# zhouzypaul/fql

Measured on AMD Instinct MI355X. Metric: FQL gradient-steps/s (batch=256), higher is better.
Workload: dtype f32

## Files before the change

### fql_amd/csrc/fql_chain.h

```cpp
#pragma once
#include "fql_kernels.h"

#define FQL_CHAIN_THREADS 512
#ifndef FQL_CHAIN_WAVES
#define FQL_CHAIN_WAVES 4
#endif

struct ChainArgs {
    const float* A;
    const float* Wf;
    const float* bias;
    float* C;
    union {
        struct {
            const float* ea_in;
            float* ea_out;
            const float* W0f;
            const float* evp_in;
            const float* eb;
            const float* W4f;
            float* evp_out;
        };
        struct {
            const float* Gv;
            const float* stats;
            const float* gamma;
            const float* dq;
            const float* wq;
            int ldq, ldw;
            int width;
            int ncol, ldc;
        };
    };
    int M, ad, ap, ea_ld;
    float inv_steps, t_s;
    int variant;
    const float* Zprev;
    int xg;
    int hw;
    int tl;
    unsigned long long* stamps;
};

struct WfragTask {
    const float* src;
    float* dst;
    int K, N, ld;
    int kvalid;
    int tile0;
    int mode;
};
__global__ __launch_bounds__(FQL_THREADS) void fql_wfrag_kernel(const WfragTask* __restrict__ tasks, int ntasks, int tl) {
    tl_enter(tl);
    const WfragTask& T = tasks[find_task(tasks, ntasks, blockIdx.x)];
    const int e = (blockIdx.x - T.tile0) * FQL_THREADS + threadIdx.x;
    if (T.mode == 1) {
        const int n = e % T.N, r = e / T.N;
        const int q = r & 3, j = r >> 2;
        if (j >= (T.K >> 5)) return;
        float v[8];
#pragma unroll
        for (int i = 0; i < 8; ++i) { const int k = 32 * j + 8 * q + i; v[i] = (k < T.kvalid) ? ldg(T.src + (size_t)k * T.ld + n) : 0.f; }
        u32x4 hi, lo;
#pragma unroll
        for (int i = 0; i < 4; ++i) { unsigned h, l; bsplit2(v[2 * i], v[2 * i + 1], h, l); hi[i] = h; lo[i] = l; }
        unsigned* d = reinterpret_cast<unsigned*>(T.dst) + (((size_t)(2 * j) * T.N + n) * 4 + q) * 4;
        *(FQL_GAS u32x4*)d = hi;
        *(FQL_GAS u32x4*)(d + (size_t)T.N * 16) = lo;
        return;
    }
    if (T.mode == 2) {
        const int n = e % T.N, k4 = e / T.N;
        if (k4 >= (T.K >> 2)) return;
        float v[4];
#pragma unroll
        for (int i = 0; i < 4; ++i) v[i] = (4 * k4 + i < T.kvalid) ? ldg(T.src + (size_t)(4 * k4 + i) * T.ld + n) : 0.f;
        unsigned h0, l0, h1, l1;
        bsplit2(v[0], v[1], h0, l0);
        bsplit2(v[2], v[3], h1, l1);
        *(FQL_GAS u32x4*)(reinterpret_cast<unsigned*>(T.dst) + ((size_t)k4 * T.N + n) * 4) = u32x4{h0, h1, l0, l1};
        return;
    }
    const int n = e % T.N, k4 = e / T.N;
    if (k4 >= (T.K >> 2)) return;
    f32x4 v;
#pragma unroll
    for (int s = 0; s < 4; ++s) v[s] = (4 * k4 + s < T.kvalid) ? ldg(T.src + (size_t)(4 * k4 + s) * T.ld + n) : 0.f;
    stg4(T.dst + ((size_t)k4 * T.N + n) * 4, v);
}

template <int H, int V>
__device__ __forceinline__ void chain_body(const ChainArgs& P) {
    static_assert(H % 128 == 0 && H <= 1024, "hidden width must be a multiple of 128");
    constexpr int S = H + 4;
    constexpr int GQ = H / 64;
    constexpr int NA = H / 128;
    constexpr int CT = H / 128;
    constexpr int NT = H / 32;
    extern __shared__ __attribute__((aligned(16))) float lds[];
    float* red = lds + 16 * S;
    float* ea = red + 4 * 2 * 64 * 4;
    float* hs = ea + 512;
    const int tid = threadIdx.x, wave = tid >> 6, lane = tid & 63;
    const int c = lane & 15, q = lane >> 4;
    const int nt = wave & 1, kp = wave >> 1;
    constexpr int variant = V;
    const int ntc = variant == 4 ? P.ncol / 32 : NT;
    int tm = blockIdx.x / ntc, tn = blockIdx.x - tm * ntc;
    if (P.xg) xcd_tile((int)blockIdx.x, P.M >> 4, ntc, P.xg, tm, tn);
    const int row0 = tm * 16, n0 = tn * 32 + nt * 16;
    tl_enter(P.tl);
#ifdef FQL_STAMPS
    unsigned long long stamp[8];
    int nst = 0;
#define CSTAMP() do { __builtin_amdgcn_s_waitcnt(0); stamp[nst++] = __builtin_amdgcn_s_memrealtime(); } while (0)
#else
#define CSTAMP() do {} while (0)
#endif
    CSTAMP();
    f32x4 bf[GQ];
    {
        if (variant == 3 || variant == 4) {
            const float* wb = P.Wf + (size_t)(n0 + c) * H + 16 * kp * GQ + 4 * q;
#pragma unroll
            for (int g = 0; g < GQ; ++g) bf[g] = ldg4(wb + 16 * g);
        } else {
            const float* wb = P.Wf + ((size_t)(4 * kp * GQ + q) * H + n0 + c) * 4;
#pragma unroll
            for (int g = 0; g < GQ; ++g) bf[g] = ldg4(wb + (size_t)g * 16 * H);
        }
    }
    const float bias = variant == 4 ? 0.f : variant == 3 ? ldg(P.Zprev + (size_t)(row0 + 4 * q + kp) * H + n0 + c) : ldg(P.bias + n0 + c);
    f32x4 bw4[2];
    if (variant == 2 && wave == 0) {
#pragma unroll
        for (int g = 0; g < 2; ++g) bw4[g] = ldg4(P.W4f + ((size_t)(tn * 8 + 4 * g + q) * P.ap + c) * 4);
    }
    if (variant == 0) {
        f32x4 cacc[CT], wf[CT];
#pragma unroll
        for (int t = 0; t < CT; ++t) {
            const int ct = wave + 8 * t;
            cacc[t] = ldg4(P.A + ((size_t)((row0 >> 2) + q) * H + 16 * ct + c) * 4);
            wf[t] = ldg4(P.W0f + ((size_t)q * H + 16 * ct + c) * 4);
        }
        {
            const int e = tid >> 1, half = tid & 1;
            const int r = e >> 4, j = e & 15;
            float a = 0.f;
            if (j < P.ad) {
                a = ldg(P.ea_in + (size_t)(row0 + r) * P.ea_ld + j);
                if (P.evp_in) {
                    float pv[NT / 2];
                    const float* pp = P.evp_in + ((size_t)(half * (NT / 2)) * P.M + row0 + r) * P.ap + j;
#pragma unroll
                    for (int tp = 0; tp < NT / 2; ++tp) pv[tp] = ldg(pp + (size_t)tp * P.M * P.ap);
                    float sum = 0.f;
#pragma unroll
                    for (int tp = 0; tp < NT / 2; ++tp) sum += pv[tp];
                    const float other = __shfl_xor(sum, 1);
                    const float tot = half ? other + sum : sum + other;
                    a += (tot + ldg(P.eb + j)) * P.inv_steps;
                }
                if (tn == 0 && half == 0 && P.ea_out) stg(P.ea_out + (size_t)(row0 + r) * P.ap + j, a);
            } else if (j == P.ad) {
                a = P.t_s;
            }
            if (half == 0) ea[r * 32 + j] = a;
        }
        CSTAMP();
        __syncthreads();
        {
            const f32x4 af = *reinterpret_cast<const f32x4*>(&ea[c * 32 + 4 * q]);
#pragma unroll
            for (int t = 0; t < CT; ++t) {
#pragma unroll
                for (int s4 = 0; s4 < 4; ++s4) cacc[t] = __builtin_amdgcn_mfma_f32_16x16x4f32(af[s4], wf[t][s4], cacc[t], 0, 0, 0);
                const int ct = wave + 8 * t;
#pragma unroll
                for (int i = 0; i < 4; ++i) lds[(4 * q + i) * S + 16 * ct + c] = gelu_f(cacc[t][i]);
            }
        }
    } else if (variant == 4) {
        constexpr int NV = H / 256;
        f32x4 dy[2][NV], zz[2][NV], gq[2][NV], gm[NV];
        float mean[2], rstd[2];
#pragma unroll
        for (int i = 0; i < NV; ++i) gm[i] = ldg4(P.gamma + 4 * (lane + 64 * i));
        float wqv[NV][4];
        if (!P.A) {
#pragma unroll
            for (int i = 0; i < NV; ++i)
#pragma unroll
                for (int e = 0; e < 4; ++e) wqv[i][e] = ldg(P.wq + (size_t)(4 * (lane + 64 * i) + e) * P.ldw);
        }
#pragma unroll
        for (int r = 0; r < 2; ++r) {
            const size_t row = (size_t)(row0 + 2 * wave + r);
            mean[r] = ldg(P.stats + 2 * row); rstd[r] = ldg(P.stats + 2 * row + 1);
            const float dqr = P.A ? 0.f : ldg(P.dq + row * P.ldq);
#pragma unroll
            for (int i = 0; i < NV; ++i) {
                const int k4 = 4 * (lane + 64 * i);
                zz[r][i] = ldg4(P.Zprev + row * H + k4);
                gq[r][i] = ldg4(P.Gv + row * H + k4);
                if (P.A) dy[r][i] = ldg4(P.A + row * H + k4);
                else dy[r][i] = f32x4{dqr * wqv[i][0], dqr * wqv[i][1], dqr * wqv[i][2], dqr * wqv[i][3]};
            }
        }
        const float inv = 1.0f / (float)P.width;
#pragma unroll
        for (int r = 0; r < 2; ++r) {
            float s1 = 0.f, s2 = 0.f;
#pragma unroll
            for (int i = 0; i < NV; ++i)
#pragma unroll
                for (int e = 0; e < 4; ++e) {
                    const float d = dy[r][i][e] * gm[i][e], xh = (gq[r][i][e] - mean[r]) * rstd[r];
                    dy[r][i][e] = d; gq[r][i][e] = xh;
                    if (4 * (lane + 64 * i) + e < P.width) { s1 += d; s2 += d * xh; }
                }
#pragma unroll
            for (int o = 1; o < 64; o <<= 1) { s1 += __shfl_xor(s1, o); s2 += __shfl_xor(s2, o); }
            const float m1 = s1 * inv, m2 = s2 * inv;
#pragma unroll
            for (int i = 0; i < NV; ++i) {
                f32x4 o;
#pragma unroll
                for (int e = 0; e < 4; ++e)
                    o[e] = (4 * (lane + 64 * i) + e < P.width) ? rstd[r] * (dy[r][i][e] - m1 - gq[r][i][e] * m2) * zz[r][i][e] : 0.f;
                *reinterpret_cast<f32x4*>(&lds[(2 * wave + r) * S + 4 * (lane + 64 * i)]) = o;
            }
        }
    } else {
        f32x4 av[NA];
        const float* Ag = P.A + (size_t)row0 * H;
#pragma unroll
        for (int i = 0; i < NA; ++i) av[i] = ldg4(Ag + (size_t)(tid + i * FQL_CHAIN_THREADS) * 4);
#pragma unroll
        for (int i = 0; i < NA; ++i) {
            const int f = tid + i * FQL_CHAIN_THREADS;
            const int r = f / (H / 4), kk = f - r * (H / 4);
            *reinterpret_cast<f32x4*>(&lds[r * S + 4 * kk]) = av[i];
        }
        CSTAMP();
    }
    __syncthreads();
    CSTAMP();
    f32x4 acc = {0.f, 0.f, 0.f, 0.f}, acc2 = {0.f, 0.f, 0.f, 0.f};
    {
        const float* arow = lds + c * S + 4 * q + 16 * kp * GQ;
#pragma unroll
        for (int g = 0; g < GQ; g += 2) {
            const f32x4 a = *reinterpret_cast<const f32x4*>(arow + 16 * g);
            const f32x4 a2 = *reinterpret_cast<const f32x4*>(arow + 16 * g + 16);
#pragma unroll
            for (int s4 = 0; s4 < 4; ++s4) {
                acc = __builtin_amdgcn_mfma_f32_16x16x4f32(a[s4], bf[g][s4], acc, 0, 0, 0);
                acc2 = __builtin_amdgcn_mfma_f32_16x16x4f32(a2[s4], bf[g + 1][s4], acc2, 0, 0, 0);
            }
        }
        acc += acc2;
    }
    *reinterpret_cast<f32x4*>(&red[((kp * 2 + nt) * 64 + lane) * 4]) = acc;
    CSTAMP();
    __syncthreads();
    float v = (variant == 3 || variant == 4) ? 0.f : bias;
#pragma unroll
    for (int p = 0; p < 4; ++p) v += red[((p * 2 + nt) * 64 + lane) * 4 + kp];
    v = variant == 4 ? v : variant == 3 ? v * bias : gelu_f(v);
    const int row = row0 + 4 * q + kp;
    if (variant == 4) {
        stg(P.C + (size_t)row * P.ldc + n0 + c, v);
    } else if (variant != 2) {
        stg(P.C + (size_t)row * H + n0 + c, v);
    } else {
        hs[(4 * q + kp) * 36 + 16 * nt + c] = v;
        __syncthreads();
        if (wave == 0) {
            f32x4 pa = {0.f, 0.f, 0.f, 0.f};
#pragma unroll
            for (int g = 0; g < 2; ++g) {
                const f32x4 a4 = *reinterpret_cast<const f32x4*>(&hs[c * 36 + 16 * g + 4 * q]);
#pragma unroll
                for (int s4 = 0; s4 < 4; ++s4) pa = __builtin_amdgcn_mfma_f32_16x16x4f32(a4[s4], bw4[g][s4], pa, 0, 0, 0);
            }
            if (c < P.ap) {
#pragma unroll
                for (int i = 0; i < 4; ++i) stg(P.evp_out + ((size_t)tn * P.M + row0 + 4 * q + i) * P.ap + c, pa[i]);
            }
        }
    }
    tl_exit(P.tl);
#ifdef FQL_STAMPS
    CSTAMP();
    if (lane == 0 && wave == 0 && P.stamps) {
        unsigned long long* d = P.stamps + (size_t)blockIdx.x * 8;
        for (int i = 0; i < nst; ++i) d[i] = stamp[i];
    }
#endif
}
struct Dgrad0Args {
    GemmTask t[4];
    int ntasks, col0;
};
__device__ __forceinline__ void fql_dgrad0_body(const Dgrad0Args& P) {
    __shared__ __attribute__((aligned(16))) float red[4 * 64 * 4];
    const int tid = threadIdx.x, kp = tid >> 6, lane = tid & 63, c = lane & 15, q = lane >> 4;
    const int ntm = P.t[0].M >> 4;
    const int ti = (int)blockIdx.x / ntm, tm = (int)blockIdx.x - ti * ntm;
    const GemmTask& T = P.t[ti];
    const int row0 = tm * 16, kq = T.K >> 2;
    const float* ap = T.A + (size_t)(row0 + c) * T.lda + kp * kq + 4 * q;
    const float* bp = T.B + (size_t)(P.col0 + c) * T.ldb + kp * kq + 4 * q;
    f32x4 acc = {0.f, 0.f, 0.f, 0.f}, acc2 = {0.f, 0.f, 0.f, 0.f};
    for (int g0 = 0; g0 < kq; g0 += 128) {
        f32x4 a[8], b[8];
#pragma unroll
        for (int g = 0; g < 8; ++g) { a[g] = ldg4(ap + g0 + 16 * g); b[g] = ldg4(bp + g0 + 16 * g); }
#pragma unroll
        for (int g = 0; g < 8; g += 2)
#pragma unroll
            for (int s4 = 0; s4 < 4; ++s4) {
                acc = __builtin_amdgcn_mfma_f32_16x16x4f32(a[g][s4], b[g][s4], acc, 0, 0, 0);
                acc2 = __builtin_amdgcn_mfma_f32_16x16x4f32(a[g + 1][s4], b[g + 1][s4], acc2, 0, 0, 0);
            }
    }
    acc += acc2;
    *reinterpret_cast<f32x4*>(&red[(kp * 64 + lane) * 4]) = acc;
    __syncthreads();
    float v = 0.f;
#pragma unroll
    for (int p = 0; p < 4; ++p) v += red[(p * 64 + lane) * 4 + kp];
    stg(T.C + (size_t)(row0 + 4 * q + kp) * T.ldc + P.col0 + c, v);
}
__global__ __launch_bounds__(FQL_THREADS) void fql_dgrad0_kernel(const Dgrad0Args P) { fql_dgrad0_body(P); }
__global__ __launch_bounds__(FQL_THREADS) void fql_dgrad0_multi_kernel(const Dgrad0Args* __restrict__ args) { fql_dgrad0_body(args[blockIdx.y]); }

__device__ __forceinline__ void fql_head_dgrad_body(const GemmTask& T) {
    __shared__ __attribute__((aligned(16))) float da[16 * 20];
    const int tid = threadIdx.x, wave = tid >> 6, lane = tid & 63, c = lane & 15, q = lane >> 4;
    const int ntn = T.N >> 6;
    const int tm = (int)blockIdx.x / ntn, tn = (int)blockIdx.x - tm * ntn;
    const int row0 = tm * 16, n0 = tn * 64 + 16 * wave;
    const f32x4 b4 = ldg4(T.B + (size_t)(n0 + c) * T.ldb + 4 * q);
    float zp[4];
#pragma unroll
    for (int i = 0; i < 4; ++i) zp[i] = ldg(T.Zprev + (size_t)(row0 + 4 * q + i) * T.ldc + n0 + c);
    {
        const int r = tid >> 4, j = tid & 15;
        float g = 0.f;
        if (j < T.i2) {
            const float ar = ldg(T.ea_in + (size_t)(row0 + r) * T.i0 + j);
            float tg;
            if (T.flags & GF_A_EULFIN) {
                float pv[32];
#pragma unroll
                for (int tp = 0; tp < 32; ++tp) pv[tp] = ldg(T.aux2 + ((size_t)min(tp, T.ln_width - 1) * T.M + row0 + r) * T.i0 + j);
                float sum = 0.f;
#pragma unroll
                for (int tp = 0; tp < 32; ++tp) sum += (tp < T.ln_width) ? pv[tp] : 0.f;
                tg = clip1(ldg(T.aux + (size_t)(row0 + r) * T.i0 + j) + (sum + ldg(T.eb + j)) * T.f1);
                if (tn == 0) stg(const_cast<float*>(T.evp) + (size_t)(row0 + r) * T.i0 + j, tg);
            } else tg = ldg(T.evp + (size_t)(row0 + r) * T.i0 + j);
            g = T.f0 * (ar - tg);
            if (ar > -1.0f && ar < 1.0f) {
                const size_t o = (size_t)(row0 + r) * T.e_ntp + T.i1 + j;
                g += ldg(T.ew + o) + ldg(T.ew4 + o);
            }
            if (tn == 0 && T.ea_out) stg(T.ea_out + (size_t)(row0 + r) * T.i0 + j, g);
        }
        da[r * 20 + j] = g;
    }
    __syncthreads();
    const f32x4 a4 = *reinterpret_cast<const f32x4*>(&da[c * 20 + 4 * q]);
    f32x4 acc = {0.f, 0.f, 0.f, 0.f};
#pragma unroll
    for (int s4 = 0; s4 < 4; ++s4) acc = __builtin_amdgcn_mfma_f32_16x16x4f32(a4[s4], b4[s4], acc, 0, 0, 0);
#pragma unroll
    for (int i = 0; i < 4; ++i) stg(T.C + (size_t)(row0 + 4 * q + i) * T.ldc + n0 + c, acc[i] * zp[i]);
}
__global__ __launch_bounds__(FQL_THREADS) void fql_head_dgrad_kernel(const GemmTask T) { fql_head_dgrad_body(T); }
__global__ __launch_bounds__(FQL_THREADS) void fql_head_dgrad_multi_kernel(const GemmTask* __restrict__ args) { const GemmTask T = ((const FQL_CONST_AS GemmTask*)args)[blockIdx.y]; fql_head_dgrad_body(T); }

template <int H, int V>
__global__ __launch_bounds__(FQL_CHAIN_THREADS, FQL_CHAIN_WAVES) void fql_chain_kernel(const ChainArgs P) { chain_body<H, V>(P); }
struct ChainPair { ChainArgs t[2]; };
template <int H, int V>
__global__ __launch_bounds__(FQL_CHAIN_THREADS, FQL_CHAIN_WAVES) void fql_chain_pair_kernel(const ChainPair P) { chain_body<H, V>(P.t[blockIdx.y]); }
template <int H, int V>
__global__ __launch_bounds__(FQL_CHAIN_THREADS, FQL_CHAIN_WAVES) void fql_chain_multi_kernel(const ChainArgs* __restrict__ args) { const ChainArgs P = args[blockIdx.y]; chain_body<H, V>(P); }
__device__ __forceinline__ float lane_xor1(float v) {
    return __int_as_float(__builtin_amdgcn_mov_dpp(__float_as_int(v), 0xB1, 0xF, 0xF, true));
}
#ifndef FQL_CHAIN_SPLIT_WAVES_A
#define FQL_CHAIN_SPLIT_WAVES_A 4
#endif
template <int H, int V>
__global__ __launch_bounds__(FQL_CHAIN_THREADS, (V == 0 ? FQL_CHAIN_SPLIT_WAVES_A : 4)) void fql_chain_split_kernel(const ChainArgs P) {
    static_assert(H % 128 == 0 && H <= 1024, "hidden width must be a multiple of 128");
    constexpr int RS = H / 2;
    constexpr int NS = H / 128;
    constexpr int NA = H / 128;
    constexpr int CT = H / 128;
    constexpr int NT = H / 32;
    extern __shared__ __attribute__((aligned(16))) float lds[];
    unsigned* ahi = reinterpret_cast<unsigned*>(lds);
    unsigned* alo = ahi + 16 * RS;
    float* red = reinterpret_cast<float*>(alo + 16 * RS);
    float* ea = red + 4 * 2 * 64 * 4;
    float* hs = ea + 512;
    const int tid = threadIdx.x, wave = tid >> 6, lane = tid & 63;
    const int c = lane & 15, q = lane >> 4;
    const int nt = wave & 1, kp = wave >> 1;
    int tm = blockIdx.x / NT, tn = blockIdx.x - tm * NT;
    if (P.xg) xcd_tile((int)blockIdx.x, P.M >> 4, NT, P.xg, tm, tn);
    const int row0 = tm * 16, n0 = tn * 32 + nt * 16;
    constexpr int variant = V;
    tl_enter(P.tl);
    u32x4 bh[NS], bl[NS];
    {
        const unsigned* wb = reinterpret_cast<const unsigned*>(P.Wf) + (((size_t)(2 * kp * NS) * H + n0 + c) * 4 + q) * 4;
#pragma unroll
        for (int s = 0; s < NS; ++s) { bh[s] = ldg4u(wb + (size_t)s * H * 32); bl[s] = ldg4u(wb + (size_t)s * H * 32 + H * 16); }
    }
    const float bias = ldg(P.bias + n0 + c);
    u32x4 w4h, w4l;
    if (variant == 2 && wave == 0) {
        const unsigned* w4 = reinterpret_cast<const unsigned*>(P.W4f) + (((size_t)(2 * tn) * P.ap + c) * 4 + q) * 4;
        w4h = ldg4u(w4); w4l = ldg4u(w4 + P.ap * 16);
    }
    if (variant == 0) {
        f32x4 cacc[CT];
        u32x4 wf[CT];
#pragma unroll
        for (int t = 0; t < CT; ++t) {
            const int ct = wave + 8 * t;
            cacc[t] = ldg4(P.A + (((size_t)(row0 >> 4) * (H / 16) + ct) * 64 + 16 * q + c) * 4);
            wf[t] = ldg4u(reinterpret_cast<const unsigned*>(P.W0f) + ((size_t)q * H + 16 * ct + c) * 4);
        }
        {
            const int e = tid >> 1, half = tid & 1;
            const int r = e >> 4, j = e & 15;
            float a = 0.f;
            if (j < P.ad) {
                a = ldg(P.ea_in + (size_t)(row0 + r) * P.ea_ld + j);
                if (P.evp_in) {
                    float pv[NT / 2];
                    const float* pp = P.evp_in + ((size_t)(half * (NT / 2)) * P.M + row0 + r) * P.ap + j;
#pragma unroll
                    for (int tp = 0; tp < NT / 2; ++tp) pv[tp] = ldg(pp + (size_t)tp * P.M * P.ap);
                    float sum = 0.f;
#pragma unroll
                    for (int tp = 0; tp < NT / 2; ++tp) sum += pv[tp];
                    const float other = __shfl_xor(sum, 1);
                    const float tot = half ? other + sum : sum + other;
                    a += (tot + ldg(P.eb + j)) * P.inv_steps;
                }
                if (tn == 0 && half == 0 && P.ea_out) stg(P.ea_out + (size_t)(row0 + r) * P.ap + j, a);
            } else if (j == P.ad) {
                a = P.t_s;
            }
            if (half == 0) ea[r * 32 + j] = a;
        }
        __syncthreads();
        {
            const f32x4 af = *reinterpret_cast<const f32x4*>(&ea[c * 32 + 4 * q]);
            u32x2 afh, afl;
            bsplit4(af, afh, afl);
#pragma unroll
            for (int t = 0; t < CT; ++t) {
                const u32x2 wh = u32x2{wf[t][0], wf[t][1]}, wl = u32x2{wf[t][2], wf[t][3]};
                cacc[t] = mfma_bf16_k16(wl, afh, cacc[t]);
                cacc[t] = mfma_bf16_k16(wh, afl, cacc[t]);
                cacc[t] = mfma_bf16_k16(wh, afh, cacc[t]);
            }
#pragma unroll
            for (int t = 0; t < CT; ++t) {
                const int ct = wave + 8 * t;
                f32x4 g;
#pragma unroll
                for (int i = 0; i < 4; ++i) g[i] = gelu_f(cacc[t][i]);
                u32x2 hi, lo;
                bsplit4(g, hi, lo);
                const int w = c * RS + 4 * ((2 * ct + (q >> 1)) ^ c) + 2 * (q & 1);
                *reinterpret_cast<u32x2*>(ahi + w) = hi;
                *reinterpret_cast<u32x2*>(alo + w) = lo;
            }
        }
    } else {
        u32x4 av[NA];
        const unsigned* Ah = reinterpret_cast<const unsigned*>(P.A) + (size_t)row0 * RS;
        const unsigned* Al = Ah + (size_t)P.M * RS;
#pragma unroll
        for (int i = 0; i < NA; ++i) {
            const int pc = (tid + i * FQL_CHAIN_THREADS) & (4 * RS - 1);
            av[i] = ldg4u((i < NA / 2 ? Ah : Al) + (size_t)pc * 4);
        }
#pragma unroll
        for (int i = 0; i < NA; ++i) {
            const int pc = (tid + i * FQL_CHAIN_THREADS) & (4 * RS - 1);
            const int r = pc / (RS / 4), sl = pc - r * (RS / 4);
            *reinterpret_cast<u32x4*>((i < NA / 2 ? ahi : alo) + r * RS + 4 * (sl ^ r)) = av[i];
        }
    }
    __syncthreads();
    f32x4 acc = {0.f, 0.f, 0.f, 0.f}, acc2 = {0.f, 0.f, 0.f, 0.f}, acc3 = {0.f, 0.f, 0.f, 0.f};
#pragma unroll
    for (int s = 0; s < NS; ++s) {
        const int w = c * RS + 4 * ((4 * (kp * NS + s) + q) ^ c);
        const u32x4 fah = *reinterpret_cast<const u32x4*>(ahi + w);
        const u32x4 fal = *reinterpret_cast<const u32x4*>(alo + w);
        acc = mfma_bf16(fah, bh[s], acc);
        acc2 = mfma_bf16(fah, bl[s], acc2);
        acc3 = mfma_bf16(fal, bh[s], acc3);
    }
    acc += acc2 + acc3;
    *reinterpret_cast<f32x4*>(&red[((kp * 2 + nt) * 64 + lane) * 4]) = acc;
    __syncthreads();
    float v = bias;
#pragma unroll
    for (int p = 0; p < 4; ++p) v += red[((p * 2 + nt) * 64 + lane) * 4 + kp];
    v = gelu_f(v);
    const int row = row0 + 4 * q + kp;
    if (variant != 2) {
        const float o = lane_xor1(v);
        unsigned h, l;
        bsplit2((c & 1) ? o : v, (c & 1) ? v : o, h, l);
        unsigned* Cw = reinterpret_cast<unsigned*>(P.C) + ((c & 1) ? (size_t)P.M * RS : 0) + (size_t)row * RS + ((n0 + c) >> 1);
        *(FQL_GAS unsigned*)Cw = (c & 1) ? l : h;
    } else {
        hs[(4 * q + kp) * 36 + 16 * nt + c] = v;
        __syncthreads();
        if (wave == 0) {
            const f32x4 a0 = *reinterpret_cast<const f32x4*>(&hs[c * 36 + 8 * q]);
            const f32x4 a1 = *reinterpret_cast<const f32x4*>(&hs[c * 36 + 8 * q + 4]);
            u32x2 h0, l0, h1, l1;
            bsplit4(a0, h0, l0);
            bsplit4(a1, h1, l1);
            const u32x4 fah = u32x4{h0[0], h0[1], h1[0], h1[1]}, fal = u32x4{l0[0], l0[1], l1[0], l1[1]};
            f32x4 pa = {0.f, 0.f, 0.f, 0.f};
            pa = mfma_bf16(fal, w4h, pa);
            pa = mfma_bf16(fah, w4l, pa);
            pa = mfma_bf16(fah, w4h, pa);
            if (c < P.ap) {
#pragma unroll
                for (int i = 0; i < 4; ++i) stg(P.evp_out + ((size_t)tn * P.M + row0 + 4 * q + i) * P.ap + c, pa[i]);
            }
        }
    }
    tl_exit(P.tl);
}
#define FQL_CHAIN_LDS_BYTES(H) ((size_t)(16 * ((H) + 4) + 4 * 2 * 64 * 4 + 512 + 16 * 36) * sizeof(float))
```

### fql_amd/csrc/fql_engine.hip

```cpp
#include "../../include/fql_amd.h"
#include "fql_kernels.h"
#include "fql_conv.h"
#include "fql_chain.h"
#include "fql_aux.h"
#include "fql_ifql.h"
#include "fql_rebrac.h"
#include "fql_sac.h"
#include "fql_bc.h"
#include "fql_iql.h"
#include "fql_iqld.h"
#include "fql_cfgrl.h"
#include <hip/hip_ext.h>
#include "fql_aql.h"

#include <algorithm>
#include <cmath>
#include <cstdarg>
#include <cstdio>
#include <cstdlib>
#include <cstring>
#include <map>
#include <memory>
#include <random>
#include <string>
// ... 131 lines not shown
template <typename... Pm, typename... A>
Bound bind(void (*k)(Pm...), Geo g, A&&... a) {
    static_assert(sizeof...(Pm) == sizeof...(A) && sizeof...(Pm) <= FQL_BOUND_ARGS, "a bound launch takes exactly the kernel's arguments");
    static_assert(packed_bytes<Pm...>() <= FQL_BOUND_BYTES, "arguments larger than a kernarg segment");
    Bound b;
    b.fn = (const void*)k;
    b.grid[0] = g.grid.x; b.grid[1] = g.grid.y; b.grid[2] = g.grid.z;
    b.block[0] = g.block.x; b.block[1] = g.block.y; b.block[2] = g.block.z;
    b.lds = (unsigned)g.lds;
    b.args.resize(packed_bytes<Pm...>());
    size_t off = 0;
    auto put = [&](auto v) {
        using T = decltype(v);
        off = (off + alignof(T) - 1) & ~(alignof(T) - 1);
        b.at[b.nargs++] = (int)off;
        std::memcpy(b.args.data() + off, &v, sizeof(T));
        off += sizeof(T);
    };
    (put(static_cast<Pm>(a)), ...);
    return b;
}
inline Bound tl_in(Bound k, size_t off) { k.tl_at = k.at[0] + (int)off; return k; }
inline Bound tl_last(Bound k) { k.tl_at = k.at[k.nargs - 1]; return k; }
inline void launch_bound(const Bound& k, const void* args, hipStream_t s, hipEvent_t pa = nullptr, hipEvent_t pb = nullptr) {
    void* argv[FQL_BOUND_ARGS];
    for (int i = 0; i < k.nargs; ++i) argv[i] = (unsigned char*)args + k.at[i];
    const dim3 g(k.grid[0], k.grid[1], k.grid[2]), b(k.block[0], k.block[1], k.block[2]);
    if (pa) (void)hipExtLaunchKernel(k.fn, g, b, argv, k.lds, s, pa, pb, 0);
    else (void)hipLaunchKernel(k.fn, g, b, argv, k.lds, s);
}

struct Op {
    OpType type;
    std::vector<const void*> reads, writes;
    GemmTask gemm;
    WgradTask wgrad;
    LnBwdTask ln;
    PostOsArgs postos;
    LossCriticArgs lc;
    LossQArgs lq;
    LossBcArgs lb;
    ConvArgs conv;
    ConvWgradArgs cw;
    ConvWredArgs cwr;
    const ConvWprepTask* wprep_tasks = nullptr;
    int wprep_n = 0;
    int cw_grid = 0;
    Bound k;
    double macs = 0.0;
    int level = 0;
    int lane = 0;
    int launch = -1;
    std::vector<int> deps;
};

struct Launch {
    Launch() = default;
    Launch(OpType t, int ln) : type(t), lane(ln) {}
    OpType type;
    int lane = 0;
    int grid = 0, ntasks = 0;
    Bound k;
    double macs = 0.0;
    void* table = nullptr;
    void *table_w = nullptr, *table_l = nullptr, *table_m = nullptr;
    int n_w = 0, n_l = 0, tile_w = 0, tile_l = 0, tile_m = 0;
    std::vector<GemmTask> h_gemm;
    std::vector<WgradTask> h_wgrad;
    std::vector<LnBwdTask> h_ln;
    std::vector<MiscTask> h_misc;
    bool ka = false;
    std::vector<int> waits;
    bool record_after = false;
    hipEvent_t ev = nullptr;
};

inline bool ka_tasks_env() {
    const char* e = getenv("FQL_KERNARG_TASKS");
    return !e || atoi(e) != 0;
}
inline bool fused_tail_env() {
    const char* e = getenv("FQL_FUSED_TAIL");
    return !e || atoi(e) != 0;
}
inline std::unique_ptr<SideArgs> ka_side_args(const Launch& L) {
    const size_t ng = L.h_gemm.size(), nw = L.h_wgrad.size(), nl = L.h_ln.size(), nm = L.h_misc.size();
    if (ng > FQL_KA_GEMM || nw > FQL_KA_WGRAD || nl > FQL_KA_LN || nm > FQL_KA_MISC) return nullptr;
    auto a = std::make_unique<SideArgs>();
    std::memset(a.get(), 0, sizeof(SideArgs));
    SideFront& f = a->f;
    f.tile_w = L.tile_w; f.tile_l = L.tile_l; f.tile_m = L.tile_m; f.tl = -1;
    for (int& v : f.g0) v = FQL_KA_FRONT_PAD;
    for (int& v : f.w0) v = FQL_KA_FRONT_PAD;
    for (int& v : f.l0) v = FQL_KA_FRONT_PAD;
    for (size_t i = 0; i < ng; ++i) { a->g[i] = L.h_gemm[i]; if (i) f.g0[i - 1] = L.h_gemm[i].tile0; }
    for (size_t i = 0; i < nw; ++i) { a->w[i] = L.h_wgrad[i]; if (i) f.w0[i - 1] = L.h_wgrad[i].tile0; }
    for (size_t i = 0; i < nl; ++i) { a->l[i] = L.h_ln[i]; if (i) f.l0[i - 1] = L.h_ln[i].tile0; }
    for (size_t i = 0; i < nm; ++i) a->m[i] = L.h_misc[i];
    return a;
}
struct AdamOpt {
    float lr = 0.f;
    DevState* st = nullptr;
    int polyak = -1;
    bool fin = false;
};
struct Program {
    std::vector<Op> ops;
    std::vector<Launch> launches;
    bool lane_used[FQL_LANES] = {};
    hipEvent_t ev_fork = nullptr, ev_join[FQL_LANES] = {};
    hipGraph_t graph = nullptr;
    hipGraphExec_t exec = nullptr;
    int64_t macs = 0;
    AqlProgram aql;
    bool aql_tried = false;
};

template <typename P, typename IssueFn>
void issue_lanes(P& pr, hipStream_t s0, const hipStream_t* ls, bool fork, IssueFn&& issue) {
    auto lazy = [](hipEvent_t& e) { if (!e) HIP_CHECK(hipEventCreateWithFlags(&e, hipEventDisableTiming)); };
    bool side = false;
    if (ls) for (int l = 1; l < FQL_LANES; ++l) side |= pr.lane_used[l];
    if (side && fork) {
        lazy(pr.ev_fork);
        HIP_CHECK(hipEventRecord(pr.ev_fork, s0));
        for (int l = 1; l < FQL_LANES; ++l) if (pr.lane_used[l]) HIP_CHECK(hipStreamWaitEvent(ls[l], pr.ev_fork, 0));
    }
    for (auto& L : pr.launches) {
        const hipStream_t s = side && L.lane != 0 ? ls[L.lane] : s0;
        if (side)
            for (int w : L.waits) if (pr.launches[w].ev) HIP_CHECK(hipStreamWaitEvent(s, pr.launches[w].ev, 0));
        issue(L, s);
        if (side && L.record_after) {
            lazy(L.ev);
            HIP_CHECK(hipEventRecord(L.ev, s));
        }
    }
    if (side)
        for (int l = 1; l < FQL_LANES; ++l) {
            if (!pr.lane_used[l]) continue;
            lazy(pr.ev_join[l]);
            HIP_CHECK(hipEventRecord(pr.ev_join[l], ls[l]));
            HIP_CHECK(hipStreamWaitEvent(s0, pr.ev_join[l], 0));
        }
    HIP_CHECK(hipGetLastError());
}
template <typename P>
void destroy_lane_events(P& pr) {
    for (auto& L : pr.launches) if (L.ev) { hipEventDestroy(L.ev); L.ev = nullptr; }
    if (pr.ev_fork) { hipEventDestroy(pr.ev_fork); pr.ev_fork = nullptr; }
    for (hipEvent_t& e : pr.ev_join) if (e) { hipEventDestroy(e); e = nullptr; }
}

template <typename Body>
void capture_graph(hipStream_t s, Body&& body, hipGraph_t& graph, hipGraphExec_t& exec) {
    static const bool trace = getenv("FQL_TRACE") != nullptr;
    HIP_CHECK(hipStreamBeginCapture(s, hipStreamCaptureModeThreadLocal));
    try {
        body();
    } catch (...) {
        hipGraph_t g = nullptr;
        hipStreamEndCapture(s, &g);
        if (g) hipGraphDestroy(g);
        throw;
    }
// ... 1692 lines not shown
            HIP_CHECK(hipMemcpy(all + at, o->wprep_tasks, (size_t)o->wprep_n * sizeof(ConvWprepTask), hipMemcpyDeviceToDevice));
            at += o->wprep_n;
        }
        Launch L(OP_CONV_WPREP, sel[0]->lane);
        L.k = bind_wprep(all, tot);
        return L;
    }
    Launch form_gemm16(const Cell& sel, std::vector<void*>& owner) {
        Launch L(OP_GEMM, sel[0]->lane);
        L.ntasks = (int)sel.size();
        int tile = 0;
        for (const Op* o : sel) {
            GemmTask t = o->gemm;
            t.wk = (t.N <= 16) ? 4 : 2;
            t.tmt = 1;
            t.ntn = (t.N / 16 + (4 / t.wk) - 1) / (4 / t.wk);
            t.tile0 = tile;
            tile += (t.M / 16) * t.ntn;
            L.h_gemm.push_back(t);
        }
        L.table = upload(owner, L.h_gemm.data(), L.h_gemm.size() * sizeof(GemmTask));
        L.grid = tile;
        bind_gemm16(L);
        return L;
    }

    static double op_macs(const Op& o) {
        if (o.type == OP_GEMM || o.type == OP_GEMM64 || o.type == OP_HEAD_DGRAD) return (double)o.gemm.M * o.gemm.N * o.gemm.K;
        if (o.type == OP_DGRAD0) return (double)o.gemm.M * 16.0 * o.gemm.K;
        if (o.type == OP_WGRAD) return (double)o.wgrad.M * o.wgrad.Kin * o.wgrad.N;
        if (o.type == OP_CHAIN) return o.macs;
        if (o.type == OP_CONV || o.type == OP_CONV_U8) return (double)o.conv.N * o.conv.H * o.conv.W * 9.0 * (o.conv.transposed ? o.conv.Ci : o.conv.Ci_real) * o.conv.Co;
        if (o.type == OP_CONV_WGRAD) return (double)o.cw.N * o.cw.H * o.cw.W * 9.0 * o.cw.Ci_real * o.cw.Co;
        return 0.0;
    }
    static void cross_lane_waits(Program& pr) {
        std::vector<int> need(pr.launches.size() * FQL_LANES, -1);
        for (const Op& o : pr.ops) {
            if (o.launch < 0) continue;
            for (int d : o.deps) {
                const int dl = pr.ops[d].launch;
                const int ol = pr.launches[dl].lane;
                int& nd = need[o.launch * FQL_LANES + ol];
                if (ol != o.lane) nd = std::max(nd, dl);
            }
        }
        int waited_upto[FQL_LANES][FQL_LANES];
        for (auto& r : waited_upto) for (int& v : r) v = -1;
        for (int li = 0; li < (int)pr.launches.size(); ++li) {
            Launch& L = pr.launches[li];
            for (int ol = 0; ol < FQL_LANES; ++ol) {
                const int nd = need[li * FQL_LANES + ol];
                if (nd <= waited_upto[L.lane][ol]) continue;
                L.waits.push_back(nd);
                pr.launches[nd].record_after = true;
                waited_upto[L.lane][ol] = nd;
            }
        }
    }
    void dump_program(const Program& pr) const {
        std::vector<int> level(pr.launches.size(), -1);
        std::vector<std::string> what(pr.launches.size());
        char b[96];
        for (const Op& o : pr.ops) {
            if (o.launch < 0) continue;
            level[o.launch] = o.level;
            if (o.type == OP_GEMM || o.type == OP_GEMM64) snprintf(b, sizeof b, " g%s(%dx%dx%d%s)", o.type == OP_GEMM64 ? "64" : "16", o.gemm.M, o.gemm.N, o.gemm.K, (o.gemm.flags & GF_TRANS_B) ? "T" : "");
            else if (o.type == OP_WGRAD) snprintf(b, sizeof b, " w(%dx%dx%d)", o.wgrad.M, o.wgrad.Kin, o.wgrad.N);
            else if (o.type == OP_LNBWD) snprintf(b, sizeof b, " ln(%d)", o.ln.M);
            else snprintf(b, sizeof b, " t%d", (int)o.type);
            what[o.launch] += b;
        }
        int cnt[FQL_LANES] = {};
        for (int li = 0; li < (int)pr.launches.size(); ++li) {
            const Launch& L = pr.launches[li];
            cnt[L.lane]++;
            fprintf(stderr, "[fql] #%2d level %3d lane %d type %2d ntasks %2d grid %5d waits[", li, level[li], L.lane, (int)L.type, L.ntasks, L.grid);
            for (int w : L.waits) fprintf(stderr, "%d ", w);
            fprintf(stderr, "] :%s\n", what[li].c_str());
        }
        fprintf(stderr, "[fql] launches per lane:");
        for (int l = 0; l < FQL_LANES; ++l) fprintf(stderr, " %d", cnt[l]);
        fprintf(stderr, "\n");
    }
    static void check_lane_edges(const Program& pr) {
        bool edge[FQL_LANES][FQL_LANES] = {};
        for (const Launch& L : pr.launches)
            for (int w : L.waits) edge[pr.launches[w].lane][L.lane] = true;
        for (int a = 1; a < FQL_LANES; ++a)
            for (int b = a + 1; b < FQL_LANES; ++b)
                if (edge[a][b] && edge[b][a])
                    invalid("lane placement makes lanes %d and %d wait on each other in both directions: not capturable on this HIP runtime "
                            "(hipStreamEndCapture recursion); move one of the passes", a, b);
    }

    hipEvent_t prof_a = nullptr, prof_b = nullptr;
    void issue_args(const Launch& L, int tl, unsigned char* a) const {
        const Bound& k = L.k;
        if (!k.fn) throw HipError{"internal: op type " + std::to_string((int)L.type) + " carries no bound launch"};
        std::memcpy(a, k.args.data(), k.args.size());
        if (k.tl_at >= 0) std::memcpy(a + k.tl_at, &tl, sizeof tl);
        if (L.type == OP_IQLD_CFG) std::memcpy(a + offsetof(IqldCfgStepArgs, cfg), &sample_cfg, sizeof sample_cfg);
    }
    void issue(const Launch& L, hipStream_t s, int tl) {
        alignas(16) unsigned char a[FQL_BOUND_BYTES];
        issue_args(L, tl, a);
        launch_bound(L.k, a, s, prof_a, prof_b);
    }
    int tl_of(const Program& pr, const Launch& L) const { return &pr == &prog_full ? (int)(&L - pr.launches.data()) : -1; }
    void run_launches(Program& pr, hipStream_t s0, const hipStream_t* ls = nullptr, bool fork = true) {
        static const bool trace_l = getenv("FQL_TRACE") != nullptr;
        issue_lanes(pr, s0, ls, fork, [&](const Launch& L, hipStream_t s) {
            if (trace_l) {
                fprintf(stderr, "[fql] launch %d type %d lane %d grid %d waits %zu:", (int)(&L - pr.launches.data()), (int)L.type, L.lane, L.grid, L.waits.size());
                for (int w : L.waits) fprintf(stderr, " %d(lane %d)", w, pr.launches[w].lane);
                fprintf(stderr, "\n");
            }
            issue(L, s, tl_of(pr, L));
        });
    }
    std::vector<AqlDispatch> dispatches(const Program& pr) const {
        std::vector<AqlDispatch> out;
        alignas(16) unsigned char a[FQL_BOUND_BYTES];
        for (const Launch& L : pr.launches) {
            issue_args(L, tl_of(pr, L), a);
            const Bound& k = L.k;
            out.push_back(AqlDispatch{k.fn, {k.grid[0], k.grid[1], k.grid[2]}, {k.block[0], k.block[1], k.block[2]}, k.lds, std::vector<uint8_t>(a, a + k.args.size())});
        }
        return out;
    }

    void build_aql(Program& pr) {
        static const bool off = getenv("FQL_AQL") && atoi(getenv("FQL_AQL")) == 0;
        static const bool trace_a = getenv("FQL_TRACE") != nullptr;
        AqlProgram& ap = pr.aql;
        ap = AqlProgram{};
        if (off || visual) return;
        void* kargs = nullptr;
        try {
            if (!aql.up && aql.why.empty()) aql.init(device, (const void*)&fql_create);
            if (!aql.up) throw AqlError{aql.why};
            const std::vector<AqlDispatch> rec = dispatches(pr);
            const size_t n = pr.launches.size();

            std::vector<const AqlKernelInfo*> ki(n);
            std::vector<size_t> koff(n);
            size_t tot = 0;
            for (size_t i = 0; i < n; ++i) {
                ki[i] = &aql.kernel(rec[i].fn);
                if (ki[i]->kernarg_size < rec[i].args.size()) throw AqlError{"recorded arguments exceed the kernel's kernarg segment"};
                koff[i] = tot;
                tot += ((size_t)ki[i]->kernarg_size + 63) & ~(size_t)63;
            }
            std::vector<uint8_t> host(tot);
            for (size_t i = 0; i < n; ++i) AqlRuntime::fill_kernarg(host.data() + koff[i], rec[i], *ki[i]);
            HIP_CHECK(hipMalloc(&kargs, tot));
            HIP_CHECK(hipMemcpy(kargs, host.data(), tot, hipMemcpyHostToDevice));
            std::vector<int> sig(n, AQL_SIG_NONE);
            int nsig = 0;
            bool used[FQL_AQL_LANES] = {};
            for (const Launch& L : pr.launches) {
                if (L.lane < 0 || L.lane >= FQL_AQL_LANES) throw AqlError{"lane out of range"};
                used[L.lane] = true;
                for (int w : L.waits) if (sig[w] == AQL_SIG_NONE) sig[w] = nsig++;
            }
            if (!used[0]) throw AqlError{"program without a lane 0"};
            int endsig[FQL_AQL_LANES];
            for (int l = 1; l < FQL_AQL_LANES; ++l) endsig[l] = used[l] ? nsig++ : AQL_SIG_NONE;
            constexpr int AG = HSA_FENCE_SCOPE_AGENT, SY = HSA_FENCE_SCOPE_SYSTEM, NO = HSA_FENCE_SCOPE_NONE;
            for (int l = 1; l < FQL_AQL_LANES; ++l)
                if (used[l]) {
                    AqlPacket b = AqlRuntime::barrier_packet(false, NO, NO);
                    b.deps[0] = AQL_SIG_PREV_DONE;
                    ap.lane[l].push_back(b);
                }
            bool first[FQL_AQL_LANES] = {true, true, true, true};
            for (size_t i = 0; i < n; ++i) {
                const Launch& L = pr.launches[i];
                for (size_t w0 = 0; w0 < L.waits.size(); w0 += 5) {
                    AqlPacket b = AqlRuntime::barrier_packet(false, NO, NO);
                    for (size_t j = 0; j < 5 && w0 + j < L.waits.size(); ++j) b.deps[j] = sig[L.waits[w0 + j]];
                    ap.lane[L.lane].push_back(b);
                }
                AqlPacket k = AqlRuntime::kernel_packet(rec[i], *ki[i], (uint64_t)(uintptr_t)kargs + koff[i], true, first[L.lane] ? SY : AG, AG);
                first[L.lane] = false;
                k.complete = sig[i];
                ap.lane[L.lane].push_back(k);
            }
            for (int l = 1; l < FQL_AQL_LANES; ++l)
                if (used[l]) {
                    AqlPacket b = AqlRuntime::barrier_packet(true, NO, AG);
                    b.complete = endsig[l];
                    ap.lane[l].push_back(b);
                }
            {
                AqlPacket b = AqlRuntime::barrier_packet(true, NO, SY);
                int j = 0;
                for (int l = 1; l < FQL_AQL_LANES; ++l) if (used[l]) b.deps[j++] = endsig[l];
                b.complete = AQL_SIG_DONE;
                ap.lane[0].push_back(b);
            }
            aql.ensure_signals(nsig);
            for (int l = 0; l < FQL_AQL_LANES; ++l) if (used[l]) aql.ensure_queue(l);
            ap.nsig = nsig;
            ap.kernargs = kargs;
            ap.ok = true;
            if (trace_a) fprintf(stderr, "[fql] AQL program: %zu launches, packets per lane %zu %zu %zu %zu, %d signals, %zu bytes of kernargs\n", n,
                                 ap.lane[0].size(), ap.lane[1].size(), ap.lane[2].size(), ap.lane[3].size(), nsig, tot);
        } catch (const AqlError& e) {
            if (kargs) hipFree(kargs);
            ap = AqlProgram{};
            if (aql.why.empty()) aql.why = e.msg;
            if (trace_a || getenv("FQL_AQL")) fprintf(stderr, "[fql] AQL path off: %s\n", e.msg.c_str());
        }
    }

    void capture(Program& pr) {
        if (pr.exec) { hipGraphExecDestroy(pr.exec); pr.exec = nullptr; }
        if (pr.graph) { hipGraphDestroy(pr.graph); pr.graph = nullptr; }
        HIP_CHECK(hipStreamSynchronize(stream));
        capture_graph(stream, [&] { run_launches(pr, stream, lane_streams); }, pr.graph, pr.exec);
    }

    bool capture_split(Program& pr) {
        int last_needed_by_lane1 = -1, first_lane0_wait = -1;
        for (int li = 0; li < (int)pr.launches.size(); ++li) {
            const Launch& L = pr.launches[li];
            if (L.lane > 1) return false;
            for (int w : L.waits) {
                if (L.lane == 1) last_needed_by_lane1 = std::max(last_needed_by_lane1, w);
                if (L.lane == 0 && first_lane0_wait < 0) first_lane0_wait = li;
            }
        }
        if (last_needed_by_lane1 < 0 || first_lane0_wait < 0 || first_lane0_wait <= last_needed_by_lane1) return false;
        auto seg_of = [&](int li) {
            const Launch& L = pr.launches[li];
            if (L.lane == 1) return 1;
            if (li <= last_needed_by_lane1) return 0;
            return li < first_lane0_wait ? 2 : 3;
        };
        for (int seg = 0; seg < 4; ++seg) {
            Program sub;
            for (int li = 0; li < (int)pr.launches.size(); ++li)
                if (seg_of(li) == seg) { Launch L = pr.launches[li]; L.waits.clear(); L.record_after = false; L.ev = nullptr; L.lane = 0; sub.launches.push_back(L); }
            if (sub.launches.empty()) return false;
            HIP_CHECK(hipStreamSynchronize(stream));
            capture_graph(stream, [&] { run_launches(sub, stream); }, split_graph[seg], split_exec[seg]);
        }
        if (!ev_a) HIP_CHECK(hipEventCreateWithFlags(&ev_a, hipEventDisableTiming));
        if (!ev_b) HIP_CHECK(hipEventCreateWithFlags(&ev_b, hipEventDisableTiming));
        return true;
    }
    void free_split() {
        for (int i = 0; i < 4; ++i) {
            if (split_exec[i]) { hipGraphExecDestroy(split_exec[i]); split_exec[i] = nullptr; }
            if (split_graph[i]) { hipGraphDestroy(split_graph[i]); split_graph[i] = nullptr; }
        }
        split_ok = false;
    }
    void launch_split(hipStream_t s0, hipStream_t s1) {
        HIP_CHECK(hipGraphLaunch(split_exec[0], s0));
        HIP_CHECK(hipEventRecord(ev_a, s0));
        HIP_CHECK(hipStreamWaitEvent(s1, ev_a, 0));
        HIP_CHECK(hipGraphLaunch(split_exec[1], s1));
        HIP_CHECK(hipEventRecord(ev_b, s1));
        HIP_CHECK(hipGraphLaunch(split_exec[2], s0));
        if (!ev_c) HIP_CHECK(hipEventCreateWithFlags(&ev_c, hipEventDisableTiming));
// ... 3723 lines not shown
        for (int j = 0; j < i; ++j) if (members[j] == h) invalid("fql_group_create: member %d appears twice", i);
        if (h->group) invalid("fql_group_create: member %d already belongs to a group", i);
        if (h->visual) invalid("fql_group_create: member %d has an encoder (groups take state agents only)", i);
        if (h->cfg.precision != 0) invalid("fql_group_create: member %d has precision %d (groups take fp32 members only)", i, h->cfg.precision);
        if (h->began) invalid("fql_group_create: member %d is between fql_update_begin and fql_update_end", i);
        require_graph(h->prog_full);
        fql_config a = h->cfg, b = members[0]->cfg;
        a.alpha = b.alpha = 0.f;
        a.batch_size = b.batch_size = 0;
        if (std::memcmp(&a, &b, sizeof a) != 0)
            invalid("fql_group_create: member %d's config differs from member 0's in more than seed and alpha", i);
        if (h->B != members[0]->B) invalid("fql_group_create: member %d has batch size %d, member 0 has %d", i, h->B, members[0]->B);
        const Program& p = h->prog_full, &p0 = members[0]->prog_full;
        if (p.launches.size() != p0.launches.size()) invalid("fql_group_create: member %d's update has %zu launches, member 0's %zu", i, p.launches.size(), p0.launches.size());
        for (size_t li = 0; li < p.launches.size(); ++li) {
            const Launch &L = p.launches[li], &L0 = p0.launches[li];
            if (L.type != L0.type || L.lane != L0.lane || L.grid != L0.grid || L.waits != L0.waits || L.record_after != L0.record_after)
                invalid("fql_group_create: launch %zu of member %d differs from member 0's (type %d/%d, lane %d/%d, grid %d/%d)", li, i, (int)L.type,
                        (int)L0.type, L.lane, L0.lane, L.grid, L0.grid);
            if (L.type == OP_WFRAG && h->wfrag_grid != members[0]->wfrag_grid) invalid("fql_group_create: member %d's weight-copy launch differs", i);
        }
    }
}
}

extern "C" {

int fql_group_create(const fql_handle* members, int k, fql_group* out) {
    if (!out) { g_create_error = "fql_group_create: out must not be NULL"; return FQL_E_INVALID; }
    *out = nullptr;
    for (int i = 0; members && i < k; ++i)
        if (members[i] && members[i]->kind != AgentKind::FQL) {
            g_create_error = "fql_group_create: member " + std::to_string(i) + " is " + members[i]->desc().label + " (groups take FQL agents only)";
            return FQL_E_STATE;
        }
    auto* g = new fql_group_s();
    try {
        group_check(members, k);
        g->m.assign(members, members + k);
        g->K = k;
        g->B = members[0]->B;
        for (fql_handle h : g->m) { h->aql_drain(); HIP_CHECK(hipStreamSynchronize(h->stream)); }
        const size_t n = g->m[0]->prog_full.launches.size();
        for (size_t li = 0; li < n; ++li)
            for (int i = 1; i < k; ++i) {
                const Bound &a = g->m[i]->prog_full.launches[li].k, &b = g->m[0]->prog_full.launches[li].k;
                if (a.fn != b.fn || std::memcmp(a.grid, b.grid, sizeof a.grid) || std::memcmp(a.block, b.block, sizeof a.block) || a.lds != b.lds)
                    invalid("fql_group_create: launch %zu of member %d runs another kernel or shape than member 0's", li, i);
            }
        for (size_t li = 0; li < n; ++li) {
            const Bound& k0 = g->m[0]->prog_full.launches[li].k;
            if (k0.grid[1] != 1 || k0.grid[2] != 1) invalid("fql_group_create: launch %zu has a 2-D grid: not groupable", li);
            g->launches.push_back(g->zip((int)li, [](fql_engine& e) -> Program& { return e.prog_full; }));
            g->lane_used[g->launches.back().lane] = true;
        }
        for (int l = 0; l < FQL_LANES; ++l) HIP_CHECK(hipStreamCreateWithFlags(&g->lanes[l], hipStreamNonBlocking));
        for (hipEvent_t* e : {&g->ev_in, &g->ev_done}) HIP_CHECK(hipEventCreateWithFlags(e, hipEventDisableTiming));
        HIP_CHECK(hipMalloc((void**)&g->d_idx, (size_t)k * g->B * sizeof(int64_t)));
        g->capture();
    } catch (const Invalid& e) {
        g_create_error = e.msg; g->release(); delete g; return FQL_E_INVALID;
    } catch (const HipError& e) {
        g_create_error = e.msg; g->release(); delete g; return FQL_E_HIP;
    }
    for (fql_handle h : g->m) { h->group = g; h->grp_done = g->ev_done; h->grp_pending = false; h->grp_touched = true; }
    *out = g;
    return FQL_OK;
}

int fql_debug_task_forms(fql_handle h, fql_group g, void* out, size_t bytes) {
    if ((!h && !g) || (bytes && !out) || bytes % sizeof(int32_t)) return FQL_E_INVALID;
    if (!g && (h->visual || !h->prog_full.exec || h->prog_full.launches.empty())) return FQL_E_STATE;
    auto form = [](const Launch& L) { return !is_table_launch(L.type) ? 0 : L.ka ? 2 : 1; };
    std::vector<int32_t> w{0, FQL_KA_GEMM, FQL_KA_WGRAD, FQL_KA_LN, FQL_KA_MISC, 0};
    if (g) for (const GLaunch& G : g->launches) w.push_back(G.form);
    else for (const Launch& L : h->prog_full.launches) w.push_back(form(L));
    w[5] = (int32_t)w.size() - 6;
    w[0] = (int32_t)w.size();
    if (bytes > w.size() * sizeof(int32_t)) return FQL_E_INVALID;
    if (bytes) std::memcpy(out, w.data(), bytes);
    return FQL_OK;
}

int fql_group_destroy(fql_group g) {
    if (!g) return FQL_OK;
    g->release();
    delete g;
    return FQL_OK;
}

int fql_group_update_from_dataset(fql_group g, const int64_t* idx, int batch_size, float* info13xk, void* stream) {
    if (!g) { g_create_error = "fql_group_update_from_dataset: NULL group"; return FQL_E_INVALID; }
    try {
        if (batch_size != g->B) invalid("fql_group_update_from_dataset: batch_size %d does not match the members' %d", batch_size, g->B);
        if (g->member_began()) { g_create_error = "fql_group_update_from_dataset: a member is between fql_update_begin and fql_update_end"; return FQL_E_STATE; }
        const hipStream_t s = g->enter(stream);
        const int64_t* rows = idx;
        if (idx && !fql_engine::is_device_ptr(idx)) {
            HIP_CHECK(hipMemcpyAsync(g->d_idx, idx, (size_t)g->K * g->B * sizeof(int64_t), hipMemcpyHostToDevice, s));
            HIP_CHECK(hipStreamSynchronize(s));
            rows = g->d_idx;
        }
        for (int i = 0; i < g->K; ++i) g->m[i]->source_from_dataset(rows ? rows + (size_t)i * g->B : nullptr, g->B, 0, 0, nullptr, s);
        HIP_CHECK(hipGraphLaunch(g->exec, s));
        if (info13xk) {
            for (int i = 0; i < g->K; ++i)
                HIP_CHECK(hipMemcpyAsync(info13xk + (size_t)i * FQL_NUM_INFO, &g->m[i]->d_state->info[0], FQL_NUM_INFO * sizeof(float), hipMemcpyDefault, s));
        }
        g->leave(s, info13xk && !fql_engine::is_device_ptr(info13xk));
    } catch (const Invalid& e) {
        g_create_error = e.msg; return FQL_E_INVALID;
    } catch (const HipError& e) {
        g_create_error = e.msg; return FQL_E_HIP;
    }
    return FQL_OK;
}

static int group_sample(fql_group g, const char* fn, bool flow, const float* obs, const float* noise, const uint64_t* seeds, int n, float* out, void* stream) {
    if (!g) { g_create_error = std::string(fn) + ": NULL group"; return FQL_E_INVALID; }
    try {
        if (n <= 0) invalid("%s: n must be positive (got %d)", fn, n);
        if (!obs || !out) invalid("%s: observations/out must not be NULL", fn);
        if (flow && !noise) invalid("%s: noises must not be NULL", fn);
        if (!noise && !seeds) invalid("%s: seeds must not be NULL when noises is NULL (one seed per member)", fn);
        if (g->member_began()) { g_create_error = std::string(fn) + ": a member is between fql_update_begin and fql_update_end"; return FQL_E_STATE; }
        const hipStream_t s = g->enter(stream);
        g->sample(flow, obs, noise, seeds, n, out, s);
        g->leave(s, !stream && fql_engine::is_device_ptr(out));
    } catch (const Invalid& e) {
        g_create_error = e.msg; return FQL_E_INVALID;
    } catch (const HipError& e) {
        g_create_error = e.msg; return FQL_E_HIP;
    } catch (const std::exception& e) {
        g_create_error = e.what(); return FQL_E_HIP;
    }
    return FQL_OK;
}
int fql_group_sample_actions(fql_group g, const float* observations, int n, const float* noises, const uint64_t* seeds, float* out, void* stream) {
    return group_sample(g, "fql_group_sample_actions", false, observations, noises, seeds, n, out, stream);
}
int fql_group_flow_actions(fql_group g, const float* observations, const float* noises, int n, float* out, void* stream) {
    return group_sample(g, "fql_group_flow_actions", true, observations, noises, nullptr, n, out, stream);
}
int fql_group_sample_stats(fql_group g, int flow, int64_t* launches_per_call) {
    if (!g) { g_create_error = "fql_group_sample_stats: NULL group"; return FQL_E_INVALID; }
    if (!launches_per_call) { g_create_error = "fql_group_sample_stats: launches_per_call must not be NULL"; return FQL_E_INVALID; }
    try {
        *launches_per_call = g->sample_launches(flow != 0);
    } catch (const Invalid& e) {
        g_create_error = e.msg; return FQL_E_INVALID;
    } catch (const HipError& e) {
        g_create_error = e.msg; return FQL_E_HIP;
    }
    return FQL_OK;
}

int fql_group_synchronize(fql_group g) {
    if (!g) { g_create_error = "fql_group_synchronize: NULL group"; return FQL_E_INVALID; }
    if ((g->last == hipStreamLegacy ? hipDeviceSynchronize() : hipEventSynchronize(g->ev_done)) != hipSuccess || hipStreamSynchronize(g->lanes[0]) != hipSuccess) {
        g_create_error = std::string("fql_group_synchronize: ") + hipGetErrorString(hipGetLastError());
        return FQL_E_HIP;
    }
    for (fql_handle h : g->m) h->grp_pending = false;
    return FQL_OK;
}

// ... 2 lines not shown
```

### fql_amd/csrc/fql_kernels.h

```cpp
#pragma once
#include <hip/hip_runtime.h>
#include <stdint.h>

typedef float f32x4 __attribute__((ext_vector_type(4)));

#define FQL_GAS __attribute__((address_space(1)))
__device__ __forceinline__ float ldg(const float* p) { return *(const FQL_GAS float*)p; }
__device__ __forceinline__ f32x4 ldg4(const float* p) { return *(const FQL_GAS f32x4*)p; }
__device__ __forceinline__ void stg(float* p, float v) { *(FQL_GAS float*)p = v; }
__device__ __forceinline__ void stg4(float* p, f32x4 v) { *(FQL_GAS f32x4*)p = v; }

#define FQL_THREADS 256

struct FastDiv {
    unsigned m;
    int d;
    __device__ __forceinline__ explicit FastDiv(int dd) : m(dd > 1 ? 0xFFFFFFFFu / (unsigned)dd + 1u : 0u), d(dd) {}
    __device__ __forceinline__ FastDiv(int dd, unsigned long long max_x) : m(dd > 1 && max_x * (unsigned long long)dd < (1ull << 32) ? 0xFFFFFFFFu / (unsigned)dd + 1u : 0u), d(dd) {}
    __device__ __forceinline__ int div(int x) const { return m ? (int)__umulhi((unsigned)x, m) : (d == 1 ? x : (int)((unsigned)x / (unsigned)d)); }
    __device__ __forceinline__ void divmod(int x, int& q, int& r) const { q = div(x); r = x - q * d; }
};

__device__ __forceinline__ float frcp(int d) { return __builtin_amdgcn_rcpf((float)d); }
__device__ __forceinline__ int sdiv(int x, float rd) { return (int)(((float)x + 0.5f) * rd); }

__device__ __forceinline__ void xcd_tile(int local, int ntm, int ntn, int gm, int& tm, int& tn) {
    const int gs = 31 - __clz(gm);
    const int x = local & 7, j = local >> 3;
    const int bn = ntn >> (3 - gs), bm = ntm >> gs;
    const int xm = x >> (3 - gs);
    const int jm = sdiv(j, frcp(bn));
    tm = xm * bm + jm;
    tn = (x - (xm << (3 - gs))) * bn + (j - jm * bn);
}

typedef unsigned u32x4 __attribute__((ext_vector_type(4)));
typedef unsigned u32x2 __attribute__((ext_vector_type(2)));
typedef __bf16 bf16x8 __attribute__((ext_vector_type(8)));
typedef __bf16 bf16x4 __attribute__((ext_vector_type(4)));
typedef __bf16 bf16x2 __attribute__((ext_vector_type(2)));
typedef float f32x2 __attribute__((ext_vector_type(2)));
__device__ __forceinline__ unsigned cvt_pk_bf16(float x0, float x1) {
    return __builtin_bit_cast(unsigned, __builtin_convertvector(f32x2{x0, x1}, bf16x2));
}
__device__ __forceinline__ void bsplit2(float x0, float x1, unsigned& hi, unsigned& lo) {
    hi = cvt_pk_bf16(x0, x1);
    const float h0 = __uint_as_float(hi << 16), h1 = __uint_as_float(hi & 0xffff0000u);
    lo = cvt_pk_bf16(x0 - h0, x1 - h1);
}
__device__ __forceinline__ void bsplit4(const f32x4& v, u32x2& hi, u32x2& lo) {
    unsigned h0, l0, h1, l1;
    bsplit2(v[0], v[1], h0, l0);
    bsplit2(v[2], v[3], h1, l1);
    hi = u32x2{h0, h1};
    lo = u32x2{l0, l1};
}
__device__ __forceinline__ f32x4 mfma_bf16(const u32x4& a, const u32x4& b, const f32x4& acc) {
    return __builtin_amdgcn_mfma_f32_16x16x32_bf16(__builtin_bit_cast(bf16x8, a), __builtin_bit_cast(bf16x8, b), acc, 0, 0, 0);
}
typedef short s16x4 __attribute__((ext_vector_type(4)));
__device__ __forceinline__ f32x4 mfma_bf16_k16(const u32x2& a, const u32x2& b, const f32x4& acc) {
    return __builtin_amdgcn_mfma_f32_16x16x16bf16_1k(__builtin_bit_cast(s16x4, a), __builtin_bit_cast(s16x4, b), acc, 0, 0, 0);
}
__device__ __forceinline__ u32x4 ldg4u(const unsigned* p) { return *(const FQL_GAS u32x4*)p; }
__device__ __forceinline__ u32x2 lds_read_tr16(const unsigned* p) {
    typedef __attribute__((address_space(3))) bf16x4* lds_bf16x4_ptr;
    return __builtin_bit_cast(u32x2, __builtin_amdgcn_ds_read_tr16_b64_v4bf16((lds_bf16x4_ptr)p));
}

#ifdef FQL_TIMELINE
#define FQL_TL_MAX 128
#define FQL_TL_WGS 2048
__device__ unsigned long long g_fql_tl[FQL_TL_MAX][FQL_TL_WGS][2];
__device__ __forceinline__ void tl_enter(int id) {
    if (id >= 0 && id < FQL_TL_MAX && threadIdx.x == 0 && blockIdx.x < FQL_TL_WGS) g_fql_tl[id][blockIdx.x][0] = __builtin_amdgcn_s_memrealtime();
}
__device__ __forceinline__ void tl_exit(int id) {
    if (id >= 0 && id < FQL_TL_MAX && threadIdx.x == 0 && blockIdx.x < FQL_TL_WGS) g_fql_tl[id][blockIdx.x][1] = __builtin_amdgcn_s_memrealtime();
}
#else
#define tl_enter(id) ((void)0)
#define tl_exit(id) ((void)0)
#endif

enum : int {
    GF_TRANS_B = 1 << 0,
    GF_BIAS = 1 << 1,
    GF_GELU = 1 << 2,
    GF_SAVE_Z = 1 << 3,
    GF_A_LN = 1 << 4,
    GF_LN_WRITE = 1 << 5,
// ... 341 lines not shown
                    acc[r] = __builtin_amdgcn_mfma_f32_16x16x4f32(a.w, bt[4 * t + 3], acc[r], 0, 0, 0);
                }
            }
        }
    }
}

template <int NA, int TMT, bool EUL>
__device__ __forceinline__ void gemm16_body(const GemmTask& T, float* lds) {
    const int local = blockIdx.x - T.tile0;
    const int tm = sdiv(local, frcp(T.ntn)), tn = local - tm * T.ntn;
    const int row0 = tm * 16 * TMT;
    const int K = T.K, N = T.N;
    const int S = K + 4;
    const int tid = threadIdx.x;
    const int wave = tid >> 6, lane = tid & 63;
    const int flags = T.flags;
    const int WK = T.wk, wks = WK >> 1, NW = 4 >> wks;
    float* red = lds + 16 * TMT * S;
#ifdef FQL_STAMPS
    unsigned long long stamp[8];
    int nst = 0;
#define STAMP() do { __builtin_amdgcn_s_waitcnt(0); stamp[nst++] = __builtin_amdgcn_s_memrealtime(); } while (0)
    STAMP();
#else
#define STAMP() do {} while (0)
#endif

    const int nt = wave & (NW - 1), kp = wave >> (2 - wks);
    const int n0 = (tn * NW + nt) * 16;
    const int c = lane & 15, q = lane >> 4;
    const bool active = n0 < N;
    const int G = K >> 4;
    const int gbeg = (kp * G) >> wks, gend = ((kp + 1) * G) >> wks;
    const bool transb = (flags & GF_TRANS_B) != 0;
    const int k4 = K >> 2;
    const float rk4 = frcp(k4);
    const int nA = 16 * k4;
    float b0[32], b1[32];
    BAddr ba = transb ? gemm_baddr<true>(T, n0, c, q) : gemm_baddr<false>(T, n0, c, q);
    float bias = 0.f;
    float* ea = red + 1024 * TMT;
    float* hs = ea + 512;
    const bool euler0 = EUL && TMT == 1 && (flags & GF_A_EULER0);
    const bool head = EUL && TMT == 1 && (flags & GF_HEAD_PART);
    auto issue_b = [&]() {
#pragma unroll
        for (int i = 0; i < 32; ++i) { b0[i] = 0.f; b1[i] = 0.f; }
        if (active) {
            const int nfull = (gend - gbeg) >> 3;
            if (transb) {
                if (nfull > 0) gemm_load_chunk<true>(b0, ba.base + (size_t)(16 * gbeg) * ba.kstep, ba.ldb);
                if (nfull > 1) gemm_load_chunk<true>(b1, ba.base + (size_t)(16 * (gbeg + 8)) * ba.kstep, ba.ldb);
            } else {
                if (nfull > 0) gemm_load_chunk<false>(b0, ba.base + (size_t)(16 * gbeg) * ba.kstep, ba.ldb);
                if (nfull > 1) gemm_load_chunk<false>(b1, ba.base + (size_t)(16 * (gbeg + 8)) * ba.kstep, ba.ldb);
            }
            if ((flags & GF_BIAS) && kp == 0) bias = ldg(T.bias + n0 + c);
        }
    };
    float bw4[8];
#pragma unroll
    for (int i = 0; i < 8; ++i) bw4[i] = 0.f;
    if (head && wave == 0) {
#pragma unroll
        for (int g = 0; g < 2; ++g)
#pragma unroll
            for (int s4 = 0; s4 < 4; ++s4) {
                const int k = tn * 32 + 16 * g + 4 * q + s4;
                const float v = ldg(T.ew4 + (size_t)min(k, N - 1) * T.i1 + c);
                bw4[4 * g + s4] = (k < N) ? v : 0.f;
            }
    }
    if (euler0) {
        issue_b();
        const int ad = T.i2, apw = T.i1, M = T.M;
        constexpr int CT = NA;
        f32x4 cacc[CT];
        float wf[CT][4];
#pragma unroll
        for (int t = 0; t < CT; ++t) {
            const int ct = min(wave + 4 * t, (K >> 4) - 1);
#pragma unroll
            for (int i = 0; i < 4; ++i) cacc[t][i] = ldg(T.A + (size_t)(row0 + 4 * q + i) * T.lda + 16 * ct + c);
#pragma unroll
            for (int s4 = 0; s4 < 4; ++s4) wf[t][s4] = ldg(T.ew + (size_t)(4 * q + s4) * K + 16 * ct + c);
        }
        for (int e = tid; e < 16 * 16; e += FQL_THREADS) {
            const int r = e >> 4, j = e & 15;
            float a = 0.f;
            if (j < ad) {
                a = ldg(T.ea_in + (size_t)(row0 + r) * T.i0 + j);
                if (T.evp) {
                    float pv[32];
#pragma unroll
                    for (int tp = 0; tp < 32; ++tp) pv[tp] = ldg(T.evp + ((size_t)min(tp, T.e_ntp - 1) * M + row0 + r) * apw + j);
                    float sum = 0.f;
#pragma unroll
                    for (int tp = 0; tp < 32; ++tp) sum += (tp < T.e_ntp) ? pv[tp] : 0.f;
                    a += (sum + ldg(T.eb + j)) * T.f0;
                }
                if (tn == 0 && T.ea_out) stg(T.ea_out + (size_t)(row0 + r) * apw + j, a);
            } else if (j == ad) {
                a = T.f1;
            }
            ea[r * 32 + j] = a;
        }
        __syncthreads();
        {
            const f32x4 af = *reinterpret_cast<const f32x4*>(&ea[c * 32 + 4 * q]);
#pragma unroll
            for (int t = 0; t < CT; ++t) {
                if (wave + 4 * t < (K >> 4)) {
#pragma unroll
                    for (int s4 = 0; s4 < 4; ++s4) cacc[t] = __builtin_amdgcn_mfma_f32_16x16x4f32(af[s4], wf[t][s4], cacc[t], 0, 0, 0);
                    const int ct = wave + 4 * t;
#pragma unroll
                    for (int i = 0; i < 4; ++i) lds[(4 * q + i) * S + 16 * ct + c] = gelu_f(cacc[t][i]);
                }
            }
        }
    } else if (EUL && TMT == 1 && (flags & GF_A_LOSSACT)) {
        issue_b();
        for (int e = tid; e < 16 * K; e += FQL_THREADS) {
            const int r = sdiv(e, frcp(K)), j = e - r * K;
            float g = 0.f;
            if (j < T.i2) {
                const float ar = ldg(T.ea_in + (size_t)(row0 + r) * T.i0 + j);
                float tg;
                if (flags & GF_A_EULFIN) {
                    float pv[32];
#pragma unroll
                    for (int tp = 0; tp < 32; ++tp) pv[tp] = ldg(T.aux2 + ((size_t)min(tp, T.ln_width - 1) * T.M + row0 + r) * T.i0 + j);
                    float sum = 0.f;
#pragma unroll
                    for (int tp = 0; tp < 32; ++tp) sum += (tp < T.ln_width) ? pv[tp] : 0.f;
                    tg = clip1(ldg(T.aux + (size_t)(row0 + r) * T.i0 + j) + (sum + ldg(T.eb + j)) * T.f1);
                    if (tn == 0) stg(const_cast<float*>(T.evp) + (size_t)(row0 + r) * T.i0 + j, tg);
                } else tg = ldg(T.evp + (size_t)(row0 + r) * T.i0 + j);
                g = T.f0 * (ar - tg);
                if (ar > -1.0f && ar < 1.0f) {
                    const size_t o = (size_t)(row0 + r) * T.e_ntp + T.i1 + j;
                    g += ldg(T.ew + o) + ldg(T.ew4 + o);
                }
                if (tn == 0 && T.ea_out) stg(T.ea_out + (size_t)(row0 + r) * T.i0 + j, g);
            }
            lds[r * S + j] = g;
        }
    } else {
#pragma unroll
    for (int pass = 0; pass < TMT; ++pass) {
        f32x4 av[NA];
        const float* __restrict__ Ag = T.A + (size_t)(row0 + 16 * pass) * T.lda;
#pragma unroll
        for (int i = 0; i < NA; ++i) {
            const int f = min(tid + i * FQL_THREADS, nA - 1);
            const int r = sdiv(f, rk4), kk = f - r * k4;
            av[i] = ldg4(Ag + (size_t)r * T.lda + 4 * kk);
        }
        if (pass == 0) issue_b();
#pragma unroll
        for (int i = 0; i < NA; ++i) {
            const int f = tid + i * FQL_THREADS;
            if (f < nA) {
                const int r = sdiv(f, rk4), kk = f - r * k4;
                *reinterpret_cast<f32x4*>(&lds[(16 * pass + r) * S + 4 * kk]) = av[i];
            }
        }
    }
    }
    STAMP();
    __syncthreads();
    STAMP();
    if (flags & GF_A_LN) {
        const int j = tid & 15;
        const int width = T.ln_width;
        const bool wr = (flags & GF_LN_WRITE) && tn == 0;
#pragma unroll
        for (int pass = 0; pass < TMT; ++pass) {
            const int r = 16 * pass + (tid >> 4);
            float s = 0.f, s2 = 0.f;
            for (int kb = j; kb < width; kb += 128) {
                float xv[8];
#pragma unroll
                for (int i = 0; i < 8; ++i) xv[i] = lds[r * S + min(kb + 16 * i, width - 1)];
#pragma unroll
                for (int i = 0; i < 8; ++i)
                    if (kb + 16 * i < width) { s += xv[i]; s2 += xv[i] * xv[i]; }
            }
#pragma unroll
            for (int o = 1; o < 16; o <<= 1) {
                s += __shfl_xor(s, o);
                s2 += __shfl_xor(s2, o);
            }
            const float inv = 1.0f / (float)width;
            const float mean = s * inv;
            const float var = fmaxf(0.0f, s2 * inv - mean * mean);
            const float rstd = 1.0f / sqrtf(var + 1e-6f);
            for (int kb = j; kb < K; kb += 128) {
                float xv[8], gv[8], bv[8];
#pragma unroll
                for (int i = 0; i < 8; ++i) {
                    const int kc = min(kb + 16 * i, width - 1);
                    gv[i] = ldg(T.ln_g + kc); bv[i] = ldg(T.ln_b + kc);
                    xv[i] = lds[r * S + kc];
                }
#pragma unroll
                for (int i = 0; i < 8; ++i) {
                    const int k = kb + 16 * i;
                    if (k >= K) continue;
                    const float v = (k < width) ? (xv[i] - mean) * rstd * gv[i] + bv[i] : 0.f;
                    lds[r * S + k] = v;
                    if (wr) stg(T.ln_xout + (size_t)(row0 + r) * T.lda + k, v);
                }
            }
            if (wr && j == 0) {
                stg(T.ln_stats + 2 * (row0 + r), mean);
                stg(T.ln_stats + 2 * (row0 + r) + 1, rstd);
            }
        }
        __syncthreads();
    }

    float zpre[TMT][4];
#pragma unroll
    for (int rt = 0; rt < TMT; ++rt)
#pragma unroll
        for (int i = 0; i < 4; ++i) zpre[rt][i] = 0.f;
    if (active && kp == 0 && (flags & (GF_GELUGRAD | GF_RELUGRAD))) {
#pragma unroll
        for (int rt = 0; rt < TMT; ++rt)
#pragma unroll
            for (int i = 0; i < 4; ++i) zpre[rt][i] = ldg(T.Zprev + (size_t)(row0 + 16 * rt + 4 * q + i) * T.ldc + n0 + c);
    }
    f32x4 acc[TMT];
#pragma unroll
    for (int r = 0; r < TMT; ++r) acc[r] = f32x4{0.f, 0.f, 0.f, 0.f};
    if (active) {
        if (transb) gemm_wave<true, TMT>(acc, ba, lds, S, gbeg, gend, c, q, b0, b1);
        else gemm_wave<false, TMT>(acc, ba, lds, S, gbeg, gend, c, q, b0, b1);
    }
    STAMP();
    if (WK > 1) {
        if (kp > 0) {
#pragma unroll
            for (int r = 0; r < TMT; ++r) *reinterpret_cast<f32x4*>(&red[((((kp - 1) * NW + nt) * TMT + r) * 64 + lane) * 4]) = acc[r];
        }
        __syncthreads();
        if (kp > 0 && !head) return;
        if (kp == 0)
        for (int p = 1; p < WK; ++p) {
#pragma unroll
            for (int r = 0; r < TMT; ++r) acc[r] += *reinterpret_cast<const f32x4*>(&red[((((p - 1) * NW + nt) * TMT + r) * 64 + lane) * 4]);
        }
    }
    if (head) {
        if (kp == 0) {
#pragma unroll
            for (int i = 0; i < 4; ++i) hs[(4 * q + i) * 36 + 16 * nt + c] = active ? gelu_f(acc[0][i] + bias) : 0.f;
        }
        __syncthreads();
        if (wave == 0) {
            f32x4 pa = {0.f, 0.f, 0.f, 0.f};
#pragma unroll
            for (int g = 0; g < 2; ++g) {
                const f32x4 a4 = *reinterpret_cast<const f32x4*>(&hs[c * 36 + 16 * g + 4 * q]);
#pragma unroll
                for (int s4 = 0; s4 < 4; ++s4) pa = __builtin_amdgcn_mfma_f32_16x16x4f32(a4[s4], bw4[4 * g + s4], pa, 0, 0, 0);
            }
            if (c < T.i1) {
#pragma unroll
                for (int i = 0; i < 4; ++i) stg(T.evp + ((size_t)tn * T.M + row0 + 4 * q + i) * T.i1 + c, pa[i]);
            }
        }
        return;
    }
    if (!active) return;
    STAMP();

    const int n = n0 + c;
    if (flags & GF_C_FRAGT) {
#pragma unroll
        for (int rt = 0; rt < TMT; ++rt) {
            const int m0 = row0 + 16 * rt;
            float* tb = T.C + ((size_t)(m0 >> 4) * (T.ldc >> 4) + (n >> 4)) * 256 + ((n & 15) >> 2) * 64 + (n & 3);
#pragma unroll
            for (int i = 0; i < 4; ++i) stg(tb + (4 * q + i) * 4, acc[rt][i] + bias);
        }
        return;
    }
    if (flags & GF_C_FRAG) {
#pragma unroll
        for (int rt = 0; rt < TMT; ++rt) {
            f32x4 o;
#pragma unroll
            for (int i = 0; i < 4; ++i) o[i] = acc[rt][i] + bias;
            stg4(T.C + ((size_t)(((row0 + 16 * rt) >> 2) + q) * T.ldc + n) * 4, o);
        }
        return;
    }
#pragma unroll
    for (int rt = 0; rt < TMT; ++rt) {
#pragma unroll
    for (int i = 0; i < 4; ++i) {
        const int row = row0 + 16 * rt + 4 * q + i;
        float v = acc[rt][i] + bias;
        const size_t o = (size_t)row * T.ldc + n;
        if (flags & GF_EULER) {
            float* xr = T.aux + (size_t)row * T.i0 + T.i1;
            if (n < T.i2) {
                const float a = ldg(xr + n) + v * T.f0;
                stg(xr + n, a);
                if (flags & GF_EULER_LAST) stg(T.aux2 + (size_t)row * T.ldc + n, clip1(a));
            }
            if (n == 0 && !(flags & GF_EULER_BARE)) stg(xr + T.i2, T.f1);
            continue;
        }
        if (flags & GF_SAVE_Z) { float gg, dg; gelu_both(v, gg, dg); stg(T.Zout + o, dg); v = (flags & GF_GELU) ? gg : v; }
        else if (flags & GF_GELU) v = gelu_f(v);
        if (flags & GF_GELUGRAD) v *= zpre[rt][i];
        if (flags & GF_RELUGRAD) v = (zpre[rt][i] > 0.f) ? v : 0.f;
        if (flags & GF_CLIP_OUT) v = clip1(v);
        stg(T.C + o, v);
        if ((flags & GF_OS_SCATTER) && n < T.i2) {
            const int B3 = T.M / 3;
            if (row < B3) stg(T.aux + (size_t)row * T.i0 + T.i1 + n, clip1(v));
            else if (row < 2 * B3) stg(T.aux2 + (size_t)(row - B3) * T.i0 + T.i1 + n, clip1(v));
        }
    }
    }
#ifdef FQL_STAMPS
    STAMP();
    if (lane == 0 && wave == 0 && T.aux) {
        unsigned long long* d = reinterpret_cast<unsigned long long*>(T.aux) + (size_t)blockIdx.x * 8;
        for (int i = 0; i < nst; ++i) d[i] = stamp[i];
    }
#endif
}

#ifndef FQL_GEMM_WAVES
#define FQL_GEMM_WAVES 1
#endif
template <bool KBIG>
__global__ __launch_bounds__(FQL_THREADS, FQL_GEMM_WAVES) void fql_gemm16_kernel(const GemmTask* __restrict__ tasks, int ntasks, int tl) {
    extern __shared__ __attribute__((aligned(16))) float lds[];
    tl_enter(tl);
    const GemmTask& T = tasks[find_task(tasks, ntasks, blockIdx.x)];
    if (T.K <= 128) gemm16_body<2, 1, false>(T, lds);
    else if (!KBIG || T.K <= 512) gemm16_body<8, 1, false>(T, lds);
    else gemm16_body<16, 1, false>(T, lds);
    tl_exit(tl);
}
template <bool KBIG>
__global__ __launch_bounds__(FQL_THREADS) void fql_gemm16_euler_kernel(const GemmTask* __restrict__ tasks, int ntasks, int tl) {
    extern __shared__ __attribute__((aligned(16))) float lds[];
    tl_enter(tl);
    const GemmTask& T = tasks[find_task(tasks, ntasks, blockIdx.x)];
    if (T.K <= 128) gemm16_body<2, 1, true>(T, lds);
    else if (!KBIG || T.K <= 512) gemm16_body<8, 1, true>(T, lds);
    else gemm16_body<16, 1, true>(T, lds);
    tl_exit(tl);
}

#define G64_S 68
template <int NR>
__device__ __forceinline__ void ln_fold_partials(const float* __restrict__ partials, int row_first, int ntin, float (&sum)[NR], float (&sumsq)[NR]) {
    const int rs = (2 * ntin + 3) & ~3;
    const int nf4 = (ntin + 1) >> 1;
#pragma unroll
    for (int i = 0; i < NR; ++i) { sum[i] = 0.f; sumsq[i] = 0.f; }
    for (int base = 0; base < nf4; base += 4) {
        f32x4 pv[NR][4];
#pragma unroll
        for (int i = 0; i < NR; ++i) {
            const float* pp = partials + (size_t)(row_first + 16 * i) * rs;
#pragma unroll
            for (int t = 0; t < 4; ++t) pv[i][t] = ldg4(pp + 4 * min(base + t, nf4 - 1));
        }
#pragma unroll
        for (int i = 0; i < NR; ++i)
#pragma unroll
            for (int t = 0; t < 4; ++t) {
                if (2 * (base + t) < ntin) { sum[i] += pv[i][t][0]; sumsq[i] += pv[i][t][1]; }
                if (2 * (base + t) + 1 < ntin) { sum[i] += pv[i][t][2]; sumsq[i] += pv[i][t][3]; }
            }
    }
}

template <bool transb, int RI>
__device__ __forceinline__ void gemm64_body(const GemmTask& T, float* lds) {
    constexpr int TM = 32 * RI;
    float* As = lds;
    float* Bs = lds + 2 * TM * G64_S;
    float* part = Bs + 2 * 64 * G64_S;
    const int local = (int)blockIdx.x - T.tile0;
    const int tm = sdiv(local, frcp(T.ntn)), tn = local - tm * T.ntn;
    const int row0 = tm * TM, n0 = tn * 64;
    const int K = T.K;
    const int tid = threadIdx.x, wave = tid >> 6, lane = tid & 63;
    const int wr = wave >> 1, wc = wave & 1;
    const int c = lane & 15, q = lane >> 4;
    const int flags = T.flags;
    const bool a_ln = (flags & GF_A_LN) != 0;
    const bool ln_wr = (flags & GF_LN_WRITE) && tn == 0;
#ifdef FQL_STAMPS
    unsigned long long stamp[8];
    int nst = 0;
#define GSTAMP() do { __builtin_amdgcn_s_waitcnt(0); stamp[nst++] = __builtin_amdgcn_s_memrealtime(); } while (0)
#else
#define GSTAMP() do {} while (0)
#endif
    GSTAMP();
    const int sr = tid >> 4, sc4 = tid & 15;
    constexpr int NRA = 2 * RI;
    f32x4 ra0[NRA], rb0[4], ra1[NRA], rb1[4], lg0, lb0, lg1, lb1;
    lg0 = lb0 = lg1 = lb1 = f32x4{0.f, 0.f, 0.f, 0.f};
    const float* __restrict__ Ag = T.A + (size_t)(row0 + sr) * T.lda + 4 * sc4;
    const float* __restrict__ Bg = transb ? T.B + (size_t)(n0 + sr) * T.ldb + 4 * sc4 : T.B + (size_t)sr * T.ldb + n0 + 4 * sc4;
    auto load_chunk = [&](f32x4 (&ra)[NRA], f32x4 (&rb)[4], f32x4& lg, f32x4& lb, int k0) {
#pragma unroll
        for (int i = 0; i < NRA; ++i) ra[i] = ldg4(Ag + (size_t)(16 * i) * T.lda + k0);
#pragma unroll
        for (int i = 0; i < 4; ++i) rb[i] = transb ? ldg4(Bg + (size_t)(16 * i) * T.ldb + k0) : ldg4(Bg + (size_t)(k0 + 16 * i) * T.ldb);
        if (a_ln) { lg = ldg4(T.ln_g + k0 + 4 * sc4); lb = ldg4(T.ln_b + k0 + 4 * sc4); }
    };
    const int nchunks = K >> 6;
    load_chunk(ra0, rb0, lg0, lb0, 0);
    if (nchunks > 1) load_chunk(ra1, rb1, lg1, lb1, 64);
    float mean[NRA], rstd[NRA];
#pragma unroll
    for (int i = 0; i < NRA; ++i) { mean[i] = 0.f; rstd[i] = 1.f; }
    if (a_ln) {
        const float inv = 1.0f / (float)T.ln_width;
        float sm[NRA], sq[NRA];
        ln_fold_partials<NRA>(T.aux2, row0 + sr, T.i0, sm, sq);
#pragma unroll
        for (int i = 0; i < NRA; ++i) {
            const int row = row0 + sr + 16 * i;
            mean[i] = sm[i] * inv;
            const float var = fmaxf(0.0f, sq[i] * inv - mean[i] * mean[i]);
            rstd[i] = 1.0f / sqrtf(var + 1e-6f);
            if (ln_wr && sc4 == 0) { stg(T.ln_stats + 2 * row, mean[i]); stg(T.ln_stats + 2 * row + 1, rstd[i]); }
        }
    }
    GSTAMP();
    auto store_chunk = [&](f32x4 (&ra)[NRA], const f32x4 (&rb)[4], const f32x4& lg, const f32x4& lb, int k0, int buf) {
        float* a = As + buf * TM * G64_S;
        float* b = Bs + buf * 64 * G64_S;
        if (a_ln) {
            const int k = k0 + 4 * sc4;
#pragma unroll
            for (int i = 0; i < NRA; ++i) {
#pragma unroll
                for (int e = 0; e < 4; ++e) {
                    const float v = (ra[i][e] - mean[i]) * rstd[i] * lg[e] + lb[e];
                    ra[i][e] = (k + e < T.ln_width) ? v : 0.f;
                }
                if (ln_wr) stg4(T.ln_xout + (size_t)(row0 + sr + 16 * i) * T.lda + k, ra[i]);
            }
        }
#pragma unroll
        for (int i = 0; i < NRA; ++i) *reinterpret_cast<f32x4*>(a + (sr + 16 * i) * G64_S + 4 * sc4) = ra[i];
#pragma unroll
        for (int i = 0; i < 4; ++i) *reinterpret_cast<f32x4*>(b + (sr + 16 * i) * G64_S + 4 * sc4) = rb[i];
    };
    f32x4 acc[RI][2];
#pragma unroll
    for (int i = 0; i < RI; ++i)
#pragma unroll
        for (int j = 0; j < 2; ++j) acc[i][j] = f32x4{0.f, 0.f, 0.f, 0.f};
    const float bias0 = (flags & GF_BIAS) ? ldg(T.bias + n0 + 32 * wc + c) : 0.f;
    const float bias1 = (flags & GF_BIAS) ? ldg(T.bias + n0 + 32 * wc + 16 + c) : 0.f;

    auto compute = [&](int buf) {
        const float* a = As + buf * TM * G64_S + (16 * RI * wr + c) * G64_S + 4 * q;
        const float* b = Bs + buf * 64 * G64_S;
        f32x4 fa[2][RI], fb[2][2];
        auto read_frags = [&](int slot, int g) {
#pragma unroll
            for (int i = 0; i < RI; ++i) fa[slot][i] = *reinterpret_cast<const f32x4*>(a + 16 * i * G64_S + 16 * g);
            if (transb) {
#pragma unroll
                for (int j = 0; j < 2; ++j) fb[slot][j] = *reinterpret_cast<const f32x4*>(b + (32 * wc + 16 * j + c) * G64_S + 16 * g + 4 * q);
            } else {
#pragma unroll
                for (int j = 0; j < 2; ++j)
#pragma unroll
                    for (int s = 0; s < 4; ++s) fb[slot][j][s] = b[(16 * g + 4 * q + s) * G64_S + 32 * wc + 16 * j + c];
            }
        };
        read_frags(0, 0);
#pragma unroll
        for (int g = 0; g < 4; ++g) {
            if (g < 3) read_frags((g + 1) & 1, g + 1);
#pragma unroll
            for (int s = 0; s < 4; ++s)
#pragma unroll
                for (int i = 0; i < RI; ++i)
#pragma unroll
                    for (int j = 0; j < 2; ++j) acc[i][j] = __builtin_amdgcn_mfma_f32_16x16x4f32(fa[g & 1][i][s], fb[g & 1][j][s], acc[i][j], 0, 0, 0);
        }
    };
    store_chunk(ra0, rb0, lg0, lb0, 0, 0);
    if (nchunks > 2) load_chunk(ra0, rb0, lg0, lb0, 128);
    __syncthreads();
    GSTAMP();
#ifdef FQL_STAMPS
    const bool dbg_noload = (flags >> 15) & 1, dbg_nocompute = (flags >> 16) & 1;
#else
    const bool dbg_noload = false, dbg_nocompute = false;
#endif
    for (int ch = 0; ch < nchunks; ch += 2) {
        if (!dbg_nocompute) compute(0);
        if (ch + 1 < nchunks) store_chunk(ra1, rb1, lg1, lb1, 64 * (ch + 1), 1);
        __syncthreads();
        if (ch + 3 < nchunks && !dbg_noload) load_chunk(ra1, rb1, lg1, lb1, 64 * (ch + 3));
        if (ch + 1 < nchunks) {
            if (!dbg_nocompute) compute(1);
            if (ch + 2 < nchunks) store_chunk(ra0, rb0, lg0, lb0, 64 * (ch + 2), 0);
            __syncthreads();
            if (ch + 4 < nchunks && !dbg_noload) load_chunk(ra0, rb0, lg0, lb0, 64 * (ch + 4));
        }
    }

    GSTAMP();
    float s1[RI][4], s2[RI][4];
#pragma unroll
    for (int i = 0; i < RI; ++i) {
#pragma unroll
        for (int r = 0; r < 4; ++r) {
            const int row = row0 + 16 * RI * wr + 16 * i + 4 * q + r;
            s1[i][r] = 0.f; s2[i][r] = 0.f;
#pragma unroll
            for (int j = 0; j < 2; ++j) {
                const int n = n0 + 32 * wc + 16 * j + c;
                const size_t o = (size_t)row * T.ldc + n;
                float v = acc[i][j][r] + (j ? bias1 : bias0);
                if (flags & GF_SAVE_Z) { float gg, dg; gelu_both(v, gg, dg); stg(T.Zout + o, dg); v = (flags & GF_GELU) ? gg : v; }
                else if (flags & GF_GELU) v = gelu_f(v);
                if (flags & GF_GELUGRAD) v *= ldg(T.Zprev + o);
                if (flags & GF_RELUGRAD) v = (ldg(T.Zprev + o) > 0.f) ? v : 0.f;
                stg(T.C + o, v);
                s1[i][r] += v; s2[i][r] += v * v;
            }
        }
    }
    if (flags & GF_LN_PART) {
#pragma unroll
        for (int i = 0; i < RI; ++i)
#pragma unroll
            for (int r = 0; r < 4; ++r) {
                float a = s1[i][r], b = s2[i][r];
#pragma unroll
                for (int o = 1; o < 16; o <<= 1) { a += __shfl_xor(a, o); b += __shfl_xor(b, o); }
                if (c == 0) {
                    const int rl = 16 * RI * wr + 16 * i + 4 * q + r;
                    part[(wc * TM + rl) * 2] = a;
                    part[(wc * TM + rl) * 2 + 1] = b;
                }
            }
        __syncthreads();
        if (tid < 2 * TM) {
            const int half = tid / TM, rl = tid - half * TM;
            float* pp = T.aux + (size_t)(row0 + rl) * ((2 * T.i1 + 3) & ~3) + 2 * (2 * tn + half);
            stg(pp, part[(half * TM + rl) * 2]);
            stg(pp + 1, part[(half * TM + rl) * 2 + 1]);
        }
    }
#ifdef FQL_STAMPS
    GSTAMP();
    if (tid == 0 && T.stamps64) {
        unsigned long long* d = T.stamps64 + (size_t)blockIdx.x * 8;
        for (int i = 0; i < nst; ++i) d[i] = stamp[i];
    }
#endif
}

template <bool transb, int NJ>
__device__ __forceinline__ void gemm32_body(const GemmTask& T, float* lds) {
    constexpr int TN = 32 * NJ;
    constexpr int BS = transb ? G64_S : TN + 4;
    constexpr int BROWS = transb ? TN : 64;
    constexpr int NB = 2 * NJ;
    float* As = lds;
    float* Bs = lds + 2 * 32 * G64_S;
    float* part = Bs + 2 * BROWS * BS;
    const int local = (int)blockIdx.x - T.tile0;
    int tm = sdiv(local, frcp(T.ntn)), tn = local - tm * T.ntn;
    if (T.xg) xcd_tile(local, T.M >> 5, T.ntn, T.xg, tm, tn);
    const int row0 = tm * 32, n0 = tn * TN;
    const int K = T.K;
    const int tid = threadIdx.x, wave = tid >> 6, lane = tid & 63;
    const int wr = wave >> 1, wc = wave & 1;
    const int c = lane & 15, q = lane >> 4;
    const int flags = T.flags;
    const bool a_ln = (flags & GF_A_LN) != 0;
    const bool ln_wr = (flags & GF_LN_WRITE) && tn == 0;
#ifdef FQL_STAMPS
    unsigned long long stamp[8];
    int nst = 0;
#define TSTAMP() do { __builtin_amdgcn_s_waitcnt(0); stamp[nst++] = __builtin_amdgcn_s_memrealtime(); } while (0)
#else
#define TSTAMP() do {} while (0)
#endif
    TSTAMP();
    const int sr = tid >> 4, sc4 = tid & 15;
    const int br0 = (transb || NJ == 2) ? sr : (tid >> 3), brs = (transb || NJ == 2) ? 16 : 32;
    const int bc4 = (transb || NJ == 2) ? sc4 : (tid & 7);
    const float* __restrict__ Ag = T.A + (size_t)(row0 + sr) * T.lda + 4 * sc4;
    const float* __restrict__ Bg = transb ? T.B + (size_t)(n0 + br0) * T.ldb + 4 * bc4 : T.B + (size_t)br0 * T.ldb + n0 + 4 * bc4;
    f32x4 ra0[2], rb0[NB], ra1[2], rb1[NB], lg0, lb0, lg1, lb1;
    lg0 = lb0 = lg1 = lb1 = f32x4{0.f, 0.f, 0.f, 0.f};
    auto load_chunk = [&](f32x4 (&ra)[2], f32x4 (&rb)[NB], f32x4& lg, f32x4& lb, int k0) {
#pragma unroll
        for (int i = 0; i < 2; ++i) ra[i] = ldg4(Ag + (size_t)(16 * i) * T.lda + k0);
#pragma unroll
        for (int i = 0; i < NB; ++i) rb[i] = transb ? ldg4(Bg + (size_t)(brs * i) * T.ldb + k0) : ldg4(Bg + (size_t)(k0 + brs * i) * T.ldb);
        if (a_ln) { lg = ldg4(T.ln_g + k0 + 4 * sc4); lb = ldg4(T.ln_b + k0 + 4 * sc4); }
    };
    const int nchunks = K >> 6;
    load_chunk(ra0, rb0, lg0, lb0, 0);
    if (nchunks > 1) load_chunk(ra1, rb1, lg1, lb1, 64);
    float mean[2] = {0.f, 0.f}, rstd[2] = {1.f, 1.f};
    if (a_ln) {
        const float inv = 1.0f / (float)T.ln_width;
        float sm[2], sq[2];
        ln_fold_partials<2>(T.aux2, row0 + sr, T.i0, sm, sq);
#pragma unroll
        for (int i = 0; i < 2; ++i) {
            mean[i] = sm[i] * inv;
            const float var = fmaxf(0.0f, sq[i] * inv - mean[i] * mean[i]);
            rstd[i] = 1.0f / sqrtf(var + 1e-6f);
            if (ln_wr && sc4 == 0) { const int row = row0 + sr + 16 * i; stg(T.ln_stats + 2 * row, mean[i]); stg(T.ln_stats + 2 * row + 1, rstd[i]); }
        }
    }
    TSTAMP();
    auto store_chunk = [&](f32x4 (&ra)[2], const f32x4 (&rb)[NB], const f32x4& lg, const f32x4& lb, int k0, int buf) {
        float* a = As + buf * 32 * G64_S;
        float* b = Bs + buf * BROWS * BS;
        if (a_ln) {
            const int k = k0 + 4 * sc4;
#pragma unroll
            for (int i = 0; i < 2; ++i) {
#pragma unroll
                for (int e = 0; e < 4; ++e) {
                    const float v = (ra[i][e] - mean[i]) * rstd[i] * lg[e] + lb[e];
                    ra[i][e] = (k + e < T.ln_width) ? v : 0.f;
                }
                if (ln_wr) stg4(T.ln_xout + (size_t)(row0 + sr + 16 * i) * T.lda + k, ra[i]);
            }
        }
#pragma unroll
        for (int i = 0; i < 2; ++i) *reinterpret_cast<f32x4*>(a + (sr + 16 * i) * G64_S + 4 * sc4) = ra[i];
#pragma unroll
        for (int i = 0; i < NB; ++i) *reinterpret_cast<f32x4*>(b + (br0 + brs * i) * BS + 4 * bc4) = rb[i];
    };
    f32x4 acc[NJ][2];
#pragma unroll
    for (int j = 0; j < NJ; ++j) acc[j][0] = acc[j][1] = f32x4{0.f, 0.f, 0.f, 0.f};
    f32x4 bias[NJ];
#pragma unroll
    for (int j = 0; j < NJ; ++j) bias[j] = (flags & GF_BIAS) ? ldg4(T.bias + n0 + (wc * NJ + j) * 16 + 4 * q) : f32x4{0.f, 0.f, 0.f, 0.f};

    auto compute = [&](int buf) {
        const float* a = As + buf * 32 * G64_S + (16 * wr + c) * G64_S + 4 * q;
        const float* b = Bs + buf * BROWS * BS;
        f32x4 fa[2], fb[2][NJ];
        auto read_frags = [&](int slot, int g) {
            fa[slot] = *reinterpret_cast<const f32x4*>(a + 16 * g);
#pragma unroll
            for (int j = 0; j < NJ; ++j) {
                const int col = (wc * NJ + j) * 16 + c;
                if (transb) fb[slot][j] = *reinterpret_cast<const f32x4*>(b + col * BS + 16 * g + 4 * q);
                else {
#pragma unroll
                    for (int s4 = 0; s4 < 4; ++s4) fb[slot][j][s4] = b[(16 * g + 4 * q + s4) * BS + col];
                }
            }
        };
        read_frags(0, 0);
#pragma unroll
        for (int g = 0; g < 4; ++g) {
            if (g < 3) read_frags((g + 1) & 1, g + 1);
#pragma unroll
            for (int s4 = 0; s4 < 4; ++s4)
#pragma unroll
                for (int j = 0; j < NJ; ++j)
                    acc[j][g & 1] = __builtin_amdgcn_mfma_f32_16x16x4f32(fb[g & 1][j][s4], fa[g & 1][s4], acc[j][g & 1], 0, 0, 0);
        }
    };
    store_chunk(ra0, rb0, lg0, lb0, 0, 0);
    if (nchunks > 2) load_chunk(ra0, rb0, lg0, lb0, 128);
    __syncthreads();
    TSTAMP();
    for (int ch = 0; ch < nchunks; ch += 2) {
        compute(0);
        if (ch + 1 < nchunks) store_chunk(ra1, rb1, lg1, lb1, 64 * (ch + 1), 1);
        __syncthreads();
        if (ch + 3 < nchunks) load_chunk(ra1, rb1, lg1, lb1, 64 * (ch + 3));
        if (ch + 1 < nchunks) {
            compute(1);
            if (ch + 2 < nchunks) store_chunk(ra0, rb0, lg0, lb0, 64 * (ch + 2), 0);
            __syncthreads();
            if (ch + 4 < nchunks) load_chunk(ra0, rb0, lg0, lb0, 64 * (ch + 4));
        }
    }
    TSTAMP();

    float s1 = 0.f, s2 = 0.f;
    {
        const int row = row0 + 16 * wr + c;
#pragma unroll
        for (int j = 0; j < NJ; ++j) {
            const int n = n0 + (wc * NJ + j) * 16 + 4 * q;
            const size_t o = (size_t)row * T.ldc + n;
            f32x4 v = acc[j][0] + acc[j][1] + bias[j];
            if (flags & GF_SAVE_Z) {
                f32x4 dgv;
#pragma unroll
                for (int r = 0; r < 4; ++r) { float gg, dg; gelu_both(v[r], gg, dg); dgv[r] = dg; v[r] = (flags & GF_GELU) ? gg : v[r]; }
                stg4(T.Zout + o, dgv);
            } else if (flags & GF_GELU) {
#pragma unroll
                for (int r = 0; r < 4; ++r) v[r] = gelu_f(v[r]);
            }
            if (flags & GF_GELUGRAD) v *= ldg4(T.Zprev + o);
            if (flags & GF_RELUGRAD) {
                const f32x4 zp = ldg4(T.Zprev + o);
#pragma unroll
                for (int r = 0; r < 4; ++r) v[r] = (zp[r] > 0.f) ? v[r] : 0.f;
            }
            stg4(T.C + o, v);
#pragma unroll
            for (int r = 0; r < 4; ++r) { s1 += v[r]; s2 += v[r] * v[r]; }
        }
    }
    if (flags & GF_LN_PART) {
        s1 += __shfl_xor(s1, 16); s2 += __shfl_xor(s2, 16);
        s1 += __shfl_xor(s1, 32); s2 += __shfl_xor(s2, 32);
        if (q == 0) {
            const int rl = 16 * wr + c;
            part[(wc * 32 + rl) * 2] = s1;
            part[(wc * 32 + rl) * 2 + 1] = s2;
        }
        __syncthreads();
        const int rs = (2 * T.i1 + 3) & ~3;
        if (NJ == 2) {
            if (tid < 64) {
                const int half = tid >> 5, rl = tid & 31;
                float* pp = T.aux + (size_t)(row0 + rl) * rs + 2 * (2 * tn + half);
                stg(pp, part[(half * 32 + rl) * 2]);
                stg(pp + 1, part[(half * 32 + rl) * 2 + 1]);
            }
        } else if (tid < 32) {
            float* pp = T.aux + (size_t)(row0 + tid) * rs + 2 * tn;
            stg(pp, part[tid * 2] + part[(32 + tid) * 2]);
            stg(pp + 1, part[tid * 2 + 1] + part[(32 + tid) * 2 + 1]);
        }
    }
#ifdef FQL_STAMPS
    TSTAMP();
    if (tid == 0 && T.stamps64) {
        unsigned long long* d = T.stamps64 + (size_t)blockIdx.x * 8;
        for (int i = 0; i < nst; ++i) d[i] = stamp[i];
    }
#endif
}
#define FQL_TILE_LDS_FLOATS(NJ) (2 * 32 * G64_S + 2 * 64 * G64_S + 128)

template <bool transb, int NJ>
__device__ __forceinline__ void gemm32s_body(const GemmTask& T, float* lds_f) {
    constexpr int TN = 32 * NJ;
    constexpr int RW = TN / 2;
    constexpr int BPL = transb ? TN * 32 : 64 * RW;
    constexpr int APL = 32 * 32;
    constexpr int NB = 2 * NJ;
    unsigned* As = reinterpret_cast<unsigned*>(lds_f);
    unsigned* Bs = As + 4 * APL;
    float* part = reinterpret_cast<float*>(Bs + 4 * BPL);
    const int local = (int)blockIdx.x - T.tile0;
    int tm = sdiv(local, frcp(T.ntn)), tn = local - tm * T.ntn;
    if (T.xg) xcd_tile(local, T.M >> 5, T.ntn, T.xg, tm, tn);
    const int row0 = tm * 32, n0 = tn * TN;
    const int K = T.K;
    const int tid = threadIdx.x, wave = tid >> 6, lane = tid & 63;
    const int wr = wave >> 1, wc = wave & 1;
    const int c = lane & 15, q = lane >> 4;
    const int flags = T.flags;
    const bool a_ln = (flags & GF_A_LN) != 0;
    const bool ln_wr = (flags & GF_LN_WRITE) && tn == 0;
#ifdef FQL_STAMPS
    unsigned long long stamp[8];
    int nst = 0;
#define SSTAMP() do { __builtin_amdgcn_s_waitcnt(0); stamp[nst++] = __builtin_amdgcn_s_memrealtime(); } while (0)
#else
#define SSTAMP() do {} while (0)
#endif
    SSTAMP();
    const int sr = tid >> 4, sc4 = tid & 15;
    const int br0 = (transb || NJ == 2) ? sr : (tid >> 3), brs = (transb || NJ == 2) ? 16 : 32;
    const int bc4 = (transb || NJ == 2) ? sc4 : (tid & 7);
    const float* __restrict__ Ag = T.A + (size_t)(row0 + sr) * T.lda + 4 * sc4;
    const float* __restrict__ Bg = transb ? T.B + (size_t)(n0 + br0) * T.ldb + 4 * bc4 : T.B + (size_t)br0 * T.ldb + n0 + 4 * bc4;
    f32x4 ra0[2], rb0[NB], ra1[2], rb1[NB], lg0, lb0, lg1, lb1;
    lg0 = lb0 = lg1 = lb1 = f32x4{0.f, 0.f, 0.f, 0.f};
    auto load_chunk = [&](f32x4 (&ra)[2], f32x4 (&rb)[NB], f32x4& lg, f32x4& lb, int k0) {
#pragma unroll
        for (int i = 0; i < 2; ++i) ra[i] = ldg4(Ag + (size_t)(16 * i) * T.lda + k0);
#pragma unroll
        for (int i = 0; i < NB; ++i) rb[i] = transb ? ldg4(Bg + (size_t)(brs * i) * T.ldb + k0) : ldg4(Bg + (size_t)(k0 + brs * i) * T.ldb);
        if (a_ln) { lg = ldg4(T.ln_g + k0 + 4 * sc4); lb = ldg4(T.ln_b + k0 + 4 * sc4); }
    };
    const int nchunks = K >> 6;
    load_chunk(ra0, rb0, lg0, lb0, 0);
    if (nchunks > 1) load_chunk(ra1, rb1, lg1, lb1, 64);
    float mean[2] = {0.f, 0.f}, rstd[2] = {1.f, 1.f};
    if (a_ln) {
        const float inv = 1.0f / (float)T.ln_width;
        float sm[2], sq[2];
        ln_fold_partials<2>(T.aux2, row0 + sr, T.i0, sm, sq);
#pragma unroll
        for (int i = 0; i < 2; ++i) {
            mean[i] = sm[i] * inv;
            const float var = fmaxf(0.0f, sq[i] * inv - mean[i] * mean[i]);
            rstd[i] = 1.0f / sqrtf(var + 1e-6f);
            if (ln_wr && sc4 == 0) { const int row = row0 + sr + 16 * i; stg(T.ln_stats + 2 * row, mean[i]); stg(T.ln_stats + 2 * row + 1, rstd[i]); }
        }
    }
    SSTAMP();
    const int st_slot = 4 * (sc4 >> 3) + (sc4 & 3), st_h = (sc4 >> 2) & 1;
    auto rowk_word = [&](int row) { return row * 32 + 4 * (st_slot ^ ((row >> 1) & 7)) + 2 * st_h; };
    auto store_chunk = [&](f32x4 (&ra)[2], const f32x4 (&rb)[NB], const f32x4& lg, const f32x4& lb, int k0, int buf) {
        unsigned* ah = As + buf * 2 * APL;
        unsigned* bh = Bs + buf * 2 * BPL;
        if (a_ln) {
            const int k = k0 + 4 * sc4;
#pragma unroll
            for (int i = 0; i < 2; ++i) {
#pragma unroll
                for (int e = 0; e < 4; ++e) {
                    const float v = (ra[i][e] - mean[i]) * rstd[i] * lg[e] + lb[e];
                    ra[i][e] = (k + e < T.ln_width) ? v : 0.f;
                }
                if (ln_wr) stg4(T.ln_xout + (size_t)(row0 + sr + 16 * i) * T.lda + k, ra[i]);
            }
        }
#pragma unroll
        for (int i = 0; i < 2; ++i) {
            u32x2 hi, lo;
            bsplit4(ra[i], hi, lo);
            const int w = rowk_word(sr + 16 * i);
            *reinterpret_cast<u32x2*>(ah + w) = hi;
            *reinterpret_cast<u32x2*>(ah + APL + w) = lo;
        }
#pragma unroll
        for (int i = 0; i < NB; ++i) {
            u32x2 hi, lo;
            bsplit4(rb[i], hi, lo);
            int w;
            if (transb) w = rowk_word(br0 + brs * i);
            else {
                const int k = br0 + brs * i;
                const int key = (NJ == 2) ? ((k >> 1) & 3) : ((k >> 2) & 1);
                w = k * RW + 8 * ((bc4 >> 2) ^ key) + 2 * (bc4 & 3);
            }
            *reinterpret_cast<u32x2*>(bh + w) = hi;
            *reinterpret_cast<u32x2*>(bh + BPL + w) = lo;
        }
    };
    f32x4 acc[NJ][2];
#pragma unroll
    for (int j = 0; j < NJ; ++j) acc[j][0] = acc[j][1] = f32x4{0.f, 0.f, 0.f, 0.f};
    f32x4 bias[NJ];
#pragma unroll
    for (int j = 0; j < NJ; ++j) bias[j] = (flags & GF_BIAS) ? ldg4(T.bias + n0 + (wc * NJ + j) * 16 + 4 * q) : f32x4{0.f, 0.f, 0.f, 0.f};

    const int a_row = (16 * wr + c) * 32, sw = (c >> 1) & 7;
    const int qq = c >> 2, p = c & 3;
    const int tr_row = 4 * q + qq;
    const int tr_key = (NJ == 2) ? ((tr_row >> 1) & 3) : ((tr_row >> 2) & 1);
    auto compute = [&](int buf) {
        const unsigned* ah = As + buf * 2 * APL;
        const unsigned* bh = Bs + buf * 2 * BPL;
#pragma unroll
        for (int kp = 0; kp < 2; ++kp) {
            const int slot = 4 * ((4 * kp + q) ^ sw);
            const u32x4 fah = *reinterpret_cast<const u32x4*>(ah + a_row + slot);
            const u32x4 fal = *reinterpret_cast<const u32x4*>(ah + APL + a_row + slot);
            u32x4 fbh[NJ], fbl[NJ];
#pragma unroll
            for (int j = 0; j < NJ; ++j) {
                if (transb) {
                    const int brow = ((wc * NJ + j) * 16 + c) * 32;
                    fbh[j] = *reinterpret_cast<const u32x4*>(bh + brow + slot);
                    fbl[j] = *reinterpret_cast<const u32x4*>(bh + BPL + brow + slot);
                } else {
                    const int w0 = (32 * kp + tr_row) * RW + 8 * ((wc * NJ + j) ^ tr_key) + 2 * p;
                    const u32x2 h0 = lds_read_tr16(bh + w0), h1 = lds_read_tr16(bh + w0 + 16 * RW);
                    const u32x2 l0 = lds_read_tr16(bh + BPL + w0), l1 = lds_read_tr16(bh + BPL + w0 + 16 * RW);
                    fbh[j] = u32x4{h0[0], h0[1], h1[0], h1[1]};
                    fbl[j] = u32x4{l0[0], l0[1], l1[0], l1[1]};
                }
            }
#pragma unroll
            for (int j = 0; j < NJ; ++j) acc[j][0] = mfma_bf16(fbh[j], fah, acc[j][0]);
#pragma unroll
            for (int j = 0; j < NJ; ++j) acc[j][1] = mfma_bf16(fbl[j], fah, acc[j][1]);
#pragma unroll
            for (int j = 0; j < NJ; ++j) acc[j][1] = mfma_bf16(fbh[j], fal, acc[j][1]);
        }
    };
    store_chunk(ra0, rb0, lg0, lb0, 0, 0);
    if (nchunks > 2) load_chunk(ra0, rb0, lg0, lb0, 128);
    __syncthreads();
    SSTAMP();
    for (int ch = 0; ch < nchunks; ch += 2) {
        compute(0);
        if (ch + 1 < nchunks) store_chunk(ra1, rb1, lg1, lb1, 64 * (ch + 1), 1);
        __syncthreads();
        if (ch + 3 < nchunks) load_chunk(ra1, rb1, lg1, lb1, 64 * (ch + 3));
        if (ch + 1 < nchunks) {
            compute(1);
            if (ch + 2 < nchunks) store_chunk(ra0, rb0, lg0, lb0, 64 * (ch + 2), 0);
            __syncthreads();
            if (ch + 4 < nchunks) load_chunk(ra0, rb0, lg0, lb0, 64 * (ch + 4));
        }
    }

    SSTAMP();
    float s1 = 0.f, s2 = 0.f;
    {
        const int row = row0 + 16 * wr + c;
#pragma unroll
        for (int j = 0; j < NJ; ++j) {
            const int n = n0 + (wc * NJ + j) * 16 + 4 * q;
            const size_t o = (size_t)row * T.ldc + n;
            f32x4 v = acc[j][0] + acc[j][1] + bias[j];
            if (flags & GF_SAVE_Z) {
                f32x4 dgv;
#pragma unroll
                for (int r = 0; r < 4; ++r) { float gg, dg; gelu_both(v[r], gg, dg); dgv[r] = dg; v[r] = (flags & GF_GELU) ? gg : v[r]; }
                stg4(T.Zout + o, dgv);
            } else if (flags & GF_GELU) {
#pragma unroll
                for (int r = 0; r < 4; ++r) v[r] = gelu_f(v[r]);
            }
            if (flags & GF_GELUGRAD) v *= ldg4(T.Zprev + o);
            if (flags & GF_RELUGRAD) {
                const f32x4 zp = ldg4(T.Zprev + o);
#pragma unroll
                for (int r = 0; r < 4; ++r) v[r] = (zp[r] > 0.f) ? v[r] : 0.f;
            }
            stg4(T.C + o, v);
#pragma unroll
            for (int r = 0; r < 4; ++r) { s1 += v[r]; s2 += v[r] * v[r]; }
        }
    }
    if (flags & GF_LN_PART) {
        s1 += __shfl_xor(s1, 16); s2 += __shfl_xor(s2, 16);
        s1 += __shfl_xor(s1, 32); s2 += __shfl_xor(s2, 32);
        if (q == 0) {
            const int rl = 16 * wr + c;
            part[(wc * 32 + rl) * 2] = s1;
            part[(wc * 32 + rl) * 2 + 1] = s2;
        }
        __syncthreads();
        const int rs = (2 * T.i1 + 3) & ~3;
        if (NJ == 2) {
            if (tid < 64) {
                const int half = tid >> 5, rl = tid & 31;
                float* pp = T.aux + (size_t)(row0 + rl) * rs + 2 * (2 * tn + half);
                stg(pp, part[(half * 32 + rl) * 2]);
                stg(pp + 1, part[(half * 32 + rl) * 2 + 1]);
            }
        } else if (tid < 32) {
            float* pp = T.aux + (size_t)(row0 + tid) * rs + 2 * tn;
            stg(pp, part[tid * 2] + part[(32 + tid) * 2]);
            stg(pp + 1, part[tid * 2 + 1] + part[(32 + tid) * 2 + 1]);
        }
    }
#ifdef FQL_STAMPS
    SSTAMP();
    if (tid == 0 && T.stamps64) {
        unsigned long long* d = T.stamps64 + (size_t)blockIdx.x * 8;
        for (int i = 0; i < nst; ++i) d[i] = stamp[i];
    }
#endif
}
#define FQL_TILE_SPLIT_LDS_FLOATS(NJ) (4 * 32 * 32 + 4 * 32 * 32 * (NJ) + 128)

template <bool BIG, bool SPLIT = false>
__device__ __forceinline__ void gemm_tile_dispatch(const GemmTask& T, float* lds) {
    if (SPLIT) {
        if (T.wk == 2) {
            if (T.flags & GF_TRANS_B) gemm32s_body<true, 2>(T, lds);
            else gemm32s_body<false, 2>(T, lds);
        } else {
            if (T.flags & GF_TRANS_B) gemm32s_body<true, 1>(T, lds);
            else gemm32s_body<false, 1>(T, lds);
        }
        return;
    }
    if (BIG && T.tmt == 2) {
        if (T.flags & GF_TRANS_B) gemm64_body<true, 2>(T, lds);
        else gemm64_body<false, 2>(T, lds);
    } else if (T.wk == 2) {
        if (T.flags & GF_TRANS_B) gemm32_body<true, 2>(T, lds);
        else gemm32_body<false, 2>(T, lds);
    } else {
        if (T.flags & GF_TRANS_B) gemm32_body<true, 1>(T, lds);
        else gemm32_body<false, 1>(T, lds);
    }
}

#define FQL_WGRAD_KT 32
#define FQL_WGRAD_LDS_FLOATS (4 * 8 * 64 * 4 + 4 * 64)
__device__ __forceinline__ void wgrad_load_chunk(f32x2 (&a)[8], f32x4 (&b)[8], const float* xp, const float* zp, unsigned xo, unsigned zo, size_t sx, size_t sz, int cnt) {
#pragma unroll
    for (int i = 0; i < 8; ++i) {
        const bool v = i < cnt;
        a[i] = v ? *(const FQL_GAS f32x2*)(xp + i * sx + xo) : f32x2{0.f, 0.f};
        b[i] = v ? ldg4(zp + i * sz + zo) : f32x4{0.f, 0.f, 0.f, 0.f};
    }
}
template <int NU>
__device__ __forceinline__ void wgrad_finish(const WgradTask& T, float* lds, const f32x4 (&acc)[NU][4], const float (&bs)[4], int tk, int k0, int n0,
                                             int ntv, bool xv) {
    float* red = lds;
    float (*redb)[64] = reinterpret_cast<float (*)[64]>(lds + 4 * 4 * NU * 64 * 4);
    const int wave = threadIdx.x >> 6, lane = threadIdx.x & 63;
    const int c = lane & 15, q = lane >> 4;
#pragma unroll
    for (int t = 0; t < 4; ++t) {
#pragma unroll
        for (int u = 0; u < NU; ++u) *reinterpret_cast<f32x4*>(&red[((wave * 4 * NU + 4 * u + t) * 64 + lane) * 4]) = acc[u][t];
        float v = bs[t];
        v += __shfl_xor(v, 16);
        v += __shfl_xor(v, 32);
        if (q == 0) redb[wave][4 * c + t] = v;
    }
    __syncthreads();
    if (xv && 4 * q + wave < 4 * ntv) {
#pragma unroll
        for (int u = 0; u < NU; ++u) {
            f32x4 r;
#pragma unroll
            for (int t = 0; t < 4; ++t) {
                float v = red[((0 * 4 * NU + 4 * u + t) * 64 + lane) * 4 + wave];
#pragma unroll
                for (int w = 1; w < 4; ++w) v += red[((w * 4 * NU + 4 * u + t) * 64 + lane) * 4 + wave];
                r[t] = v;
            }
            stg4(T.dW + (size_t)(k0 + NU * c + u) * T.ldw + n0 + 16 * q + 4 * wave, r);
        }
    }
    if (tk == 0 && T.db && wave == 0 && lane < 16 * ntv) T.db[n0 + lane] = redb[0][lane] + redb[1][lane] + redb[2][lane] + redb[3][lane];
}
__device__ __forceinline__ void wgrad_body(const WgradTask& T, int bid, float* lds) {
    const int local = bid - T.tile0;
    const int tk = sdiv(local, frcp(T.ntn)), tn = local - tk * T.ntn;
    const int wave = __builtin_amdgcn_readfirstlane(threadIdx.x >> 6), lane = threadIdx.x & 63;
    const int c = lane & 15, q = lane >> 4;
    const int k0 = tk * FQL_WGRAD_KT, n0 = tn * 64;
    const int ntv = min(4, (T.N - n0) >> 4);
    const bool xv = k0 + 2 * c < T.Kin;
    const int steps = T.M >> 4;
    const size_t sx = (size_t)4 * T.ldx, sz = (size_t)4 * T.ldz;
    const float* __restrict__ xp = T.X + (size_t)(4 * wave * steps) * T.ldx;
    const float* __restrict__ zp = T.dZ + (size_t)(4 * wave * steps) * T.ldz;
    const unsigned xo = (unsigned)(q * T.ldx + min(k0 + 2 * c, T.Kin - 2)), zo = (unsigned)(q * T.ldz + n0 + min(4 * c, 16 * ntv - 4));
    f32x4 acc[2][4];
#pragma unroll
    for (int t = 0; t < 4; ++t) acc[0][t] = acc[1][t] = f32x4{0.f, 0.f, 0.f, 0.f};
    float bs[4] = {0.f, 0.f, 0.f, 0.f};
    f32x2 a0[8], a1[8];
    f32x4 b0[8], b1[8];
    auto mma = [&](const f32x2(&a)[8], const f32x4(&b)[8]) {
#pragma unroll
        for (int i = 0; i < 8; ++i)
#pragma unroll
            for (int t = 0; t < 4; ++t) {
                bs[t] += b[i][t];
                acc[0][t] = __builtin_amdgcn_mfma_f32_16x16x4f32(b[i][t], a[i][0], acc[0][t], 0, 0, 0);
                acc[1][t] = __builtin_amdgcn_mfma_f32_16x16x4f32(b[i][t], a[i][1], acc[1][t], 0, 0, 0);
            }
    };
    wgrad_load_chunk(a0, b0, xp, zp, xo, zo, sx, sz, steps);
    for (int s = 0; s < steps; s += 16) {
        if (s + 8 < steps) wgrad_load_chunk(a1, b1, xp + (s + 8) * sx, zp + (s + 8) * sz, xo, zo, sx, sz, steps - s - 8);
        mma(a0, b0);
        if (s + 8 < steps) {
            if (s + 16 < steps) wgrad_load_chunk(a0, b0, xp + (s + 16) * sx, zp + (s + 16) * sz, xo, zo, sx, sz, steps - s - 16);
            mma(a1, b1);
        }
    }
    wgrad_finish<2>(T, lds, acc, bs, tk, k0, n0, ntv, xv);
}
#define FQL_WGRAD_KT_SPLIT 16
__device__ __forceinline__ void wgrad_split_body(const WgradTask& T, int bid, float* lds) {
    const int local = bid - T.tile0;
    const int tk = sdiv(local, frcp(T.ntn)), tn = local - tk * T.ntn;
    const int wave = __builtin_amdgcn_readfirstlane(threadIdx.x >> 6), lane = threadIdx.x & 63;
    const int c = lane & 15, q = lane >> 4;
    const int k0 = tk * FQL_WGRAD_KT_SPLIT, n0 = tn * 64;
    const int ntv = min(4, (T.N - n0) >> 4);
    const bool zv = c < 4 * ntv;
    const int steps = T.M >> 4;
    const size_t sx = (size_t)4 * T.ldx, sz = (size_t)4 * T.ldz;
    const float* __restrict__ xp = T.X + (size_t)(4 * wave * steps) * T.ldx;
    const float* __restrict__ zp = T.dZ + (size_t)(4 * wave * steps) * T.ldz;
    const unsigned xo = (unsigned)(q * T.ldx + k0 + c), zo = (unsigned)(q * T.ldz + n0 + min(4 * c, 16 * ntv - 4));
    f32x4 acc[1][4];
#pragma unroll
    for (int t = 0; t < 4; ++t) acc[0][t] = f32x4{0.f, 0.f, 0.f, 0.f};
    float bs[4] = {0.f, 0.f, 0.f, 0.f};
    float a0[8], a1[8];
    f32x4 b0[8], b1[8];
    auto load = [&](float (&a)[8], f32x4 (&b)[8], int s0) {
#pragma unroll
        for (int i = 0; i < 8; ++i) {
            const int st = min(s0 + i, steps - 1);
            a[i] = ldg(xp + st * sx + xo);
            b[i] = ldg4(zp + st * sz + zo);
        }
    };
    auto mma = [&](const float (&a)[8], const f32x4 (&b)[8], int s0) {
        float av[8];
#pragma unroll
        for (int i = 0; i < 8; ++i) av[i] = (s0 + i < steps) ? a[i] : 0.f;
        u32x4 ah, al;
#pragma unroll
        for (int i = 0; i < 4; ++i) { unsigned h, l; bsplit2(av[2 * i], av[2 * i + 1], h, l); ah[i] = h; al[i] = l; }
#pragma unroll
        for (int t = 0; t < 4; ++t) {
            u32x4 bh, bl;
#pragma unroll
            for (int i = 0; i < 4; ++i) {
                unsigned h, l;
                const float b0v = (s0 + 2 * i < steps && zv) ? b[2 * i][t] : 0.f;
                const float b1v = (s0 + 2 * i + 1 < steps && zv) ? b[2 * i + 1][t] : 0.f;
                bs[t] += b0v + b1v;
                bsplit2(b0v, b1v, h, l);
                bh[i] = h; bl[i] = l;
            }
            acc[0][t] = mfma_bf16(bh, al, acc[0][t]);
            acc[0][t] = mfma_bf16(bl, ah, acc[0][t]);
            acc[0][t] = mfma_bf16(bh, ah, acc[0][t]);
            __builtin_amdgcn_sched_barrier(0);
        }
    };
    load(a0, b0, 0);
    for (int s = 0; s < steps; s += 16) {
        if (s + 8 < steps) load(a1, b1, s + 8);
        mma(a0, b0, s);
        if (s + 8 < steps) {
            if (s + 16 < steps) load(a0, b0, s + 16);
            mma(a1, b1, s + 8);
        }
    }
    wgrad_finish<1>(T, lds, acc, bs, tk, k0, n0, ntv, true);
}

template <bool SYN>
__device__ __forceinline__ void lnbwd_body(const LnBwdTask& T, int bid, float (*red)[16][16]) {
    const int local = bid - T.tile0;
    const int wave = threadIdx.x >> 6, lane = threadIdx.x & 63;
    if (local < T.ntiles_rows) {
        const int row = local * 4 + wave;
        if (row >= T.M) return;
        const float mean = ldg(T.stats + 2 * row), rstd = ldg(T.stats + 2 * row + 1);
        const float* dy = T.dY + (size_t)row * T.ld;
        const float* z = T.Z + (size_t)row * T.ld;
        const float* gv = T.Gv + (size_t)row * T.ld;
        const float dqr = SYN ? ldg(T.dq + (size_t)row * T.ldq) : 0.f;
        f32x4 zz[4], dd[4], gm[4], gq[4];
#pragma unroll
        for (int i = 0; i < 4; ++i) {
            const int k4 = 4 * (lane + 64 * i);
            if (k4 < T.H) {
                zz[i] = ldg4(z + k4);
                gq[i] = ldg4(gv + k4);
                gm[i] = ldg4(T.gamma + k4);
                if (SYN) {
#pragma unroll
                    for (int e = 0; e < 4; ++e) dd[i][e] = dqr * ldg(T.wq + (size_t)(k4 + e) * T.ldw);
                } else dd[i] = ldg4(dy + k4);
            } else zz[i] = gq[i] = gm[i] = dd[i] = f32x4{0.f, 0.f, 0.f, 0.f};
        }
        f32x4 d[4], xh[4];
        float s1 = 0.f, s2 = 0.f;
#pragma unroll
        for (int i = 0; i < 4; ++i)
#pragma unroll
            for (int e = 0; e < 4; ++e) {
                const int k = 4 * (lane + 64 * i) + e;
                xh[i][e] = (gq[i][e] - mean) * rstd;
                d[i][e] = dd[i][e] * gm[i][e];
                if (k < T.width) { s1 += d[i][e]; s2 += d[i][e] * xh[i][e]; }
            }
#pragma unroll
        for (int o = 1; o < 64; o <<= 1) {
            s1 += __shfl_xor(s1, o);
            s2 += __shfl_xor(s2, o);
        }
        const float inv = 1.0f / (float)T.width;
        const float m1 = s1 * inv, m2 = s2 * inv;
        float* dz = T.dZ + (size_t)row * T.ld;
#pragma unroll
        for (int i = 0; i < 4; ++i) {
            const int k4 = 4 * (lane + 64 * i);
            if (k4 < T.H) {
                f32x4 o;
#pragma unroll
                for (int e = 0; e < 4; ++e) o[e] = (k4 + e < T.width) ? rstd * (d[i][e] - m1 - xh[i][e] * m2) * zz[i][e] : 0.f;
                stg4(dz + k4, o);
            }
        }
    } else {
        const int cc = threadIdx.x & 15, rg = threadIdx.x >> 4;
        const int col = (local - T.ntiles_rows) * 16 + cc;
        float sg = 0.f, sb = 0.f;
        if (col < T.width) {
            const float wc = SYN ? ldg(T.wq + (size_t)col * T.ldw) : 0.f;
            for (int m0 = rg; m0 < T.M; m0 += 256) {
                f32x2 st[16];
                float dv[16], zv[16];
#pragma unroll
                for (int u = 0; u < 16; ++u) {
                    const int m = min(m0 + 16 * u, T.M - 1);
                    st[u] = *(const FQL_GAS f32x2*)(T.stats + 2 * m);
                    dv[u] = SYN ? ldg(T.dq + (size_t)m * T.ldq) * wc : ldg(T.dY + (size_t)m * T.ld + col);
                    zv[u] = ldg(T.Gv + (size_t)m * T.ld + col);
                }
#pragma unroll
                for (int u = 0; u < 16; ++u) {
                    if (m0 + 16 * u < T.M) {
                        const float xh = (zv[u] - st[u][0]) * st[u][1];
                        sg += dv[u] * xh; sb += dv[u];
                    }
                }
            }
        }
        red[0][rg][cc] = sg; red[1][rg][cc] = sb;
        __syncthreads();
        if (rg == 0 && col < T.H) {
            float g = 0.f, b = 0.f;
#pragma unroll
            for (int r = 0; r < 16; ++r) { g += red[0][r][cc]; b += red[1][r][cc]; }
            stg(T.dgamma + col, (col < T.width) ? g : 0.f);
            stg(T.dbeta + col, (col < T.width) ? b : 0.f);
        }
    }
}

struct DevState {
    uint64_t rng_step;
    uint64_t rng_stream;
    int64_t adam_count;
    int64_t train_step;
    double b1pow, b2pow;
    float grad_scale;
    float lam;
    float info[16];
    float gmax_bits_pad;
    int gmax, gmin;
    float leaf_sumsq[256];
};

struct SrcDesc {
    const float *obs, *act, *rew, *mask, *nobs;
    const int64_t* idx;
    const float *eps1, *x0, *t, *z, *eps2;
    int64_t lo, span;
    int use_rng_idx;
    int advance;
    int split;
    const float *obs2, *act2, *rew2, *mask2, *nobs2;
    int64_t lo2, span2;
    const float* nact;
    int64_t nact_rows;
};

struct PrepArgs {
    const SrcDesc* src;
    DevState* st;
    uint64_t key;
    int B, od, ad;
    int inp_c, inp_b;
    int ap;
    float *X_os, *X_bc, *X_eu, *X_c1, *X_c2, *X_ct, *vel, *w_rew, *w_mask, *w_act;
    float* X_e0;
    const float *E_c, *E_t, *E_bc, *E_os;
    int tl;
    int part;
};

__device__ __forceinline__ void fql_prep_body(const PrepArgs& P) {
    tl_enter(P.tl);
    const SrcDesc& S = *P.src;
    const int wave = threadIdx.x >> 6, lane = threadIdx.x & 63;
    const int b = blockIdx.x * 4 + wave;
    if (b >= P.B) return;
    const uint64_t step = P.st->rng_step;
    const uint64_t key = P.key ^ (P.st->rng_stream * 0x9E3779B97F4A7C15ull);
    int64_t src = b;
    const bool second = S.split > 0 && b >= S.split;
    if (S.idx) src = S.idx[b];
    else if (S.use_rng_idx) {
        const uint64_t u = rng_u32(key, step, 7u, (uint32_t)b);
        src = second ? S.lo2 + (int64_t)((u * (uint64_t)S.span2) >> 32) : S.lo + (int64_t)((u * (uint64_t)S.span) >> 32);
    }
    const int od = P.od, ad = P.ad, B = P.B;
    const bool vis = P.E_c != nullptr;
    const float* obs = vis ? nullptr : (second ? S.obs2 : S.obs) + (size_t)src * od;
    const float* nobs = vis ? nullptr : (second ? S.nobs2 : S.nobs) + (size_t)src * od;
    const float* act = (second ? S.act2 : S.act) + (size_t)src * ad;
    const float tt = S.t ? S.t[b] : rng_uniform(key, step, 3u, (uint32_t)b);
    const int maxw = P.inp_c > P.inp_b ? P.inp_c : P.inp_b;
    for (int j = lane; j < maxw; j += 64) {
        const bool is_obs = j < od, is_act = (j >= od) && (j < od + ad);
        const int a = j - od;
        float o = 0.f, no = 0.f, av = 0.f, e1 = 0.f, e2 = 0.f, zz = 0.f, xx = 0.f;
        float o_c, o_bc, o_os, no_os, no_t;
        if (is_obs && !vis) { o = obs[j]; no = nobs[j]; }
        o_c = o_bc = o_os = o; no_os = no_t = no;
        if (is_obs && vis) {
            const size_t r = (size_t)b * od + j;
            o_c = P.E_c[r]; o_bc = P.E_bc[r]; no_t = P.E_t[r];
            o_os = P.E_os[r]; no_os = P.E_os[(size_t)B * od + r];
        }
        if (is_act) {
            av = act[a];
            e1 = S.eps1 ? S.eps1[(size_t)b * ad + a] : rng_normal(key, step, 1u, (uint32_t)b, (uint32_t)a);
            xx = S.x0 ? S.x0[(size_t)b * ad + a] : rng_normal(key, step, 2u, (uint32_t)b, (uint32_t)a);
            zz = S.z ? S.z[(size_t)b * ad + a] : rng_normal(key, step, 4u, (uint32_t)b, (uint32_t)a);
            e2 = S.eps2 ? S.eps2[(size_t)b * ad + a] : rng_normal(key, step, 5u, (uint32_t)b, (uint32_t)a);
        }
        if (j < P.inp_c && P.part != 1) {
            const size_t w = P.inp_c;
            P.X_os[(size_t)b * w + j] = is_obs ? no_os : e1;
            P.X_os[(size_t)(B + b) * w + j] = is_obs ? o_os : zz;
            P.X_os[(size_t)(2 * B + b) * w + j] = is_obs ? o_os : e2;
            P.X_c1[(size_t)b * w + j] = is_obs ? o_c : av;
            P.X_c2[(size_t)b * w + j] = is_obs ? o_c : 0.f;
            P.X_ct[(size_t)b * w + j] = is_obs ? no_t : 0.f;
        }
        if (j < P.inp_b) {
            const size_t w = P.inp_b;
            const float xt = (1.0f - tt) * xx + tt * av;
            if (P.part != 1) P.X_bc[(size_t)b * w + j] = is_obs ? o_bc : (is_act ? xt : (j == od + ad ? tt : 0.f));
            if (P.part != 2) {
                P.X_eu[(size_t)b * w + j] = is_obs ? o_bc : (is_act ? zz : 0.f);
                if (P.X_e0) P.X_e0[(size_t)b * w + j] = is_obs ? o_bc : 0.f;
            }
        }
        if (is_act && P.part != 1) {
            P.vel[(size_t)b * P.ap + a] = av - xx;
            P.w_act[(size_t)b * P.ap + a] = av;
        }
    }
    if (lane == 0 && P.part != 1) {
        P.w_rew[b] = (second ? S.rew2 : S.rew)[src];
        P.w_mask[b] = (second ? S.mask2 : S.mask)[src];
    }
}
__global__ __launch_bounds__(FQL_THREADS) void fql_prep_kernel(PrepArgs P) { fql_prep_body(P); }
__global__ __launch_bounds__(FQL_THREADS) void fql_prep_multi_kernel(const PrepArgs* __restrict__ args) { const PrepArgs P = ((const FQL_CONST_AS PrepArgs*)args)[blockIdx.y]; fql_prep_body(P); }

__device__ __forceinline__ float block_sum(float v, float* sh) {
#pragma unroll
    for (int o = 1; o < 64; o <<= 1) v += __shfl_xor(v, o);
    __syncthreads();
    if ((threadIdx.x & 63) == 0) sh[threadIdx.x >> 6] = v;
    __syncthreads();
    return sh[0] + sh[1] + sh[2] + sh[3];
}
__device__ __forceinline__ float block_max(float v, float* sh) {
#pragma unroll
    for (int o = 1; o < 64; o <<= 1) v = fmaxf(v, __shfl_xor(v, o));
    __syncthreads();
    if ((threadIdx.x & 63) == 0) sh[threadIdx.x >> 6] = v;
    __syncthreads();
    return fmaxf(fmaxf(sh[0], sh[1]), fmaxf(sh[2], sh[3]));
}

struct PostOsArgs {
    const float* A_os;
    const float* w_act;
    float *X_ct, *X_c2;
    DevState* st;
    int B, od, ad, inp_c, ap;
};
__device__ __forceinline__ void fql_post_onestep_body(const PostOsArgs& P, float* sh) {
    float se = 0.f;
    const int n = P.B * P.ad;
    for (int e = threadIdx.x; e < n; e += FQL_THREADS) {
        const int b = sdiv(e, frcp(P.ad)), a = e - b * P.ad;
        const float d = clip1(P.A_os[(size_t)(2 * P.B + b) * P.ap + a]) - P.w_act[(size_t)b * P.ap + a];
        se += d * d;
    }
    const float tot = block_sum(se, sh);
    if (threadIdx.x == 0) P.st->info[9] = tot / (float)n;
}

struct LossCriticArgs {
    const float *q1a, *q1b, *tqa, *tqb;
    const float *w_rew, *w_mask;
    float *dq1a, *dq1b;
    DevState* st;
    int B, q_agg, want_grad;
    float discount;
};
__device__ __forceinline__ void fql_loss_critic_body(const LossCriticArgs& P, float* sh) {
    float sl = 0.f, sq = 0.f, mx = -INFINITY, mn = INFINITY;
    const float gs = 1.0f / (float)P.B;
    for (int b = threadIdx.x; b < P.B; b += FQL_THREADS) {
        const float ta = P.tqa[(size_t)b * 16], tb = P.tqb[(size_t)b * 16];
        const float nq = P.q_agg ? fminf(ta, tb) : 0.5f * (ta + tb);
        const float y = P.w_rew[b] + P.discount * P.w_mask[b] * nq;
        const float qa = P.q1a[(size_t)b * 16], qb = P.q1b[(size_t)b * 16];
        const float da = qa - y, db = qb - y;
        sl += da * da + db * db;
        sq += qa + qb;
        mx = fmaxf(mx, fmaxf(qa, qb));
        mn = fminf(mn, fminf(qa, qb));
        if (P.want_grad) {
            P.dq1a[(size_t)b * 16] = da * gs;
            P.dq1b[(size_t)b * 16] = db * gs;
        }
    }
    const float tl = block_sum(sl, sh), tq = block_sum(sq, sh);
    const float tmx = block_max(mx, sh), tmn = -block_max(-mn, sh);
    if (threadIdx.x == 0) {
        const float inv = 1.0f / (2.0f * (float)P.B);
        P.st->info[0] = tl * inv;
        P.st->info[1] = tq * inv;
        P.st->info[2] = tmx;
        P.st->info[3] = tmn;
    }
}

struct LossQArgs {
    const float *q2a, *q2b;
    float *dq2a, *dq2b;
    DevState* st;
    int B, normalize, want_grad;
};
__device__ __forceinline__ void fql_loss_q_body(const LossQArgs& P, float* sh) {
    float s = 0.f, sa = 0.f;
    for (int b = threadIdx.x; b < P.B; b += FQL_THREADS) {
        const float q = 0.5f * (P.q2a[(size_t)b * 16] + P.q2b[(size_t)b * 16]);
        s += q; sa += fabsf(q);
    }
    const float ts = block_sum(s, sh), tsa = block_sum(sa, sh);
    const float qmean = ts / (float)P.B;
    const float lam = P.normalize ? 1.0f / (tsa / (float)P.B) : 1.0f;
    if (P.want_grad) {
        const float g = -lam / (2.0f * (float)P.B);
        for (int b = threadIdx.x; b < P.B; b += FQL_THREADS) {
            P.dq2a[(size_t)b * 16] = g;
            P.dq2b[(size_t)b * 16] = g;
        }
    }
    if (threadIdx.x == 0) {
        P.st->info[7] = lam * (-qmean);
        P.st->info[8] = qmean;
        P.st->lam = lam;
    }
}

struct LossBcArgs {
    const float *pred, *vel;
    float* dpred;
    DevState* st;
    int B, ad, ap, want_grad;
};
__device__ __forceinline__ void fql_loss_bc_body(const LossBcArgs& P, float* sh) {
    const int n = P.B * P.ad;
    const float gs = 2.0f / (float)n;
    float s = 0.f;
    for (int e = threadIdx.x; e < n; e += FQL_THREADS) {
        const int b = sdiv(e, frcp(P.ad)), a = e - b * P.ad;
        const float d = P.pred[(size_t)b * P.ap + a] - P.vel[(size_t)b * P.ap + a];
        s += d * d;
        if (P.want_grad) P.dpred[(size_t)b * P.ap + a] = gs * d;
    }
    const float t = block_sum(s, sh);
    if (threadIdx.x == 0) P.st->info[5] = t / (float)n;
}

struct LossActorArgs {
    const float* a_raw;
    const float* tgt;
    const float *dxa, *dxb;
    float* da;
    DevState* st;
    int B, od, ad, inp_c, ap, want_grad;
    float alpha;
};
__device__ __forceinline__ void fql_loss_actor_body(const LossActorArgs& P, float* sh) {
    const int n = P.B * P.ad;
    const float gs = P.alpha * 2.0f / (float)n;
    float s = 0.f;
    for (int e = threadIdx.x; e < n; e += FQL_THREADS) {
        const int b = sdiv(e, frcp(P.ad)), a = e - b * P.ad;
        const float ar = P.a_raw[(size_t)b * P.ap + a];
        const float d = ar - P.tgt[(size_t)b * P.ap + a];
        s += d * d;
        if (P.want_grad) {
            float g = gs * d;
            if (ar > -1.0f && ar < 1.0f) {
                const size_t o = (size_t)b * P.inp_c + P.od + a;
                g += P.dxa[o] + P.dxb[o];
            }
            P.da[(size_t)b * P.ap + a] = g;
        }
    }
    const float t = block_sum(s, sh);
    if (threadIdx.x == 0) {
        const float distill = t / (float)n;
        P.st->info[6] = distill;
        P.st->info[4] = P.st->info[5] + P.alpha * distill + P.st->info[7];
    }
}

__global__ __launch_bounds__(FQL_THREADS) void fql_loss_actor_kernel(LossActorArgs P) { __shared__ float sh[4]; fql_loss_actor_body(P, sh); }
__global__ __launch_bounds__(FQL_THREADS) void fql_loss_actor_multi_kernel(const LossActorArgs* __restrict__ args) { __shared__ float sh[4]; const LossActorArgs P = args[blockIdx.y]; fql_loss_actor_body(P, sh); }

enum : int { MISC_POSTOS = 0, MISC_LOSS_CRITIC, MISC_LOSS_Q, MISC_LOSS_BC };
struct MiscTask {
    int kind;
    union {
        PostOsArgs po;
        LossCriticArgs lc;
        LossQArgs lq;
        LossBcArgs lb;
    };
};

struct AdamChunk { int off, len, leaf; };
struct FinalizeArgs {
    DevState* st;
    const AdamChunk* chunks;
    const float* partials;
    const int* leaf_range;
    int n_chunks, nleaves, do_grad_stats;
    int tl;
};
struct AdamArgs {
    float *P, *G, *Mu, *Nu, *T;
    const AdamChunk* chunks;
    DevState* st;
    float* partials;
    int chunk0;
    int critic_size;
    float lr, tau;
    int tl;
    int n0, chunk1;
    unsigned* ticket;
    int ticket_n;
    FinalizeArgs fin;
};
__device__ __forceinline__ int f2ord(float f) {
    const int i = __float_as_int(f);
    return i >= 0 ? i : i ^ 0x7FFFFFFF;
}
__device__ __forceinline__ float ord2f(int i) { return __int_as_float(i >= 0 ? i : i ^ 0x7FFFFFFF); }

template <bool SC1>
__device__ __forceinline__ float ld_partial(const float* p) {
    if constexpr (SC1) return __hip_atomic_load((FQL_GAS float*)p, __ATOMIC_RELAXED, __HIP_MEMORY_SCOPE_AGENT);
    else return *p;
}
template <bool SC1>
__device__ __forceinline__ void fql_finalize_core(const FinalizeArgs& A, float* sh, float* leafn) {
    DevState* st = A.st;
    if (!A.do_grad_stats) return;
    float mx = -INFINITY, mn = INFINITY;
    for (int c0 = threadIdx.x; c0 < A.n_chunks; c0 += 4 * FQL_THREADS) {
        float vx[4], vn[4];
#pragma unroll
        for (int j = 0; j < 4; ++j) {
            const int cidx = c0 + j * FQL_THREADS;
            vx[j] = cidx < A.n_chunks ? ld_partial<SC1>(A.partials + 4 * cidx + 1) : -INFINITY;
            vn[j] = cidx < A.n_chunks ? ld_partial<SC1>(A.partials + 4 * cidx + 2) : INFINITY;
        }
#pragma unroll
        for (int j = 0; j < 4; ++j) { mx = fmaxf(mx, vx[j]); mn = fminf(mn, vn[j]); }
    }
    for (int base = 0; base < A.nleaves; base += 64) {
        const int l = base + (threadIdx.x >> 2), sub = threadIdx.x & 3;
        float s = 0.f;
        if (l < A.nleaves) {
            const int b = A.leaf_range[l], e = A.leaf_range[l + 1];
            const int per = (e - b + 3) >> 2;
            const int lo = b + sub * per, hi = min(e, lo + per);
            for (int c0 = lo; c0 < hi; c0 += 8) {
                float v[8];
#pragma unroll
                for (int j = 0; j < 8; ++j) v[j] = c0 + j < hi ? ld_partial<SC1>(A.partials + 4 * (c0 + j)) : 0.f;
#pragma unroll
                for (int j = 0; j < 8; ++j) if (c0 + j < hi) s += v[j];
            }
        }
        s += __shfl_xor(s, 1);
        s += __shfl_xor(s, 2);
        if (l < A.nleaves && sub == 0) leafn[l] = sqrtf(s);
    }
    const float tmx = block_max(mx, sh), tmn = -block_max(-mn, sh);
    __syncthreads();
    if (threadIdx.x == 0) {
        float nrm = 0.f;
        for (int i = 0; i < A.nleaves; ++i) nrm += leafn[i];
        st->info[10] = fmaxf(tmx, 0.0f);
        st->info[11] = fminf(tmn, 0.0f);
        st->info[12] = nrm;
        st->rng_step += 1;
        st->adam_count += 1;
        st->train_step += 1;
        st->b1pow *= 0.9;
        st->b2pow *= 0.999;
    }
}

__device__ __forceinline__ void fql_adam_body(const AdamArgs& A) {
    __shared__ float sh[4];
    __shared__ float leafn[256];
    tl_enter(A.tl);
    const int cidx = (A.n0 < 0 || (int)blockIdx.x < A.n0) ? (int)blockIdx.x + A.chunk0 : (int)blockIdx.x - A.n0 + A.chunk1;
    const AdamChunk ch = A.chunks[cidx];
    const float c1 = (float)(1.0 - A.st->b1pow * 0.9), c2 = (float)(1.0 - A.st->b2pow * 0.999);
    const float gsc = A.st->grad_scale;
    float ss = 0.f, mx = -INFINITY, mn = INFINITY;
    const int n4 = ch.len >> 2;
#pragma unroll
    for (int it = 0; it < 4; ++it) {
        const int i = threadIdx.x + it * FQL_THREADS;
        if (i < n4) {
            const int o = ch.off + 4 * i;
            f32x4 g = ldg4(A.G + o);
            const f32x4 p = ldg4(A.P + o);
            f32x4 m = ldg4(A.Mu + o);
            f32x4 v = ldg4(A.Nu + o);
            f32x4 pn;
#pragma unroll
            for (int e = 0; e < 4; ++e) {
                const float ge = g[e] * gsc;
                m[e] = 0.9f * m[e] + 0.1f * ge;
                v[e] = 0.999f * v[e] + 0.001f * ge * ge;
                const float mh = m[e] / c1, vh = v[e] / c2;
                pn[e] = p[e] - A.lr * (mh / (sqrtf(vh) + 1e-8f));
                ss += ge * ge; mx = fmaxf(mx, ge); mn = fminf(mn, ge);
            }
            stg4(A.Mu + o, m);
            stg4(A.Nu + o, v);
            stg4(A.P + o, pn);
            if (o < A.critic_size) {
                f32x4 t = ldg4(A.T + o);
#pragma unroll
                for (int e = 0; e < 4; ++e) t[e] = p[e] * A.tau + t[e] * (1.0f - A.tau);
                stg4(A.T + o, t);
            }
        }
    }
    const float tss = block_sum(ss, sh);
    const float tmx = block_max(mx, sh), tmn = -block_max(-mn, sh);
    float* pp = A.partials + 4 * (size_t)cidx;
    if (!A.ticket) {
        if (threadIdx.x == 0) { pp[0] = tss; pp[1] = tmx; pp[2] = tmn; }
        tl_exit(A.tl);
        return;
    }
    if (threadIdx.x == 0) {
        const u32x4 v = {__float_as_uint(tss), __float_as_uint(tmx), __float_as_uint(tmn), 0u};
        __builtin_amdgcn_raw_buffer_store_b128(v, __builtin_amdgcn_make_buffer_rsrc(pp, 0, 16, 0x00020000), 0, 0, 16);
        asm volatile("s_waitcnt vmcnt(0)" ::: "memory");
        const unsigned t = __hip_atomic_fetch_add((FQL_GAS unsigned*)A.ticket, 1u, __ATOMIC_RELAXED, __HIP_MEMORY_SCOPE_AGENT);
        sh[0] = t == (unsigned)(A.ticket_n - 1) ? 1.0f : 0.0f;
    }
    __syncthreads();
    const bool last = sh[0] != 0.0f;
    if (last) {
        fql_finalize_core<true>(A.fin, sh, leafn);
        if (threadIdx.x == 0) __hip_atomic_store((FQL_GAS unsigned*)A.ticket, 0u, __ATOMIC_RELAXED, __HIP_MEMORY_SCOPE_AGENT);
    }
    tl_exit(A.tl);
}
__global__ __launch_bounds__(FQL_THREADS) void fql_adam_kernel(AdamArgs A) { fql_adam_body(A); }
__global__ __launch_bounds__(FQL_THREADS) void fql_adam_multi_kernel(const AdamArgs* __restrict__ args) { const AdamArgs A = ((const FQL_CONST_AS AdamArgs*)args)[blockIdx.y]; fql_adam_body(A); }

__device__ __forceinline__ void fql_finalize_body(const FinalizeArgs& A) {
    __shared__ float sh[4];
    __shared__ float leafn[256];
    tl_enter(A.tl);
    fql_finalize_core<false>(A, sh, leafn);
}
__global__ __launch_bounds__(FQL_THREADS) void fql_finalize_kernel(FinalizeArgs A) { fql_finalize_body(A); }
__global__ __launch_bounds__(FQL_THREADS) void fql_finalize_multi_kernel(const FinalizeArgs* __restrict__ args) { const FinalizeArgs A = args[blockIdx.y]; fql_finalize_body(A); }

struct EulerFinishArgs {
    const float* a_in;
    const float* evp;
    const float* eb;
    float* tgt;
    int M, ad, ap, ntp, a_ld;
    float scale;
};
__device__ __forceinline__ void fql_euler_finish_body(const EulerFinishArgs& P) {
    const int e = blockIdx.x * FQL_THREADS + threadIdx.x;
    if (e >= P.M * P.ad) return;
    const int r = sdiv(e, frcp(P.ad)), j = e - r * P.ad;
    float pv[32];
#pragma unroll
    for (int tp = 0; tp < 32; ++tp) pv[tp] = ldg(P.evp + ((size_t)min(tp, P.ntp - 1) * P.M + r) * P.ap + j);
    float sum = 0.f;
#pragma unroll
    for (int tp = 0; tp < 32; ++tp) sum += (tp < P.ntp) ? pv[tp] : 0.f;
    stg(P.tgt + (size_t)r * P.ap + j, clip1(ldg(P.a_in + (size_t)r * P.a_ld + j) + (sum + ldg(P.eb + j)) * P.scale));
}
__global__ __launch_bounds__(FQL_THREADS) void fql_euler_finish_kernel(EulerFinishArgs P) { fql_euler_finish_body(P); }
__global__ __launch_bounds__(FQL_THREADS) void fql_euler_finish_multi_kernel(const EulerFinishArgs* __restrict__ args) { const EulerFinishArgs P = args[blockIdx.y]; fql_euler_finish_body(P); }

struct EncDzArgs {
    const float *dxa, *dxb;
    const float* z;
    float* dz;
    int M, n, ld;
};
__global__ __launch_bounds__(FQL_THREADS) void fql_enc_dz_kernel(const EncDzArgs P) {
    const int e = blockIdx.x * FQL_THREADS + threadIdx.x;
    if (e >= P.M * P.n) return;
    const int r = e / P.n, j = e - r * P.n;
    float g = ldg(P.dxa + (size_t)r * P.ld + j);
    if (P.dxb) g += ldg(P.dxb + (size_t)r * P.ld + j);
    stg(P.dz + e, g * ldg(P.z + e));
}

struct AssembleArgs {
    const float *obs, *noise;
    float* X;
    uint64_t key, seed;
    int n, n_pad, od, ad, inp;
};
__device__ __forceinline__ void fql_assemble_body(const AssembleArgs& P) {
    const int wave = threadIdx.x >> 6, lane = threadIdx.x & 63;
    const int b = blockIdx.x * 4 + wave;
    if (b >= P.n_pad) return;
    for (int j = lane; j < P.inp; j += 64) {
        float v = 0.f;
        if (b < P.n) {
            if (j < P.od) v = P.obs[(size_t)b * P.od + j];
            else if (j < P.od + P.ad) {
                const int a = j - P.od;
                v = P.noise ? P.noise[(size_t)b * P.ad + a] : rng_normal(P.key, P.seed, 9u, (uint32_t)b, (uint32_t)a);
            }
        }
        P.X[(size_t)b * P.inp + j] = v;
    }
}
__global__ __launch_bounds__(FQL_THREADS) void fql_assemble_kernel(AssembleArgs P) { fql_assemble_body(P); }
__device__ __forceinline__ void fql_extract_body(const float* src, float* out, int n, int ad, int ap) {
    const int e = blockIdx.x * blockDim.x + threadIdx.x;
    if (e < n * ad) out[e] = src[(size_t)(e / ad) * ap + (e % ad)];
}
__global__ void fql_extract_kernel(const float* src, float* out, int n, int ad, int ap) { fql_extract_body(src, out, n, ad, ap); }
__global__ void fql_dataset_add_kernel(float* obs, float* act, float* rew, float* mask, float* nobs,
                                       const float* row, int64_t pos, int od, int ad) {
    const int j = threadIdx.x;
    if (j < od) { obs[pos * od + j] = row[j]; nobs[pos * od + j] = row[od + ad + 2 + j]; }
    if (j < ad) act[pos * ad + j] = row[od + j];
    if (j == 0) { rew[pos] = row[od + ad]; mask[pos] = row[od + ad + 1]; }
}

#ifndef FQL_SIDE_WAVES
#define FQL_SIDE_WAVES 3
#endif
#ifndef FQL_SIDE_VGPRS
#define FQL_SIDE_VGPRS 168
#endif
template <bool BIG, bool SPLIT = false>
__device__ __forceinline__ void side_body(const GemmTask* __restrict__ gt, int ngt, const WgradTask* __restrict__ wt, int nwt, const LnBwdTask* __restrict__ lt,
                                          int nlt, int tile_w, int tile_l, const MiscTask* __restrict__ mt, int tile_m) {
    extern __shared__ __attribute__((aligned(16))) float lds[];
    const int b = blockIdx.x;
    if (b < tile_w) {
        gemm_tile_dispatch<BIG, SPLIT>(gt[find_task(gt, ngt, b)], lds);
    } else if (b < tile_l) {
        const int bid = b - tile_w;
        if (SPLIT) wgrad_split_body(wt[find_task(wt, nwt, bid)], bid, lds);
        else wgrad_body(wt[find_task(wt, nwt, bid)], bid, lds);
    } else if (b < tile_m) {
        const int bid = b - tile_l;
        const LnBwdTask& T = lt[find_task(lt, nlt, bid)];
        float (*red)[16][16] = reinterpret_cast<float (*)[16][16]>(lds);
        if (T.dq) lnbwd_body<true>(T, bid, red);
        else lnbwd_body<false>(T, bid, red);
    } else {
        const MiscTask& T = mt[b - tile_m];
        switch (T.kind) {
            case MISC_POSTOS: fql_post_onestep_body(T.po, lds); break;
            case MISC_LOSS_CRITIC: fql_loss_critic_body(T.lc, lds); break;
// ... 94 lines not shown
```

Baseline: 2981.

## Drop interior AQL acquire fences by routing in-step reads through L1-bypassing loads

```diff
diff --git a/fql_amd/csrc/fql_chain.h b/fql_amd/csrc/fql_chain.h
--- a/fql_amd/csrc/fql_chain.h
+++ b/fql_amd/csrc/fql_chain.h
@@ -60,7 +60,7 @@
         if (j >= (T.K >> 5)) return;
         float v[8];
 #pragma unroll
-        for (int i = 0; i < 8; ++i) { const int k = 32 * j + 8 * q + i; v[i] = (k < T.kvalid) ? ldg(T.src + (size_t)k * T.ld + n) : 0.f; }
+        for (int i = 0; i < 8; ++i) { const int k = 32 * j + 8 * q + i; v[i] = (k < T.kvalid) ? ldx(T.src + (size_t)k * T.ld + n) : 0.f; }
         u32x4 hi, lo;
 #pragma unroll
         for (int i = 0; i < 4; ++i) { unsigned h, l; bsplit2(v[2 * i], v[2 * i + 1], h, l); hi[i] = h; lo[i] = l; }
@@ -74,7 +74,7 @@
         if (k4 >= (T.K >> 2)) return;
         float v[4];
 #pragma unroll
-        for (int i = 0; i < 4; ++i) v[i] = (4 * k4 + i < T.kvalid) ? ldg(T.src + (size_t)(4 * k4 + i) * T.ld + n) : 0.f;
+        for (int i = 0; i < 4; ++i) v[i] = (4 * k4 + i < T.kvalid) ? ldx(T.src + (size_t)(4 * k4 + i) * T.ld + n) : 0.f;
         unsigned h0, l0, h1, l1;
         bsplit2(v[0], v[1], h0, l0);
         bsplit2(v[2], v[3], h1, l1);
@@ -85,7 +85,7 @@
     if (k4 >= (T.K >> 2)) return;
     f32x4 v;
 #pragma unroll
-    for (int s = 0; s < 4; ++s) v[s] = (4 * k4 + s < T.kvalid) ? ldg(T.src + (size_t)(4 * k4 + s) * T.ld + n) : 0.f;
+    for (int s = 0; s < 4; ++s) v[s] = (4 * k4 + s < T.kvalid) ? ldx(T.src + (size_t)(4 * k4 + s) * T.ld + n) : 0.f;
     stg4(T.dst + ((size_t)k4 * T.N + n) * 4, v);
 }
 
@@ -130,7 +130,7 @@
             for (int g = 0; g < GQ; ++g) bf[g] = ldg4(wb + (size_t)g * 16 * H);
         }
     }
-    const float bias = variant == 4 ? 0.f : variant == 3 ? ldg(P.Zprev + (size_t)(row0 + 4 * q + kp) * H + n0 + c) : ldg(P.bias + n0 + c);
+    const float bias = variant == 4 ? 0.f : variant == 3 ? ldx(P.Zprev + (size_t)(row0 + 4 * q + kp) * H + n0 + c) : ldg(P.bias + n0 + c);
     f32x4 bw4[2];
     if (variant == 2 && wave == 0) {
 #pragma unroll
@@ -141,7 +141,7 @@
 #pragma unroll
         for (int t = 0; t < CT; ++t) {
             const int ct = wave + 8 * t;
-            cacc[t] = ldg4(P.A + ((size_t)((row0 >> 2) + q) * H + 16 * ct + c) * 4);
+            cacc[t] = ldx4(P.A + (size_t)(row0 >> 2) * H * 4, (unsigned)((q * H + 16 * ct + c) * 4));
             wf[t] = ldg4(P.W0f + ((size_t)q * H + 16 * ct + c) * 4);
         }
         {
@@ -149,12 +149,12 @@
             const int r = e >> 4, j = e & 15;
             float a = 0.f;
             if (j < P.ad) {
-                a = ldg(P.ea_in + (size_t)(row0 + r) * P.ea_ld + j);
+                a = ldx(P.ea_in + (size_t)(row0 + r) * P.ea_ld + j);
                 if (P.evp_in) {
                     float pv[NT / 2];
                     const float* pp = P.evp_in + ((size_t)(half * (NT / 2)) * P.M + row0 + r) * P.ap + j;
 #pragma unroll
-                    for (int tp = 0; tp < NT / 2; ++tp) pv[tp] = ldg(pp + (size_t)tp * P.M * P.ap);
+                    for (int tp = 0; tp < NT / 2; ++tp) pv[tp] = ldx(pp + (size_t)tp * P.M * P.ap);
                     float sum = 0.f;
 #pragma unroll
                     for (int tp = 0; tp < NT / 2; ++tp) sum += pv[tp];
@@ -197,14 +197,15 @@
 #pragma unroll
         for (int r = 0; r < 2; ++r) {
             const size_t row = (size_t)(row0 + 2 * wave + r);
-            mean[r] = ldg(P.stats + 2 * row); rstd[r] = ldg(P.stats + 2 * row + 1);
-            const float dqr = P.A ? 0.f : ldg(P.dq + row * P.ldq);
+            mean[r] = ldx(P.stats + 2 * row); rstd[r] = ldx(P.stats + 2 * row + 1);
+            const float dqr = P.A ? 0.f : ldx(P.dq + row * P.ldq);
 #pragma unroll
             for (int i = 0; i < NV; ++i) {
                 const int k4 = 4 * (lane + 64 * i);
-                zz[r][i] = ldg4(P.Zprev + row * H + k4);
-                gq[r][i] = ldg4(P.Gv + row * H + k4);
-                if (P.A) dy[r][i] = ldg4(P.A + row * H + k4);
+                const unsigned ro = (unsigned)((2 * wave + r) * H + k4);
+                zz[r][i] = ldx4(P.Zprev + (size_t)row0 * H, ro);
+                gq[r][i] = ldx4(P.Gv + (size_t)row0 * H, ro);
+                if (P.A) dy[r][i] = ldx4(P.A + (size_t)row0 * H, ro);
                 else dy[r][i] = f32x4{dqr * wqv[i][0], dqr * wqv[i][1], dqr * wqv[i][2], dqr * wqv[i][3]};
             }
         }
@@ -236,7 +237,7 @@
         f32x4 av[NA];
         const float* Ag = P.A + (size_t)row0 * H;
 #pragma unroll
-        for (int i = 0; i < NA; ++i) av[i] = ldg4(Ag + (size_t)(tid + i * FQL_CHAIN_THREADS) * 4);
+        for (int i = 0; i < NA; ++i) av[i] = ldx4(Ag, (unsigned)(tid + i * FQL_CHAIN_THREADS) * 4);
 #pragma unroll
         for (int i = 0; i < NA; ++i) {
             const int f = tid + i * FQL_CHAIN_THREADS;
@@ -311,13 +312,14 @@
     const int ti = (int)blockIdx.x / ntm, tm = (int)blockIdx.x - ti * ntm;
     const GemmTask& T = P.t[ti];
     const int row0 = tm * 16, kq = T.K >> 2;
-    const float* ap = T.A + (size_t)(row0 + c) * T.lda + kp * kq + 4 * q;
+    const float* ap = T.A + (size_t)row0 * T.lda;
+    const unsigned ao = (unsigned)(c * T.lda + kp * kq + 4 * q);
     const float* bp = T.B + (size_t)(P.col0 + c) * T.ldb + kp * kq + 4 * q;
     f32x4 acc = {0.f, 0.f, 0.f, 0.f}, acc2 = {0.f, 0.f, 0.f, 0.f};
     for (int g0 = 0; g0 < kq; g0 += 128) {
         f32x4 a[8], b[8];
 #pragma unroll
-        for (int g = 0; g < 8; ++g) { a[g] = ldg4(ap + g0 + 16 * g); b[g] = ldg4(bp + g0 + 16 * g); }
+        for (int g = 0; g < 8; ++g) { a[g] = ldx4(ap, ao, (unsigned)(g0 + 16 * g)); b[g] = ldg4(bp + g0 + 16 * g); }
 #pragma unroll
         for (int g = 0; g < 8; g += 2)
 #pragma unroll
@@ -346,27 +348,27 @@
     const f32x4 b4 = ldg4(T.B + (size_t)(n0 + c) * T.ldb + 4 * q);
     float zp[4];
 #pragma unroll
-    for (int i = 0; i < 4; ++i) zp[i] = ldg(T.Zprev + (size_t)(row0 + 4 * q + i) * T.ldc + n0 + c);
+    for (int i = 0; i < 4; ++i) zp[i] = ldx(T.Zprev + (size_t)(row0 + 4 * q + i) * T.ldc + n0 + c);
     {
         const int r = tid >> 4, j = tid & 15;
         float g = 0.f;
         if (j < T.i2) {
-            const float ar = ldg(T.ea_in + (size_t)(row0 + r) * T.i0 + j);
+            const float ar = ldx(T.ea_in + (size_t)(row0 + r) * T.i0 + j);
             float tg;
             if (T.flags & GF_A_EULFIN) {
                 float pv[32];
 #pragma unroll
-                for (int tp = 0; tp < 32; ++tp) pv[tp] = ldg(T.aux2 + ((size_t)min(tp, T.ln_width - 1) * T.M + row0 + r) * T.i0 + j);
+                for (int tp = 0; tp < 32; ++tp) pv[tp] = ldx(T.aux2 + ((size_t)min(tp, T.ln_width - 1) * T.M + row0 + r) * T.i0 + j);
                 float sum = 0.f;
 #pragma unroll
                 for (int tp = 0; tp < 32; ++tp) sum += (tp < T.ln_width) ? pv[tp] : 0.f;
-                tg = clip1(ldg(T.aux + (size_t)(row0 + r) * T.i0 + j) + (sum + ldg(T.eb + j)) * T.f1);
+                tg = clip1(ldx(T.aux + (size_t)(row0 + r) * T.i0 + j) + (sum + ldg(T.eb + j)) * T.f1);
                 if (tn == 0) stg(const_cast<float*>(T.evp) + (size_t)(row0 + r) * T.i0 + j, tg);
-            } else tg = ldg(T.evp + (size_t)(row0 + r) * T.i0 + j);
+            } else tg = ldx(T.evp + (size_t)(row0 + r) * T.i0 + j);
             g = T.f0 * (ar - tg);
             if (ar > -1.0f && ar < 1.0f) {
                 const size_t o = (size_t)(row0 + r) * T.e_ntp + T.i1 + j;
-                g += ldg(T.ew + o) + ldg(T.ew4 + o);
+                g += ldx(T.ew + o) + ldx(T.ew4 + o);
             }
             if (tn == 0 && T.ea_out) stg(T.ea_out + (size_t)(row0 + r) * T.i0 + j, g);
         }
@@ -436,7 +438,7 @@
 #pragma unroll
         for (int t = 0; t < CT; ++t) {
             const int ct = wave + 8 * t;
-            cacc[t] = ldg4(P.A + (((size_t)(row0 >> 4) * (H / 16) + ct) * 64 + 16 * q + c) * 4);
+            cacc[t] = ldx4(P.A + (size_t)(row0 >> 4) * (H / 16) * 256, (unsigned)((ct * 64 + 16 * q + c) * 4));
             wf[t] = ldg4u(reinterpret_cast<const unsigned*>(P.W0f) + ((size_t)q * H + 16 * ct + c) * 4);
         }
         {
@@ -444,12 +446,12 @@
             const int r = e >> 4, j = e & 15;
             float a = 0.f;
             if (j < P.ad) {
-                a = ldg(P.ea_in + (size_t)(row0 + r) * P.ea_ld + j);
+                a = ldx(P.ea_in + (size_t)(row0 + r) * P.ea_ld + j);
                 if (P.evp_in) {
                     float pv[NT / 2];
                     const float* pp = P.evp_in + ((size_t)(half * (NT / 2)) * P.M + row0 + r) * P.ap + j;
 #pragma unroll
-                    for (int tp = 0; tp < NT / 2; ++tp) pv[tp] = ldg(pp + (size_t)tp * P.M * P.ap);
+                    for (int tp = 0; tp < NT / 2; ++tp) pv[tp] = ldx(pp + (size_t)tp * P.M * P.ap);
                     float sum = 0.f;
 #pragma unroll
                     for (int tp = 0; tp < NT / 2; ++tp) sum += pv[tp];
@@ -495,7 +497,7 @@
 #pragma unroll
         for (int i = 0; i < NA; ++i) {
             const int pc = (tid + i * FQL_CHAIN_THREADS) & (4 * RS - 1);
-            av[i] = ldg4u((i < NA / 2 ? Ah : Al) + (size_t)pc * 4);
+            av[i] = ldx4u(i < NA / 2 ? Ah : Al, (unsigned)pc * 4);
         }
 #pragma unroll
         for (int i = 0; i < NA; ++i) {
diff --git a/fql_amd/csrc/fql_engine.hip b/fql_amd/csrc/fql_engine.hip
--- a/fql_amd/csrc/fql_engine.hip
+++ b/fql_amd/csrc/fql_engine.hip
@@ -237,6 +237,31 @@
 inline bool fused_tail_env() {
     const char* e = getenv("FQL_FUSED_TAIL");
     return !e || atoi(e) != 0;
+}
+inline bool aql_acquire_env() {
+    const char* e = getenv("FQL_AQL_ACQUIRE");
+    return e && atoi(e) != 0;
+}
+inline bool l1_independent_kernel(const void* fn) {
+#define FQL_L1_CHAIN(HH)                                                                                                                             \
+    (const void*)fql_chain_kernel<HH, 0>, (const void*)fql_chain_kernel<HH, 1>, (const void*)fql_chain_kernel<HH, 2>, (const void*)fql_chain_kernel<HH, 3>, \
+    (const void*)fql_chain_multi_kernel<HH, 0>, (const void*)fql_chain_multi_kernel<HH, 1>, (const void*)fql_chain_multi_kernel<HH, 2>,             \
+    (const void*)fql_chain_multi_kernel<HH, 3>, (const void*)fql_chain_split_kernel<HH, 0>, (const void*)fql_chain_split_kernel<HH, 1>,             \
+    (const void*)fql_chain_split_kernel<HH, 2>
+    static const void* const table[] = {
+        (const void*)fql_prep_kernel, (const void*)fql_prep_multi_kernel,
+        (const void*)fql_gemm16_kernel<false>, (const void*)fql_gemm16_kernel<true>,
+        (const void*)fql_gemm16_euler_kernel<false>, (const void*)fql_gemm16_euler_kernel<true>,
+        (const void*)fql_side_kernel, (const void*)fql_side_ka_kernel, (const void*)fql_side_big_kernel, (const void*)fql_side_big_ka_kernel,
+        (const void*)fql_side_split_kernel, (const void*)fql_side_split_ka_kernel,
+        FQL_L1_CHAIN(256), FQL_L1_CHAIN(512),
+        (const void*)fql_dgrad0_kernel, (const void*)fql_dgrad0_multi_kernel, (const void*)fql_head_dgrad_kernel, (const void*)fql_head_dgrad_multi_kernel,
+        (const void*)fql_loss_actor_kernel, (const void*)fql_loss_actor_multi_kernel,
+        (const void*)fql_euler_finish_kernel, (const void*)fql_euler_finish_multi_kernel,
+        (const void*)fql_adam_kernel, (const void*)fql_adam_multi_kernel, (const void*)fql_wfrag_kernel};
+#undef FQL_L1_CHAIN
+    for (const void* k : table) if (k == fn) return true;
+    return false;
 }
 inline std::unique_ptr<SideArgs> ka_side_args(const Launch& L) {
     const size_t ng = L.h_gemm.size(), nw = L.h_wgrad.size(), nl = L.h_ln.size(), nm = L.h_misc.size();
@@ -2095,6 +2120,43 @@
         fprintf(stderr, "[fql] launches per lane:");
         for (int l = 0; l < FQL_LANES; ++l) fprintf(stderr, " %d", cnt[l]);
         fprintf(stderr, "\n");
+        dump_in_update_reads(pr);
+    }
+    void dump_in_update_reads(const Program& pr) const {
+        auto member = [](const Op& o, const void* p) -> std::string {
+            std::string s;
+            auto add = [&](const char* n, const void* q) { if (q == p) { if (!s.empty()) s += '/'; s += n; } };
+            if (o.type == OP_GEMM || o.type == OP_GEMM64 || o.type == OP_HEAD_DGRAD) {
+                const GemmTask& t = o.gemm;
+                add("A", t.A); add("B", t.B); add("bias", t.bias); add("Zprev", t.Zprev); add("aux", t.aux); add("aux2", t.aux2); add("ln_g", t.ln_g);
+                add("ln_b", t.ln_b); add("ea_in", t.ea_in); add("evp", t.evp); add("ew", t.ew); add("ew4", t.ew4); add("eb", t.eb);
+            } else if (o.type == OP_WGRAD) {
+                add("X", o.wgrad.X); add("dZ", o.wgrad.dZ);
+            } else if (o.type == OP_LNBWD) {
+                const LnBwdTask& t = o.ln;
+                add("dY", t.dY); add("Z", t.Z); add("Gv", t.Gv); add("stats", t.stats); add("gamma", t.gamma); add("dq", t.dq); add("wq", t.wq);
+            }
+            return s;
+        };
+        std::map<const void*, int> writer;
+        size_t oi = 0;
+        for (int li = 0; li < (int)pr.launches.size(); ++li) {
+            std::string line;
+            std::vector<const Op*> mine;
+            for (const Op& o : pr.ops) if (o.launch == li) mine.push_back(&o);
+            for (const Op* o : mine)
+                for (size_t ri = 0; ri < o->reads.size(); ++ri) {
+                    auto it = writer.find(o->reads[ri]);
+                    if (it == writer.end()) continue;
+                    char b[96];
+                    const std::string m = member(*o, o->reads[ri]);
+                    snprintf(b, sizeof b, " t%d.%s%s<-#%d", (int)o->type, m.empty() ? "r" : m.c_str(), m.empty() ? std::to_string(ri).c_str() : "", it->second);
+                    line += b;
+                }
+            for (const Op* o : mine) for (const void* w : o->writes) writer[w] = li;
+            fprintf(stderr, "[fql] #%2d type %2d in-update reads:%s\n", li, (int)pr.launches[li].type, line.empty() ? " none" : line.c_str());
+        }
+        (void)oi;
     }
     static void check_lane_edges(const Program& pr) {
         bool edge[FQL_LANES][FQL_LANES] = {};
@@ -2143,6 +2205,12 @@
         return out;
     }
 
+    const bool aql_acquire = aql_acquire_env();
+    static bool l1_independent(const Program& pr) {
+        for (const Launch& L : pr.launches)
+            if (!l1_independent_kernel(L.k.fn) || L.type == OP_IQLD_CFG) return false;
+        return !pr.launches.empty();
+    }
     void build_aql(Program& pr) {
         static const bool off = getenv("FQL_AQL") && atoi(getenv("FQL_AQL")) == 0;
         static const bool trace_a = getenv("FQL_TRACE") != nullptr;
@@ -2181,6 +2249,7 @@
             int endsig[FQL_AQL_LANES];
             for (int l = 1; l < FQL_AQL_LANES; ++l) endsig[l] = used[l] ? nsig++ : AQL_SIG_NONE;
             constexpr int AG = HSA_FENCE_SCOPE_AGENT, SY = HSA_FENCE_SCOPE_SYSTEM, NO = HSA_FENCE_SCOPE_NONE;
+            const int interior = l1_independent(pr) && !aql_acquire ? NO : AG;
             for (int l = 1; l < FQL_AQL_LANES; ++l)
                 if (used[l]) {
                     AqlPacket b = AqlRuntime::barrier_packet(false, NO, NO);
@@ -2195,7 +2264,7 @@
                     for (size_t j = 0; j < 5 && w0 + j < L.waits.size(); ++j) b.deps[j] = sig[L.waits[w0 + j]];
                     ap.lane[L.lane].push_back(b);
                 }
-                AqlPacket k = AqlRuntime::kernel_packet(rec[i], *ki[i], (uint64_t)(uintptr_t)kargs + koff[i], true, first[L.lane] ? SY : AG, AG);
+                AqlPacket k = AqlRuntime::kernel_packet(rec[i], *ki[i], (uint64_t)(uintptr_t)kargs + koff[i], true, first[L.lane] ? SY : interior, AG);
                 first[L.lane] = false;
                 k.complete = sig[i];
                 ap.lane[L.lane].push_back(k);
@@ -6085,6 +6154,36 @@
     return FQL_OK;
 }
 
+int fql_debug_aql_fences(fql_handle h, fql_group g, void* out, size_t bytes) {
+    if ((!h && !g) || (bytes && !out) || bytes % sizeof(int32_t)) return FQL_E_INVALID;
+    if (!g && (h->visual || !h->prog_full.exec || h->prog_full.launches.empty())) return FQL_E_STATE;
+    std::vector<int32_t> w{0, 0, 0, 0};
+    if (g) {
+        bool all = !g->launches.empty();
+        for (const GLaunch& G : g->launches) all = all && l1_independent_kernel(G.k.fn);
+        w[1] = all;
+        w[2] = g->m.empty() ? 0 : (int32_t)g->m[0]->aql_acquire;
+    } else {
+        w[1] = fql_engine::l1_independent(h->prog_full);
+        w[2] = h->aql_acquire;
+        const AqlProgram& ap = h->prog_full.aql;
+        if (ap.ok)
+            for (int l = 0; l < FQL_AQL_LANES; ++l)
+                for (const AqlPacket& p : ap.lane[l]) {
+                    if (p.barrier) continue;
+                    const uint32_t hdr = p.w[0] & 0xFFFFu;
+                    w.push_back(l);
+                    w.push_back((int32_t)((hdr >> HSA_PACKET_HEADER_SCACQUIRE_FENCE_SCOPE) & 3u));
+                    w.push_back((int32_t)((hdr >> HSA_PACKET_HEADER_SCRELEASE_FENCE_SCOPE) & 3u));
+                }
+    }
+    w[3] = ((int32_t)w.size() - 4) / 3;
+    w[0] = (int32_t)w.size();
+    if (bytes > w.size() * sizeof(int32_t)) return FQL_E_INVALID;
+    if (bytes) std::memcpy(out, w.data(), bytes);
+    return FQL_OK;
+}
+
 int fql_group_destroy(fql_group g) {
     if (!g) return FQL_OK;
     g->release();
diff --git a/fql_amd/csrc/fql_kernels.h b/fql_amd/csrc/fql_kernels.h
--- a/fql_amd/csrc/fql_kernels.h
+++ b/fql_amd/csrc/fql_kernels.h
@@ -7,6 +7,22 @@
 #define FQL_GAS __attribute__((address_space(1)))
 __device__ __forceinline__ float ldg(const float* p) { return *(const FQL_GAS float*)p; }
 __device__ __forceinline__ f32x4 ldg4(const float* p) { return *(const FQL_GAS f32x4*)p; }
+typedef unsigned u32x4 __attribute__((ext_vector_type(4)));
+__device__ __forceinline__ __amdgpu_buffer_rsrc_t ldx_rsrc(const void* base) {
+    const uint64_t b = (uint64_t)base;
+    const uint64_t u = ((uint64_t)(unsigned)__builtin_amdgcn_readfirstlane((int)(b >> 32)) << 32) | (unsigned)__builtin_amdgcn_readfirstlane((int)b);
+    return __builtin_amdgcn_make_buffer_rsrc((void*)u, 0, 0x7FFFFFFF, 0x00020000);
+}
+__device__ __forceinline__ float ldx(const float* p) { return __hip_atomic_load((const FQL_GAS float*)p, __ATOMIC_RELAXED, __HIP_MEMORY_SCOPE_AGENT); }
+__device__ __forceinline__ u32x4 ldx4u(const unsigned* base, unsigned i, unsigned s = 0) {
+    return __builtin_amdgcn_raw_buffer_load_b128(ldx_rsrc(base), (int)(i * 4u), __builtin_amdgcn_readfirstlane((int)(s * 4u)), 16);
+}
+typedef float f32x2 __attribute__((ext_vector_type(2)));
+typedef unsigned u32x2 __attribute__((ext_vector_type(2)));
+__device__ __forceinline__ f32x2 ldx2(const float* base, unsigned i, unsigned s = 0) {
+    return __builtin_bit_cast(f32x2, __builtin_amdgcn_raw_buffer_load_b64(ldx_rsrc(base), (int)(i * 4u), __builtin_amdgcn_readfirstlane((int)(s * 4u)), 16));
+}
+__device__ __forceinline__ f32x4 ldx4(const float* base, unsigned i, unsigned s = 0) { return __builtin_bit_cast(f32x4, ldx4u((const unsigned*)base, i, s)); }
 __device__ __forceinline__ void stg(float* p, float v) { *(FQL_GAS float*)p = v; }
 __device__ __forceinline__ void stg4(float* p, f32x4 v) { *(FQL_GAS f32x4*)p = v; }
 
@@ -514,7 +530,7 @@
         for (int t = 0; t < CT; ++t) {
             const int ct = min(wave + 4 * t, (K >> 4) - 1);
 #pragma unroll
-            for (int i = 0; i < 4; ++i) cacc[t][i] = ldg(T.A + (size_t)(row0 + 4 * q + i) * T.lda + 16 * ct + c);
+            for (int i = 0; i < 4; ++i) cacc[t][i] = ldx(T.A + (size_t)(row0 + 4 * q + i) * T.lda + 16 * ct + c);
 #pragma unroll
             for (int s4 = 0; s4 < 4; ++s4) wf[t][s4] = ldg(T.ew + (size_t)(4 * q + s4) * K + 16 * ct + c);
         }
@@ -522,11 +538,11 @@
             const int r = e >> 4, j = e & 15;
             float a = 0.f;
             if (j < ad) {
-                a = ldg(T.ea_in + (size_t)(row0 + r) * T.i0 + j);
+                a = ldx(T.ea_in + (size_t)(row0 + r) * T.i0 + j);
                 if (T.evp) {
                     float pv[32];
 #pragma unroll
-                    for (int tp = 0; tp < 32; ++tp) pv[tp] = ldg(T.evp + ((size_t)min(tp, T.e_ntp - 1) * M + row0 + r) * apw + j);
+                    for (int tp = 0; tp < 32; ++tp) pv[tp] = ldx(T.evp + ((size_t)min(tp, T.e_ntp - 1) * M + row0 + r) * apw + j);
                     float sum = 0.f;
 #pragma unroll
                     for (int tp = 0; tp < 32; ++tp) sum += (tp < T.e_ntp) ? pv[tp] : 0.f;
@@ -558,22 +574,22 @@
             const int r = sdiv(e, frcp(K)), j = e - r * K;
             float g = 0.f;
             if (j < T.i2) {
-                const float ar = ldg(T.ea_in + (size_t)(row0 + r) * T.i0 + j);
+                const float ar = ldx(T.ea_in + (size_t)(row0 + r) * T.i0 + j);
                 float tg;
                 if (flags & GF_A_EULFIN) {
                     float pv[32];
 #pragma unroll
-                    for (int tp = 0; tp < 32; ++tp) pv[tp] = ldg(T.aux2 + ((size_t)min(tp, T.ln_width - 1) * T.M + row0 + r) * T.i0 + j);
+                    for (int tp = 0; tp < 32; ++tp) pv[tp] = ldx(T.aux2 + ((size_t)min(tp, T.ln_width - 1) * T.M + row0 + r) * T.i0 + j);
                     float sum = 0.f;
 #pragma unroll
                     for (int tp = 0; tp < 32; ++tp) sum += (tp < T.ln_width) ? pv[tp] : 0.f;
-                    tg = clip1(ldg(T.aux + (size_t)(row0 + r) * T.i0 + j) + (sum + ldg(T.eb + j)) * T.f1);
+                    tg = clip1(ldx(T.aux + (size_t)(row0 + r) * T.i0 + j) + (sum + ldg(T.eb + j)) * T.f1);
                     if (tn == 0) stg(const_cast<float*>(T.evp) + (size_t)(row0 + r) * T.i0 + j, tg);
-                } else tg = ldg(T.evp + (size_t)(row0 + r) * T.i0 + j);
+                } else tg = ldx(T.evp + (size_t)(row0 + r) * T.i0 + j);
                 g = T.f0 * (ar - tg);
                 if (ar > -1.0f && ar < 1.0f) {
                     const size_t o = (size_t)(row0 + r) * T.e_ntp + T.i1 + j;
-                    g += ldg(T.ew + o) + ldg(T.ew4 + o);
+                    g += ldx(T.ew + o) + ldx(T.ew4 + o);
                 }
                 if (tn == 0 && T.ea_out) stg(T.ea_out + (size_t)(row0 + r) * T.i0 + j, g);
             }
@@ -588,7 +604,7 @@
         for (int i = 0; i < NA; ++i) {
             const int f = min(tid + i * FQL_THREADS, nA - 1);
             const int r = sdiv(f, rk4), kk = f - r * k4;
-            av[i] = ldg4(Ag + (size_t)r * T.lda + 4 * kk);
+            av[i] = ldx4(Ag, (unsigned)(r * T.lda + 4 * kk));
         }
         if (pass == 0) issue_b();
 #pragma unroll
@@ -663,7 +679,7 @@
 #pragma unroll
         for (int rt = 0; rt < TMT; ++rt)
 #pragma unroll
-            for (int i = 0; i < 4; ++i) zpre[rt][i] = ldg(T.Zprev + (size_t)(row0 + 16 * rt + 4 * q + i) * T.ldc + n0 + c);
+            for (int i = 0; i < 4; ++i) zpre[rt][i] = ldx(T.Zprev + (size_t)(row0 + 16 * rt + 4 * q + i) * T.ldc + n0 + c);
     }
     f32x4 acc[TMT];
 #pragma unroll
@@ -741,7 +757,7 @@
         if (flags & GF_EULER) {
             float* xr = T.aux + (size_t)row * T.i0 + T.i1;
             if (n < T.i2) {
-                const float a = ldg(xr + n) + v * T.f0;
+                const float a = ldx(xr + n) + v * T.f0;
                 stg(xr + n, a);
                 if (flags & GF_EULER_LAST) stg(T.aux2 + (size_t)row * T.ldc + n, clip1(a));
             }
@@ -805,9 +821,9 @@
         f32x4 pv[NR][4];
 #pragma unroll
         for (int i = 0; i < NR; ++i) {
-            const float* pp = partials + (size_t)(row_first + 16 * i) * rs;
-#pragma unroll
-            for (int t = 0; t < 4; ++t) pv[i][t] = ldg4(pp + 4 * min(base + t, nf4 - 1));
+            const unsigned po = (unsigned)((row_first + 16 * i) * rs);
+#pragma unroll
+            for (int t = 0; t < 4; ++t) pv[i][t] = ldx4(partials, po + 4 * min(base + t, nf4 - 1));
         }
 #pragma unroll
         for (int i = 0; i < NR; ++i)
@@ -847,11 +863,12 @@
     constexpr int NRA = 2 * RI;
     f32x4 ra0[NRA], rb0[4], ra1[NRA], rb1[4], lg0, lb0, lg1, lb1;
     lg0 = lb0 = lg1 = lb1 = f32x4{0.f, 0.f, 0.f, 0.f};
-    const float* __restrict__ Ag = T.A + (size_t)(row0 + sr) * T.lda + 4 * sc4;
+    const float* __restrict__ Ag = T.A + (size_t)row0 * T.lda;
+    const unsigned ao = (unsigned)(sr * T.lda + 4 * sc4);
     const float* __restrict__ Bg = transb ? T.B + (size_t)(n0 + sr) * T.ldb + 4 * sc4 : T.B + (size_t)sr * T.ldb + n0 + 4 * sc4;
     auto load_chunk = [&](f32x4 (&ra)[NRA], f32x4 (&rb)[4], f32x4& lg, f32x4& lb, int k0) {
 #pragma unroll
-        for (int i = 0; i < NRA; ++i) ra[i] = ldg4(Ag + (size_t)(16 * i) * T.lda + k0);
+        for (int i = 0; i < NRA; ++i) ra[i] = ldx4(Ag, ao, (unsigned)(16 * i * T.lda + k0));
 #pragma unroll
         for (int i = 0; i < 4; ++i) rb[i] = transb ? ldg4(Bg + (size_t)(16 * i) * T.ldb + k0) : ldg4(Bg + (size_t)(k0 + 16 * i) * T.ldb);
         if (a_ln) { lg = ldg4(T.ln_g + k0 + 4 * sc4); lb = ldg4(T.ln_b + k0 + 4 * sc4); }
@@ -970,8 +987,8 @@
                 float v = acc[i][j][r] + (j ? bias1 : bias0);
                 if (flags & GF_SAVE_Z) { float gg, dg; gelu_both(v, gg, dg); stg(T.Zout + o, dg); v = (flags & GF_GELU) ? gg : v; }
                 else if (flags & GF_GELU) v = gelu_f(v);
-                if (flags & GF_GELUGRAD) v *= ldg(T.Zprev + o);
-                if (flags & GF_RELUGRAD) v = (ldg(T.Zprev + o) > 0.f) ? v : 0.f;
+                if (flags & GF_GELUGRAD) v *= ldx(T.Zprev + o);
+                if (flags & GF_RELUGRAD) v = (ldx(T.Zprev + o) > 0.f) ? v : 0.f;
                 stg(T.C + o, v);
                 s1[i][r] += v; s2[i][r] += v * v;
             }
@@ -1039,13 +1056,14 @@
     const int sr = tid >> 4, sc4 = tid & 15;
     const int br0 = (transb || NJ == 2) ? sr : (tid >> 3), brs = (transb || NJ == 2) ? 16 : 32;
     const int bc4 = (transb || NJ == 2) ? sc4 : (tid & 7);
-    const float* __restrict__ Ag = T.A + (size_t)(row0 + sr) * T.lda + 4 * sc4;
+    const float* __restrict__ Ag = T.A + (size_t)row0 * T.lda;
+    const unsigned ao = (unsigned)(sr * T.lda + 4 * sc4);
     const float* __restrict__ Bg = transb ? T.B + (size_t)(n0 + br0) * T.ldb + 4 * bc4 : T.B + (size_t)br0 * T.ldb + n0 + 4 * bc4;
     f32x4 ra0[2], rb0[NB], ra1[2], rb1[NB], lg0, lb0, lg1, lb1;
     lg0 = lb0 = lg1 = lb1 = f32x4{0.f, 0.f, 0.f, 0.f};
     auto load_chunk = [&](f32x4 (&ra)[2], f32x4 (&rb)[NB], f32x4& lg, f32x4& lb, int k0) {
 #pragma unroll
-        for (int i = 0; i < 2; ++i) ra[i] = ldg4(Ag + (size_t)(16 * i) * T.lda + k0);
+        for (int i = 0; i < 2; ++i) ra[i] = ldx4(Ag, ao, (unsigned)(16 * i * T.lda + k0));
 #pragma unroll
         for (int i = 0; i < NB; ++i) rb[i] = transb ? ldg4(Bg + (size_t)(brs * i) * T.ldb + k0) : ldg4(Bg + (size_t)(k0 + brs * i) * T.ldb);
         if (a_ln) { lg = ldg4(T.ln_g + k0 + 4 * sc4); lb = ldg4(T.ln_b + k0 + 4 * sc4); }
@@ -1156,9 +1174,9 @@
 #pragma unroll
                 for (int r = 0; r < 4; ++r) v[r] = gelu_f(v[r]);
             }
-            if (flags & GF_GELUGRAD) v *= ldg4(T.Zprev + o);
+            if (flags & GF_GELUGRAD) v *= ldx4(T.Zprev + (size_t)row0 * T.ldc, (unsigned)((16 * wr + c) * T.ldc + n));
             if (flags & GF_RELUGRAD) {
-                const f32x4 zp = ldg4(T.Zprev + o);
+                const f32x4 zp = ldx4(T.Zprev + (size_t)row0 * T.ldc, (unsigned)((16 * wr + c) * T.ldc + n));
 #pragma unroll
                 for (int r = 0; r < 4; ++r) v[r] = (zp[r] > 0.f) ? v[r] : 0.f;
             }
@@ -1232,13 +1250,14 @@
     const int sr = tid >> 4, sc4 = tid & 15;
     const int br0 = (transb || NJ == 2) ? sr : (tid >> 3), brs = (transb || NJ == 2) ? 16 : 32;
     const int bc4 = (transb || NJ == 2) ? sc4 : (tid & 7);
-    const float* __restrict__ Ag = T.A + (size_t)(row0 + sr) * T.lda + 4 * sc4;
+    const float* __restrict__ Ag = T.A + (size_t)row0 * T.lda;
+    const unsigned ao = (unsigned)(sr * T.lda + 4 * sc4);
     const float* __restrict__ Bg = transb ? T.B + (size_t)(n0 + br0) * T.ldb + 4 * bc4 : T.B + (size_t)br0 * T.ldb + n0 + 4 * bc4;
     f32x4 ra0[2], rb0[NB], ra1[2], rb1[NB], lg0, lb0, lg1, lb1;
     lg0 = lb0 = lg1 = lb1 = f32x4{0.f, 0.f, 0.f, 0.f};
     auto load_chunk = [&](f32x4 (&ra)[2], f32x4 (&rb)[NB], f32x4& lg, f32x4& lb, int k0) {
 #pragma unroll
-        for (int i = 0; i < 2; ++i) ra[i] = ldg4(Ag + (size_t)(16 * i) * T.lda + k0);
+        for (int i = 0; i < 2; ++i) ra[i] = ldx4(Ag, ao, (unsigned)(16 * i * T.lda + k0));
 #pragma unroll
         for (int i = 0; i < NB; ++i) rb[i] = transb ? ldg4(Bg + (size_t)(brs * i) * T.ldb + k0) : ldg4(Bg + (size_t)(k0 + brs * i) * T.ldb);
         if (a_ln) { lg = ldg4(T.ln_g + k0 + 4 * sc4); lb = ldg4(T.ln_b + k0 + 4 * sc4); }
@@ -1377,9 +1396,9 @@
 #pragma unroll
                 for (int r = 0; r < 4; ++r) v[r] = gelu_f(v[r]);
             }
-            if (flags & GF_GELUGRAD) v *= ldg4(T.Zprev + o);
+            if (flags & GF_GELUGRAD) v *= ldx4(T.Zprev + (size_t)row0 * T.ldc, (unsigned)((16 * wr + c) * T.ldc + n));
             if (flags & GF_RELUGRAD) {
-                const f32x4 zp = ldg4(T.Zprev + o);
+                const f32x4 zp = ldx4(T.Zprev + (size_t)row0 * T.ldc, (unsigned)((16 * wr + c) * T.ldc + n));
 #pragma unroll
                 for (int r = 0; r < 4; ++r) v[r] = (zp[r] > 0.f) ? v[r] : 0.f;
             }
@@ -1451,8 +1470,8 @@
 #pragma unroll
     for (int i = 0; i < 8; ++i) {
         const bool v = i < cnt;
-        a[i] = v ? *(const FQL_GAS f32x2*)(xp + i * sx + xo) : f32x2{0.f, 0.f};
-        b[i] = v ? ldg4(zp + i * sz + zo) : f32x4{0.f, 0.f, 0.f, 0.f};
+        a[i] = v ? ldx2(xp, xo, (unsigned)(i * sx)) : f32x2{0.f, 0.f};
+        b[i] = v ? ldx4(zp, zo, (unsigned)(i * sz)) : f32x4{0.f, 0.f, 0.f, 0.f};
     }
 }
 template <int NU>
@@ -1552,8 +1571,8 @@
 #pragma unroll
         for (int i = 0; i < 8; ++i) {
             const int st = min(s0 + i, steps - 1);
-            a[i] = ldg(xp + st * sx + xo);
-            b[i] = ldg4(zp + st * sz + zo);
+            a[i] = ldx(xp + st * sx + xo);
+            b[i] = ldx4(zp, zo, (unsigned)(st * sz));
         }
     };
     auto mma = [&](const float (&a)[8], const f32x4 (&b)[8], int s0) {
@@ -1600,23 +1619,21 @@
     if (local < T.ntiles_rows) {
         const int row = local * 4 + wave;
         if (row >= T.M) return;
-        const float mean = ldg(T.stats + 2 * row), rstd = ldg(T.stats + 2 * row + 1);
-        const float* dy = T.dY + (size_t)row * T.ld;
-        const float* z = T.Z + (size_t)row * T.ld;
-        const float* gv = T.Gv + (size_t)row * T.ld;
-        const float dqr = SYN ? ldg(T.dq + (size_t)row * T.ldq) : 0.f;
+        const float mean = ldx(T.stats + 2 * row), rstd = ldx(T.stats + 2 * row + 1);
+        const unsigned ro = (unsigned)(row * T.ld);
+        const float dqr = SYN ? ldx(T.dq + (size_t)row * T.ldq) : 0.f;
         f32x4 zz[4], dd[4], gm[4], gq[4];
 #pragma unroll
         for (int i = 0; i < 4; ++i) {
             const int k4 = 4 * (lane + 64 * i);
             if (k4 < T.H) {
-                zz[i] = ldg4(z + k4);
-                gq[i] = ldg4(gv + k4);
+                zz[i] = ldx4(T.Z, ro + k4);
+                gq[i] = ldx4(T.Gv, ro + k4);
                 gm[i] = ldg4(T.gamma + k4);
                 if (SYN) {
 #pragma unroll
                     for (int e = 0; e < 4; ++e) dd[i][e] = dqr * ldg(T.wq + (size_t)(k4 + e) * T.ldw);
-                } else dd[i] = ldg4(dy + k4);
+                } else dd[i] = ldx4(T.dY, ro + k4);
             } else zz[i] = gq[i] = gm[i] = dd[i] = f32x4{0.f, 0.f, 0.f, 0.f};
         }
         f32x4 d[4], xh[4];
@@ -1660,9 +1677,9 @@
 #pragma unroll
                 for (int u = 0; u < 16; ++u) {
                     const int m = min(m0 + 16 * u, T.M - 1);
-                    st[u] = *(const FQL_GAS f32x2*)(T.stats + 2 * m);
-                    dv[u] = SYN ? ldg(T.dq + (size_t)m * T.ldq) * wc : ldg(T.dY + (size_t)m * T.ld + col);
-                    zv[u] = ldg(T.Gv + (size_t)m * T.ld + col);
+                    st[u] = ldx2(T.stats, 2 * m);
+                    dv[u] = SYN ? ldx(T.dq + (size_t)m * T.ldq) * wc : ldx(T.dY + (size_t)m * T.ld + col);
+                    zv[u] = ldx(T.Gv + (size_t)m * T.ld + col);
                 }
 #pragma unroll
                 for (int u = 0; u < 16; ++u) {
@@ -1828,7 +1845,7 @@
     const int n = P.B * P.ad;
     for (int e = threadIdx.x; e < n; e += FQL_THREADS) {
         const int b = sdiv(e, frcp(P.ad)), a = e - b * P.ad;
-        const float d = clip1(P.A_os[(size_t)(2 * P.B + b) * P.ap + a]) - P.w_act[(size_t)b * P.ap + a];
+        const float d = clip1(ldx(P.A_os + (size_t)(2 * P.B + b) * P.ap + a)) - ldx(P.w_act + (size_t)b * P.ap + a);
         se += d * d;
     }
     const float tot = block_sum(se, sh);
@@ -1847,10 +1864,10 @@
     float sl = 0.f, sq = 0.f, mx = -INFINITY, mn = INFINITY;
     const float gs = 1.0f / (float)P.B;
     for (int b = threadIdx.x; b < P.B; b += FQL_THREADS) {
-        const float ta = P.tqa[(size_t)b * 16], tb = P.tqb[(size_t)b * 16];
+        const float ta = ldx(P.tqa + (size_t)b * 16), tb = ldx(P.tqb + (size_t)b * 16);
         const float nq = P.q_agg ? fminf(ta, tb) : 0.5f * (ta + tb);
-        const float y = P.w_rew[b] + P.discount * P.w_mask[b] * nq;
-        const float qa = P.q1a[(size_t)b * 16], qb = P.q1b[(size_t)b * 16];
+        const float y = ldx(P.w_rew + b) + P.discount * ldx(P.w_mask + b) * nq;
+        const float qa = ldx(P.q1a + (size_t)b * 16), qb = ldx(P.q1b + (size_t)b * 16);
         const float da = qa - y, db = qb - y;
         sl += da * da + db * db;
         sq += qa + qb;
@@ -1881,7 +1898,7 @@
 __device__ __forceinline__ void fql_loss_q_body(const LossQArgs& P, float* sh) {
     float s = 0.f, sa = 0.f;
     for (int b = threadIdx.x; b < P.B; b += FQL_THREADS) {
-        const float q = 0.5f * (P.q2a[(size_t)b * 16] + P.q2b[(size_t)b * 16]);
+        const float q = 0.5f * (ldx(P.q2a + (size_t)b * 16) + ldx(P.q2b + (size_t)b * 16));
         s += q; sa += fabsf(q);
     }
     const float ts = block_sum(s, sh), tsa = block_sum(sa, sh);
@@ -1913,7 +1930,7 @@
     float s = 0.f;
     for (int e = threadIdx.x; e < n; e += FQL_THREADS) {
         const int b = sdiv(e, frcp(P.ad)), a = e - b * P.ad;
-        const float d = P.pred[(size_t)b * P.ap + a] - P.vel[(size_t)b * P.ap + a];
+        const float d = ldx(P.pred + (size_t)b * P.ap + a) - ldx(P.vel + (size_t)b * P.ap + a);
         s += d * d;
         if (P.want_grad) P.dpred[(size_t)b * P.ap + a] = gs * d;
     }
@@ -1936,14 +1953,14 @@
     float s = 0.f;
     for (int e = threadIdx.x; e < n; e += FQL_THREADS) {
         const int b = sdiv(e, frcp(P.ad)), a = e - b * P.ad;
-        const float ar = P.a_raw[(size_t)b * P.ap + a];
-        const float d = ar - P.tgt[(size_t)b * P.ap + a];
+        const float ar = ldx(P.a_raw + (size_t)b * P.ap + a);
+        const float d = ar - ldx(P.tgt + (size_t)b * P.ap + a);
         s += d * d;
         if (P.want_grad) {
             float g = gs * d;
             if (ar > -1.0f && ar < 1.0f) {
                 const size_t o = (size_t)b * P.inp_c + P.od + a;
-                g += P.dxa[o] + P.dxb[o];
+                g += ldx(P.dxa + o) + ldx(P.dxb + o);
             }
             P.da[(size_t)b * P.ap + a] = g;
         }
@@ -1952,7 +1969,7 @@
     if (threadIdx.x == 0) {
         const float distill = t / (float)n;
         P.st->info[6] = distill;
-        P.st->info[4] = P.st->info[5] + P.alpha * distill + P.st->info[7];
+        P.st->info[4] = ldx(&P.st->info[5]) + P.alpha * distill + ldx(&P.st->info[7]);
     }
 }
 
@@ -2070,7 +2087,7 @@
         const int i = threadIdx.x + it * FQL_THREADS;
         if (i < n4) {
             const int o = ch.off + 4 * i;
-            f32x4 g = ldg4(A.G + o);
+            f32x4 g = ldx4(A.G, (unsigned)o);
             const f32x4 p = ldg4(A.P + o);
             f32x4 m = ldg4(A.Mu + o);
             f32x4 v = ldg4(A.Nu + o);
@@ -2078,10 +2095,10 @@
 #pragma unroll
             for (int e = 0; e < 4; ++e) {
                 const float ge = g[e] * gsc;
-                m[e] = 0.9f * m[e] + 0.1f * ge;
-                v[e] = 0.999f * v[e] + 0.001f * ge * ge;
+                m[e] = __builtin_fmaf(ge, 0.1f, 0.9f * m[e]);
+                v[e] = __builtin_fmaf(ge, 0.001f * ge, 0.999f * v[e]);
                 const float mh = m[e] / c1, vh = v[e] / c2;
-                pn[e] = p[e] - A.lr * (mh / (sqrtf(vh) + 1e-8f));
+                pn[e] = __builtin_fmaf(-A.lr, mh / (sqrtf(vh) + 1e-8f), p[e]);
                 ss += ge * ge; mx = fmaxf(mx, ge); mn = fminf(mn, ge);
             }
             stg4(A.Mu + o, m);
@@ -2090,7 +2107,7 @@
             if (o < A.critic_size) {
                 f32x4 t = ldg4(A.T + o);
 #pragma unroll
-                for (int e = 0; e < 4; ++e) t[e] = p[e] * A.tau + t[e] * (1.0f - A.tau);
+                for (int e = 0; e < 4; ++e) t[e] = __builtin_fmaf(p[e], A.tau, t[e] * (1.0f - A.tau));
                 stg4(A.T + o, t);
             }
         }
@@ -2144,11 +2161,11 @@
     const int r = sdiv(e, frcp(P.ad)), j = e - r * P.ad;
     float pv[32];
 #pragma unroll
-    for (int tp = 0; tp < 32; ++tp) pv[tp] = ldg(P.evp + ((size_t)min(tp, P.ntp - 1) * P.M + r) * P.ap + j);
+    for (int tp = 0; tp < 32; ++tp) pv[tp] = ldx(P.evp + ((size_t)min(tp, P.ntp - 1) * P.M + r) * P.ap + j);
     float sum = 0.f;
 #pragma unroll
     for (int tp = 0; tp < 32; ++tp) sum += (tp < P.ntp) ? pv[tp] : 0.f;
-    stg(P.tgt + (size_t)r * P.ap + j, clip1(ldg(P.a_in + (size_t)r * P.a_ld + j) + (sum + ldg(P.eb + j)) * P.scale));
+    stg(P.tgt + (size_t)r * P.ap + j, clip1(ldx(P.a_in + (size_t)r * P.a_ld + j) + (sum + ldg(P.eb + j)) * P.scale));
 }
 __global__ __launch_bounds__(FQL_THREADS) void fql_euler_finish_kernel(EulerFinishArgs P) { fql_euler_finish_body(P); }
 __global__ __launch_bounds__(FQL_THREADS) void fql_euler_finish_multi_kernel(const EulerFinishArgs* __restrict__ args) { const EulerFinishArgs P = args[blockIdx.y]; fql_euler_finish_body(P); }
```

Result: faster. 3053, median of 6 (+2.4%).
